# igashov/DiffLinker

Hardware: NVIDIA H100
Metric: molecules/sec (T=500 denoising) (higher is better)
Workload: dtype f32

## Files before the change

difflinker_b200/_native.py:

```python
import ctypes as C
import os

from .build import LIB_PATH, build_native, is_stale, nvcc_path

DL_OK, DL_NAN_DETECTED = 0, 1
GRAPH_TYPES = {"FC": 0, "4A": 1, "FC-4A": 2, "FC-10A-4A": 3}
EDGE_IMPLS = {"auto": 0, "simt": 1, "wgmma": 2}
SAMPLER_LINKER, SAMPLER_INPAINT = 0, 1


class DLConfig(C.Structure):
    _fields_ = [("n_dims", C.c_int32), ("in_node_nf", C.c_int32), ("context_node_nf", C.c_int32),
                ("hidden_nf", C.c_int32), ("n_layers", C.c_int32), ("inv_sublayers", C.c_int32),
                ("condition_time", C.c_int32), ("centering", C.c_int32), ("graph_type", C.c_int32),
                ("device", C.c_int32), ("edge_impl", C.c_int32), ("norm_constant", C.c_float),
                ("normalization_factor", C.c_float)]


class DLSizeGNNConfig(C.Structure):
    _fields_ = [("in_node_nf", C.c_int32), ("hidden_nf", C.c_int32), ("out_node_nf", C.c_int32),
                ("n_layers", C.c_int32), ("device", C.c_int32)]


class DLStepCoef(C.Structure):
    _fields_ = [("t", C.c_float), ("a", C.c_float), ("b", C.c_float), ("c", C.c_float), ("frame", C.c_int32),
                ("qa", C.c_float), ("qb", C.c_float), ("pad", C.c_float)]


_P, _I32, _I64, _F = C.c_void_p, C.c_int32, C.c_int64, C.c_float
SYMBOLS = {
    "dl_version": (C.c_char_p, []),
    "dl_last_error": (C.c_char_p, []),
    "dl_create": (_I32, [C.POINTER(DLConfig), C.POINTER(_P)]),
    "dl_destroy": (_I32, [_P]),
    "dl_set_weight": (_I32, [_P, C.c_char_p, _P, _I64]),
    "dl_finalize_weights": (_I32, [_P]),
    "dl_expected_param_count": (_I64, [_P]),
    "dl_dynamics_forward": (_I32, [_P, _I32, _I32, _P, _I32, _P, _P, _P, _P, _P, _P, _P, _P]),
    "dl_dynamics_forward_host": (_I32, [_P, _I32, _I32, _P, _I32, _P, _P, _P, _P, _P, _P, _P]),
    "dl_sample_chain": (_I32, [_P, _I32, _I32, _I32, _I32, _I32, _P, _P, _P, _P, _P, _P, _P, _P, _P, _P, _P, _P]),
    "dl_sample_chain_rng": (_I32, [_P, _I32, _I32, _I32, _I32, _I32, _P, _P, _P, _P, _P, _P, C.c_uint64, C.c_uint64, _P, _P, _P, _P,
                                   _P, _P]),
    "dl_set_noise_slice": (_I32, [_P, _I32, _I32]),
    "dl_noise_fill": (_I32, [_P, _I32, _I32, _I32, C.c_uint64, C.c_uint64, _P, _P, _P]),
    "dl_sample_chain_host": (_I32, [_P, _I32, _I32, _I32, _I32, _I32, _P, _P, _P, _P, _P, _P, _P, _P, _P, _P, _P]),
    "dl_launch_count": (_I64, [_P]),
    "dl_last_elapsed_ms": (_F, [_P]),
    "dl_time_edge_kernel": (_F, [_P, _I32]),
    "dl_selftest_tc": (_I32, [_P, C.POINTER(_F), C.POINTER(_F)]),
    "dl_selftest_tc_layout": (_I32, [_P, _I32, C.POINTER(_F), C.POINTER(_F)]),
    "dl_cut_graph_stats": (_I32, [_P, C.POINTER(_I64)]),
    "dl_sizegnn_create": (_I32, [C.POINTER(DLSizeGNNConfig), C.POINTER(_P)]),
    "dl_sizegnn_destroy": (_I32, [_P]),
    "dl_sizegnn_set_weight": (_I32, [_P, C.c_char_p, _P, _I64]),
    "dl_sizegnn_finalize_weights": (_I32, [_P]),
    "dl_sizegnn_forward": (_I32, [_P, _I32, _I32, _P, _P, _P, _P, _P]),
    "dl_restore_frame": (_I32, [_I32, _I32, _I32, _P, _P, _P, _P, _P]),
    "dl_restore_frame2": (_I32, [_I32, _I32, _I32, _I32, _P, _P, _P, _P, _P]),
    "dl_bond_orders": (_I32, [_I32, _I32, _I32, _P, _I32, _P, _P, _P, _P, _P, _P, _P]),
    "dl_format_xyz": (_I64, [_I32, _I32, _I32, _P, _I32, _P, _I32, _P, C.POINTER(C.c_char_p), _I32, _P, _I64, _P]),
}

_lib = None


def load_library():
    global _lib
    if _lib is not None:
        return _lib
    if is_stale():
        if nvcc_path() is not None:
            build_native()
        elif not os.path.isfile(LIB_PATH):
            raise RuntimeError(
                f"{LIB_PATH} is missing and nvcc is unavailable; build it with `python -m difflinker_b200.build`. "
                "difflinker_b200 has no CPU fallback.")
    lib = C.CDLL(LIB_PATH)
    for name, (res, args) in SYMBOLS.items():
        fn = getattr(lib, name)
        fn.restype = res
        fn.argtypes = args
    _lib = lib
    return lib


class NativeError(RuntimeError):
    pass


def check(status: int, what: str):
    if status < 0:
        raise NativeError(f"{what} failed with status {status}: {load_library().dl_last_error().decode()}")
    return status
```

difflinker_b200/build.py:

```python
import os
import shutil
import subprocess
import sys

PKG_DIR = os.path.dirname(os.path.abspath(__file__))
CSRC = os.path.join(PKG_DIR, "csrc")
LIB_PATH = os.path.join(PKG_DIR, "libdifflinker_b200.so")
SOURCES = ["dl_engine.cu", "output_stage.cu"]
HEADERS = ["common.cuh", "size_gnn.cuh", "kernels_simt.cuh", "kernels_tc.cuh", "kernels_node_tc.cuh", os.path.join("..", "..", "include", "difflinker_b200.h")]


def nvcc_path():
    for cand in (os.environ.get("NVCC"), shutil.which("nvcc"), "/usr/local/cuda/bin/nvcc"):
        if cand and os.path.isfile(cand):
            return cand
    return None


def is_stale() -> bool:
    if not os.path.isfile(LIB_PATH):
        return True
    t = os.path.getmtime(LIB_PATH)
    for f in SOURCES + HEADERS:
        p = os.path.join(CSRC, f)
        if os.path.isfile(p) and os.path.getmtime(p) > t:
            return True
    return False


def build_native(force: bool = False, verbose: bool = False) -> str:
    if not force and not is_stale():
        return LIB_PATH
    nvcc = nvcc_path()
    if nvcc is None:
        raise RuntimeError("nvcc not found: cannot build libdifflinker_b200.so")
    cmd = [nvcc, "-gencode", "arch=compute_90a,code=sm_90a", "-O3", "-lineinfo", "-std=c++17",
           "-Xcompiler", "-fPIC", "-shared", "-o", LIB_PATH] + [os.path.join(CSRC, s) for s in SOURCES]
    if verbose:
        cmd.insert(1, "-Xptxas=-v")
        print(" ".join(cmd), file=sys.stderr)
    res = subprocess.run(cmd, capture_output=True, text=True)
    if res.returncode != 0:
        raise RuntimeError(f"nvcc failed:\n{res.stdout}\n{res.stderr}")
    if verbose:
        print(res.stderr, file=sys.stderr)
    return LIB_PATH


if __name__ == "__main__":
    print(build_native(force="--force" in sys.argv, verbose=True))
```

difflinker_b200/csrc/common.cuh:

```cuda
#pragma once
#include <cuda_runtime.h>
#include <stdint.h>

namespace dl {

constexpr int H = 128;
constexpr int MAX_DIN = 32;
constexpr int MAX_XHD = 16;

__device__ __forceinline__ void chain_wait() { asm volatile("griddepcontrol.wait;" ::: "memory"); }
__device__ __forceinline__ void chain_release() { asm volatile("griddepcontrol.launch_dependents;" ::: "memory"); }

inline bool& chain_overlap_enabled() { static bool on = true; return on; }

template <typename... KArgs, typename... Args>
inline cudaError_t launch_chain(void (*kernel)(KArgs...), dim3 grid, dim3 block, size_t smem, cudaStream_t st, Args&&... args) {
  cudaLaunchConfig_t cfg = {};
  cfg.gridDim = grid; cfg.blockDim = block; cfg.dynamicSmemBytes = smem; cfg.stream = st;
  cudaLaunchAttribute at[1];
  at[0].id = cudaLaunchAttributeProgrammaticStreamSerialization;
  at[0].val.programmaticStreamSerializationAllowed = chain_overlap_enabled() ? 1 : 0;
  cfg.attrs = at; cfg.numAttrs = 1;
  return cudaLaunchKernelEx(&cfg, kernel, KArgs(static_cast<Args&&>(args))...);
}

__device__ __forceinline__ float silu_f(float x) {
  float t, r;
  asm("ex2.approx.ftz.f32 %0, %1;" : "=f"(t) : "f"(x * -1.4426950408889634f));
  asm("rcp.approx.ftz.f32 %0, %1;" : "=f"(r) : "f"(1.0f + t));
  return x * r;
}

__device__ __forceinline__ float usig_f(float u) {
  float t, r;
  asm("ex2.approx.ftz.f32 %0, %1;" : "=f"(t) : "f"(u));
  asm("rcp.approx.ftz.f32 %0, %1;" : "=f"(r) : "f"(1.0f + t));
  return u * r;
}

__device__ __forceinline__ float2 fadd2(float2 a, float2 b) { return make_float2(__fadd_rn(a.x, b.x), __fadd_rn(a.y, b.y)); }
__device__ __forceinline__ float2 fmul2(float2 a, float2 b) { return make_float2(__fmul_rn(a.x, b.x), __fmul_rn(a.y, b.y)); }
__device__ __forceinline__ float2 ffma2(float2 a, float2 b, float2 c) { return make_float2(__fmaf_rn(a.x, b.x, c.x), __fmaf_rn(a.y, b.y, c.y)); }
__device__ __forceinline__ float ex2_approx(float x) { float y; asm("ex2.approx.ftz.f32 %0, %1;" : "=f"(y) : "f"(x)); return y; }
__device__ __forceinline__ float rcp_approx(float x) { float y; asm("rcp.approx.ftz.f32 %0, %1;" : "=f"(y) : "f"(x)); return y; }
__device__ __forceinline__ float2 sigmoid_pair_log2(float2 u) {
  const float2 den = fadd2(make_float2(ex2_approx(fminf(u.x, 63.0f)), ex2_approx(fminf(u.y, 63.0f))), make_float2(1.0f, 1.0f));
  const float r = rcp_approx(den.x * den.y);
  return fmul2(make_float2(r, r), make_float2(den.y, den.x));
}
__device__ __forceinline__ void usig4(float2 u01, float2 u23, float2& s01, float2& s23) {
  const float2 one = make_float2(1.0f, 1.0f);
  const float2 ab = fadd2(make_float2(ex2_approx(fminf(u01.x, 31.0f)), ex2_approx(fminf(u01.y, 31.0f))), one);
  const float2 cd = fadd2(make_float2(ex2_approx(fminf(u23.x, 31.0f)), ex2_approx(fminf(u23.y, 31.0f))), one);
  const float2 m = fmul2(ab, cd);
  const float r = rcp_approx(m.x * m.y);
  const float2 rm = fmul2(make_float2(r, r), make_float2(m.y, m.x));
  s01 = fmul2(u01, fmul2(rm, cd));
  s23 = fmul2(u23, fmul2(rm, ab));
}
__device__ __forceinline__ float2 usig2(float2 u) { return fmul2(u, sigmoid_pair_log2(u)); }
__device__ __forceinline__ float2 silu2(float2 x) {
  return fmul2(x, sigmoid_pair_log2(fmul2(x, make_float2(-1.4426950408889634f, -1.4426950408889634f))));
}

struct GclW {
  const float* W1a_t;
  const float* W1b_t;
  const float* b1;
  const float* wd;
  const float* w0;
  const float* W2_t;
  const float* b2;
  const float* W3_t;
  const float* b3;
  const float* W4_t;
  const float* b4;
  const void* W2_tc;
  float w2_descale;
  float wdmax, w0max;
  const void* W1_tc;
  const void* W3_tc;
  const void* W4_tc;
  float w1_descale, w3_descale, w4_descale;
  const float* b1_u;
  const float* wd_u;
  const float* w0_u;
};

struct EqW {
  const float* W1a_t;
  const float* W1b_t;
  const float* b1;
  const float* wd;
  const float* w0;
  const float* W2_t;
  const float* b2;
  const float* w5;
  const void* W2_tc;
  float w2_descale;
  float wdmax, w0max;
  const void* W1_tc;
  float w1_descale;
  const float* b1_u;
  const float* wd_u;
  const float* w0_u;
};

struct ProjW {
  const float* W1a_t;
  const float* W1b_t;
  const float* b1;
};

struct Plan {
  const int* rowidx;
  const int* colidx;
  const int* xrowidx;
  const int* nr;
  const int* nc;
  const int* nxr;
  const int4* items;
  const int* n_items;
  const int* xmols;
  const int* n_xmols;
  const int4* xitems;
  const int* n_xitems;
};

struct Geom {
  int B, N;
  int F;
  int C;
  int D;
  int graph_type;
  float norm_constant;
  float normalization_factor;
};

}
```

difflinker_b200/csrc/dl_engine.cu:

```cuda
#include <cuda_fp16.h>
#include <cuda_runtime.h>

#include <algorithm>
#include <cmath>
#include <cstdarg>
#include <cstdio>
#include <cstdlib>
#include <cstring>
#include <ctime>
#include <map>
#include <string>
#include <vector>

#include "../../include/difflinker_b200.h"
#include "kernels_simt.cuh"
#include "kernels_tc.cuh"
#include "kernels_node_tc.cuh"

using namespace dl;

static thread_local char g_err[1024] = "";
static void set_err(const char* fmt, ...) {
  va_list ap;
  va_start(ap, fmt);
  vsnprintf(g_err, sizeof(g_err), fmt, ap);
  va_end(ap);
}

#define CK(call)                                                                          \
  do {                                                                                    \
    cudaError_t _e = (call);                                                              \
    if (_e != cudaSuccess) {                                                              \
      set_err("%s:%d %s -> %s", __FILE__, __LINE__, #call, cudaGetErrorString(_e));       \
      return DL_ERR_CUDA;                                                                 \
    }                                                                                     \
  } while (0)

namespace {

struct Workspace {
  int B = 0, N = 0;
  float *nm = nullptr, *x0 = nullptr, *xa = nullptr, *xb = nullptr, *h = nullptr, *ABg = nullptr, *ABc = nullptr,
        *agg = nullptr, *z = nullptr, *ABgmax = nullptr, *ABcmax = nullptr, *eps = nullptr;
  int* cls = nullptr;
  int *nbr = nullptr, *recs = nullptr, *xrecs = nullptr, *n_recs = nullptr;
  float4 *x04 = nullptr, *xa4 = nullptr, *xb4 = nullptr;
  int *rowidx = nullptr, *colidx = nullptr, *xrowidx = nullptr, *nr = nullptr, *nc = nullptr, *nxr = nullptr,
      *n_items = nullptr, *xmols = nullptr, *n_xmols = nullptr, *n_xitems = nullptr;
  int4* items = nullptr;
  int4* xitems = nullptr;
  int* tile_ctr = nullptr;
  std::vector<void*> allocs;
};

struct HostStage {
  size_t cap = 0;
  char* buf = nullptr;
};

}

struct dl_engine {
  dl_config cfg{};
  int D = 0;
  int num_sms = 0;
  int max_threads_per_sm = 2048;
  int slice_B_full = 0, slice_b0 = 0;
  bool finalized = false;
  std::map<std::string, std::vector<float>> raw;
  float* wblob = nullptr;
  void* wblob_tc = nullptr;
  std::vector<GclW> gcl;
  std::vector<EqW> eq;
  const float *We_t = nullptr, *be = nullptr, *Wo = nullptr, *bo = nullptr;
  Workspace ws;
  cudaStream_t loop_stream = nullptr;
  cudaEvent_t ev_in = nullptr, ev_out = nullptr, ev_t0 = nullptr, ev_t1 = nullptr;
  float* coef_dev = nullptr;
  int coef_cap = 0;
  int* step_ctr = nullptr;
  int64_t launches = 0;
  HostStage stage;
  bool use_tc = false;
  const int8_t* last_edge_mask = nullptr;
  const float* last_linker_mask = nullptr;
  int last_B = 0, last_N = 0;
};

namespace {

struct KernelTimes {
  bool on = false;
  struct Rec { const char* label; cudaEvent_t a, b; };
  std::vector<Rec> pending;
  std::map<std::string, std::pair<double, long>> acc;
  void begin(cudaStream_t st, const char* label) {
    if (!on) return;
    cudaStreamCaptureStatus cap = cudaStreamCaptureStatusNone;
    cudaStreamIsCapturing(st, &cap);
    if (cap != cudaStreamCaptureStatusNone) return;
    Rec r{label, nullptr, nullptr};
    cudaEventCreate(&r.a); cudaEventCreate(&r.b);
    cudaEventRecord(r.a, st);
    pending.push_back(r);
  }
  void end(cudaStream_t st) {
    if (!on || pending.empty() || pending.back().b == nullptr) return;
    cudaStreamCaptureStatus cap = cudaStreamCaptureStatusNone;
    cudaStreamIsCapturing(st, &cap);
    if (cap != cudaStreamCaptureStatusNone) return;
    cudaEventRecord(pending.back().b, st);
  }
  void collect(cudaStream_t st) {
    if (!on || pending.empty()) return;
    cudaStreamSynchronize(st);
    for (auto& r : pending) {
      float ms = 0.f;
      if (cudaEventElapsedTime(&ms, r.a, r.b) == cudaSuccess) { auto& a = acc[r.label]; a.first += ms; a.second += 1; }
      cudaEventDestroy(r.a); cudaEventDestroy(r.b);
    }
    pending.clear();
  }
  void report() {
    if (!on || acc.empty()) return;
    double tot = 0;
    for (auto& kv : acc) tot += kv.second.first;
    for (auto& kv : acc)
      fprintf(stderr, "[dl times] %-22s %6ld launches  avg %8.2f us  share %5.1f%%\n", kv.first.c_str(), kv.second.second,
              1e3 * kv.second.first / kv.second.second, 100.0 * kv.second.first / tot);
  }
};
KernelTimes g_times;
#define TIMED(label, stream, stmt) do { g_times.begin(stream, label); stmt; g_times.end(stream); } while (0)

struct ExpectedParam {
  std::string name;
  int64_t numel;
};

std::vector<ExpectedParam> expected_params(const dl_config& c) {
  const int D = c.in_node_nf + c.context_node_nf + (c.condition_time ? 1 : 0);
  const int Hh = c.hidden_nf;
  std::vector<ExpectedParam> v;
  v.push_back({"dynamics.embedding.weight", (int64_t)Hh * D});
  v.push_back({"dynamics.embedding.bias", Hh});
  v.push_back({"dynamics.embedding_out.weight", (int64_t)D * Hh});
  v.push_back({"dynamics.embedding_out.bias", D});
  char buf[160];
  for (int l = 0; l < c.n_layers; ++l) {
    for (int s = 0; s < c.inv_sublayers; ++s) {
      snprintf(buf, sizeof(buf), "dynamics.e_block_%d.gcl_%d.", l, s);
      std::string p(buf);
      v.push_back({p + "edge_mlp.0.weight", (int64_t)Hh * (2 * Hh + 2)});
      v.push_back({p + "edge_mlp.0.bias", Hh});
      v.push_back({p + "edge_mlp.2.weight", (int64_t)Hh * Hh});
      v.push_back({p + "edge_mlp.2.bias", Hh});
      v.push_back({p + "node_mlp.0.weight", (int64_t)Hh * 2 * Hh});
      v.push_back({p + "node_mlp.0.bias", Hh});
      v.push_back({p + "node_mlp.2.weight", (int64_t)Hh * Hh});
      v.push_back({p + "node_mlp.2.bias", Hh});
    }
    snprintf(buf, sizeof(buf), "dynamics.e_block_%d.gcl_equiv.", l);
    std::string p(buf);
    v.push_back({p + "coord_mlp.0.weight", (int64_t)Hh * (2 * Hh + 2)});
    v.push_back({p + "coord_mlp.0.bias", Hh});
    v.push_back({p + "coord_mlp.2.weight", (int64_t)Hh * Hh});
    v.push_back({p + "coord_mlp.2.bias", Hh});
    v.push_back({p + "coord_mlp.4.weight", Hh});
  }
  return v;
}

struct Packer {
  std::vector<float> blob;
  size_t add(const std::vector<float>& seg) {
    while (blob.size() % 4) blob.push_back(0.f);
    size_t off = blob.size();
    blob.insert(blob.end(), seg.begin(), seg.end());
    return off;
  }
};

std::vector<float> transpose_block(const std::vector<float>& W, int out, int in_stride, int c0, int k) {
  std::vector<float> t((size_t)k * out);
  for (int o = 0; o < out; ++o)
    for (int i = 0; i < k; ++i) t[(size_t)i * out + o] = W[(size_t)o * in_stride + c0 + i];
  return t;
}
std::vector<float> column(const std::vector<float>& W, int out, int in_stride, int c) {
  std::vector<float> t(out);
  for (int o = 0; o < out; ++o) t[o] = W[(size_t)o * in_stride + c];
  return t;
}

template <typename T>
dl_status dev_alloc(Workspace& ws, T** p, size_t count) {
  void* q = nullptr;
  CK(cudaMalloc(&q, std::max<size_t>(count, 1) * sizeof(T)));
  ws.allocs.push_back(q);
  *p = reinterpret_cast<T*>(q);
  return DL_OK;
}

void free_workspace(Workspace& ws) {
  for (void* p : ws.allocs) cudaFree(p);
  ws = Workspace();
}

dl_status ensure_workspace(dl_engine* e, int B, int N) {
  Workspace& ws = e->ws;
  if (ws.B == B && ws.N == N) return DL_OK;
  free_workspace(ws);
  const size_t n = (size_t)B * N;
  const int xd = 3 + e->cfg.in_node_nf;
  dl_status s;
#define WSA(field, cnt) if ((s = dev_alloc(ws, &ws.field, (cnt))) != DL_OK) return s
  WSA(nm, n); WSA(x0, n * 3); WSA(xa, n * 3); WSA(xb, n * 3); WSA(h, n * H); WSA(ABg, n * 2 * H); WSA(ABc, n * 2 * H);
  WSA(agg, n * H); WSA(z, n * xd); WSA(eps, n * xd); WSA(cls, n); WSA(x04, n); WSA(xa4, n); WSA(xb4, n); WSA(ABgmax, n * 2); WSA(ABcmax, n * 2);
  WSA(rowidx, n); WSA(colidx, n); WSA(xrowidx, n); WSA(nr, B); WSA(nc, B); WSA(nxr, B); WSA(n_items, 1);
  WSA(xmols, B); WSA(n_xmols, 1); WSA(items, n); WSA(xitems, n); WSA(n_xitems, 1); WSA(tile_ctr, 64);
  if (e->use_tc && e->cfg.graph_type != 0) { WSA(nbr, n * N); WSA(recs, n * CUT_REC); WSA(xrecs, n * CUT_REC); WSA(n_recs, 2); }
#undef WSA
  ws.B = B; ws.N = N;
  return DL_OK;
}

Plan make_plan(const Workspace& ws) {
  Plan p;
  p.rowidx = ws.rowidx; p.colidx = ws.colidx; p.xrowidx = ws.xrowidx; p.nr = ws.nr; p.nc = ws.nc; p.nxr = ws.nxr;
  p.items = ws.items; p.n_items = ws.n_items; p.xmols = ws.xmols; p.n_xmols = ws.n_xmols;
  p.xitems = ws.xitems; p.n_xitems = ws.n_xitems;
  return p;
}

Geom make_geom(const dl_engine* e, int B, int N) {
  Geom g;
  g.B = B; g.N = N; g.F = e->cfg.in_node_nf; g.C = e->cfg.context_node_nf; g.D = e->D;
  g.graph_type = e->cfg.graph_type; g.norm_constant = e->cfg.norm_constant;
  g.normalization_factor = e->cfg.normalization_factor;
  return g;
}

#define LAUNCH_CHECK()                                                                    \
  do {                                                                                    \
    cudaError_t _e = cudaGetLastError();                                                  \
    if (_e != cudaSuccess) {                                                              \
      set_err("%s:%d kernel launch -> %s", __FILE__, __LINE__, cudaGetErrorString(_e));   \
      return DL_ERR_CUDA;                                                                 \
    }                                                                                     \
  } while (0)

dl_status build_plan(dl_engine* e, int B, int N, const int8_t* node_mask, const float* linker_mask,
                     const int8_t* edge_mask, cudaStream_t st) {
  Workspace& ws = e->ws;
  CK(cudaMemsetAsync(ws.agg, 0, (size_t)B * N * H * sizeof(float), st));
  k_plan_mol<<<B, 256, 2 * N * sizeof(int), st>>>(N, e->cfg.graph_type, edge_mask, node_mask, linker_mask, ws.rowidx,
                                                  ws.colidx, ws.xrowidx, ws.nr, ws.nc, ws.nxr);
  LAUNCH_CHECK();
  const int tile_edges = e->use_tc ? tc::TN : ET;
  const int max_rows = e->use_tc ? tc::MAXR : MAXR;
  k_plan_items<<<1, 1, 0, st>>>(B, tile_edges, max_rows, 1, max_rows, ws.nr, ws.nc, ws.nxr, ws.items, ws.n_items, ws.xmols,
                                ws.n_xmols, ws.xitems, ws.n_xitems);
  LAUNCH_CHECK();
  e->launches += 2;
  return DL_OK;
}

struct FwdIO {
  const float* xh = nullptr; const float* t = nullptr; int t_numel = 0; float* out = nullptr;
  const int8_t* node_mask = nullptr; const float* linker_mask = nullptr; const int8_t* edge_mask = nullptr;
  const float* context = nullptr; int* nan_flags = nullptr;
  bool sampler = false; bool inpaint = false; const float* xh0 = nullptr; const float* upd_linker_mask = nullptr;
  const float* fragment_mask = nullptr; const float* noise = nullptr; float* chain = nullptr;
  NoiseRng rng{};
  int T = 0; float norm0 = 1.f, norm1 = 1.f, bias1 = 0.f;
};

ProjW proj_of(const GclW& w) { return ProjW{w.W1a_t, w.W1b_t, w.b1}; }
ProjW proj_of(const EqW& w) { return ProjW{w.W1a_t, w.W1b_t, w.b1}; }

dl_status launch_edge(dl_engine* e, const Geom& gm, const EdgeArgs& ea, bool coord, const void* w2_tc, cudaStream_t st) {
  if (e->use_tc) {
    dl_status s = tc::launch_edge_tc(gm, ea, coord, w2_tc, e->num_sms, st);
    if (s != DL_OK) return s;
  } else {
    if (coord) k_edge_simt<true><<<e->num_sms, 256, EDGE_SIMT_SMEM, st>>>(gm, ea);
    else k_edge_simt<false><<<e->num_sms, 256, EDGE_SIMT_SMEM, st>>>(gm, ea);
  }
  LAUNCH_CHECK();
  e->launches += 1;
  return DL_OK;
}

dl_status enqueue_forward(dl_engine* e, int B, int N, const FwdIO& io, cudaStream_t st) {
  Workspace& ws = e->ws;
  const Geom gm = make_geom(e, B, N);
  const int n = B * N;
  const int L = e->cfg.n_layers, S = e->cfg.inv_sublayers;
  const int node_blocks = (n + NODE_TM - 1) / NODE_TM;
  const size_t node_smem = 3 * NODE_TM * LDX * sizeof(float);

  PrepArgs pa{};
  pa.xh = io.sampler ? ws.z : io.xh;
  pa.node_mask = io.node_mask; pa.linker_mask = io.linker_mask;
  pa.t = io.t; pa.t_numel = io.t_numel; pa.context = io.context;
  pa.We_t = e->We_t; pa.be = e->be; pa.proj = proj_of(e->gcl[0]);
  pa.nm = ws.nm; pa.x0 = ws.x0; pa.x = ws.xa; pa.x04 = e->use_tc ? ws.x04 : nullptr; pa.x4 = e->use_tc ? ws.xa4 : nullptr; pa.cls = ws.cls; pa.h = ws.h;
  pa.AB = e->use_tc ? nullptr : ws.ABg; pa.ABmax = ws.ABgmax;
  pa.coef = io.sampler ? e->coef_dev : nullptr;
  pa.step_prep = io.sampler ? e->step_ctr : nullptr;
  pa.step_fin = io.sampler ? e->step_ctr + 1 : nullptr;
  TIMED("k_prep", st, (launch_chain(k_prep, dim3(node_blocks), dim3(256), 0, st, gm, pa)));
  LAUNCH_CHECK();
  e->launches += 1;
  if (e->use_tc) {
    const GclW& w0 = e->gcl[0];
    tcn::NodeTcArgs ta{};
    ta.h = ws.h; ta.agg = ws.h; ta.nm = ws.nm; ta.proj_only = 1;
    ta.w3 = reinterpret_cast<const __half*>(w0.W3_tc); ta.w4 = reinterpret_cast<const __half*>(w0.W4_tc);
    ta.b3 = w0.b3; ta.b4 = w0.b4; ta.w3_descale = 1.f; ta.w4_descale = 1.f;
    ta.n_proj = 1; ta.pw[0] = reinterpret_cast<const __half*>(w0.W1_tc); ta.pb1[0] = w0.b1_u;
    ta.p_descale[0] = w0.w1_descale; ta.AB[0] = ws.ABg; ta.ABmax[0] = ws.ABgmax;
    ta.tile_nodes = tcn::pick_tile_nodes(n, e->num_sms);
    TIMED("k_node_tc(proj only)", st, (tcn::launch_node(n, ta, st)));
    LAUNCH_CHECK();
    e->launches += 1;
  }

  if (ws.nbr != nullptr) {
    CK(cudaMemsetAsync(ws.n_recs, 0, 2 * sizeof(int), st));
    k_nbr<<<B, 512, (size_t)N * CUT_SMEM_PER_NODE, st>>>(N, e->cfg.graph_type, ws.x04, ws.cls, ws.rowidx, ws.colidx,
                                                        ws.xrowidx, ws.nr, ws.nc, ws.nxr, ws.nbr, ws.recs, ws.xrecs,
                                                        ws.n_recs);
    LAUNCH_CHECK();
    e->launches += 1;
  }

  float* xin = ws.xa;
  float* xout = ws.xb;
  float4* xin4 = ws.xa4;
  float4* xout4 = ws.xb4;
  const Plan plan = make_plan(ws);
  const float ksc = e->use_tc ? 1.4426950408889634f : 1.0f;
  e->last_edge_mask = io.edge_mask; e->last_linker_mask = io.linker_mask; e->last_B = B; e->last_N = N;
  for (int l = 0; l < L; ++l) {
    for (int s = 0; s < S; ++s) {
      const GclW& w = e->gcl[l * S + s];
      EdgeArgs ea{};
      ea.AB = ws.ABg; ea.ABmax = ws.ABgmax; ea.w2_descale = w.w2_descale; ea.wdmax = w.wdmax * ksc; ea.w0max = w.w0max * ksc;
      ea.x = xin; ea.x0 = ws.x0; ea.x4 = xin4; ea.x04 = ws.x04; ea.x4_out = nullptr;
      ea.edge_mask = io.edge_mask; ea.cls = ws.cls; ea.nm = ws.nm;
      ea.linker_mask = io.linker_mask; ea.W2_t = w.W2_t; ea.b2 = w.b2; ea.wd = e->use_tc ? w.wd_u : w.wd; ea.w0 = e->use_tc ? w.w0_u : w.w0; ea.w5 = nullptr;
      ea.plan = plan; ea.agg = ws.agg; ea.x_out = nullptr; ea.nbr = ws.nbr; ea.recs = ws.recs; ea.n_recs = ws.n_recs;
      g_times.begin(st, "edge GCL");
      dl_status st2 = launch_edge(e, gm, ea, false, w.W2_tc, st);
      g_times.end(st);
      if (st2 != DL_OK) return st2;

      const bool last_sub = s + 1 >= S;
      if (e->use_tc) {
        tcn::NodeTcArgs ta{};
        ta.h = ws.h; ta.agg = ws.agg; ta.nm = ws.nm;
        ta.w3 = reinterpret_cast<const __half*>(w.W3_tc); ta.w4 = reinterpret_cast<const __half*>(w.W4_tc);
        ta.b3 = w.b3; ta.b4 = w.b4; ta.w3_descale = w.w3_descale; ta.w4_descale = w.w4_descale;
        if (!last_sub) {
          const GclW& nx = e->gcl[l * S + s + 1];
          ta.n_proj = 1; ta.pw[0] = reinterpret_cast<const __half*>(nx.W1_tc); ta.pb1[0] = nx.b1_u;
          ta.p_descale[0] = nx.w1_descale; ta.AB[0] = ws.ABg; ta.ABmax[0] = ws.ABgmax;
        } else {
          const EqW& q = e->eq[l];
          ta.n_proj = 1; ta.pw[0] = reinterpret_cast<const __half*>(q.W1_tc); ta.pb1[0] = q.b1_u;
          ta.p_descale[0] = q.w1_descale; ta.AB[0] = ws.ABc; ta.ABmax[0] = ws.ABcmax;
          if (l + 1 < L) {
            const GclW& nx = e->gcl[(l + 1) * S];
            ta.n_proj = 2; ta.pw[1] = reinterpret_cast<const __half*>(nx.W1_tc); ta.pb1[1] = nx.b1_u;
            ta.p_descale[1] = nx.w1_descale; ta.AB[1] = ws.ABg; ta.ABmax[1] = ws.ABgmax;
          }
        }
        ta.tile_nodes = tcn::pick_tile_nodes(n, e->num_sms);
        TIMED(ta.n_proj == 2 ? "k_node_tc(2 proj)" : "k_node_tc(1 proj)", st, (tcn::launch_node(n, ta, st)));
      } else {
        NodeArgs na{};
        na.h = ws.h; na.agg = ws.agg; na.nm = ws.nm; na.W3_t = w.W3_t; na.b3 = w.b3; na.W4_t = w.W4_t; na.b4 = w.b4;
        if (!last_sub) {
          na.proj1 = proj_of(e->gcl[l * S + s + 1]); na.AB1 = ws.ABg; na.ABmax1 = ws.ABgmax; na.AB2 = nullptr;
        } else {
          na.proj1 = proj_of(e->eq[l]); na.AB1 = ws.ABc; na.ABmax1 = ws.ABcmax;
          if (l + 1 < L) { na.proj2 = proj_of(e->gcl[(l + 1) * S]); na.AB2 = ws.ABg; na.ABmax2 = ws.ABgmax; }
          else na.AB2 = nullptr;
        }
        k_node<ACT_SILU><<<node_blocks, 256, node_smem, st>>>(n, na);
      }
      LAUNCH_CHECK();
      e->launches += 1;
    }
    k_copy_x<<<(n * 3 + 255) / 256, 256, 0, st>>>(n * 3, xin, xout, e->use_tc ? xin4 : nullptr, xout4);
    LAUNCH_CHECK();
    e->launches += 1;
    const EqW& w = e->eq[l];
    EdgeArgs ea{};
    ea.AB = ws.ABc; ea.ABmax = ws.ABcmax; ea.w2_descale = w.w2_descale; ea.wdmax = w.wdmax * ksc; ea.w0max = w.w0max * ksc;
    ea.x = xin; ea.x0 = ws.x0; ea.x4 = xin4; ea.x04 = ws.x04; ea.x4_out = xout4;
    ea.edge_mask = io.edge_mask; ea.cls = ws.cls; ea.nm = ws.nm;
    ea.linker_mask = io.linker_mask; ea.W2_t = w.W2_t; ea.b2 = w.b2; ea.wd = e->use_tc ? w.wd_u : w.wd; ea.w0 = e->use_tc ? w.w0_u : w.w0; ea.w5 = w.w5;
    ea.plan = plan; ea.agg = nullptr; ea.x_out = xout; ea.nbr = ws.nbr; ea.recs = ws.xrecs; ea.n_recs = ws.n_recs ? ws.n_recs + 1 : nullptr;
    g_times.begin(st, "edge COORD");
    dl_status st2 = launch_edge(e, gm, ea, true, w.W2_tc, st);
    g_times.end(st);
    if (st2 != DL_OK) return st2;
    std::swap(xin, xout);
    std::swap(xin4, xout4);
  }

  FinishArgs fa{};
  fa.h = ws.h; fa.x = xin; fa.x0 = ws.x0; fa.nm = ws.nm; fa.Wo = e->Wo; fa.bo = e->bo;
  fa.nan_flags = io.nan_flags;
  const bool fused_update = io.sampler && !io.inpaint;
  fa.out = fused_update ? nullptr : (io.sampler ? ws.eps : io.out);
  if (fused_update) {
    fa.z = ws.z; fa.fragment_mask = io.fragment_mask; fa.linker_mask = io.linker_mask; fa.noise = io.noise; fa.rng = io.rng;
    fa.coef = e->coef_dev; fa.step_fin = e->step_ctr + 1; fa.step_prep = e->step_ctr; fa.T = io.T;
    fa.norm0 = io.norm0; fa.norm1 = io.norm1; fa.bias1 = io.bias1; fa.chain = io.chain;
  } else if (io.sampler) {
    fa.tag_step = e->step_ctr + 1;
  }
  TIMED("k_finish", st, (launch_chain(k_finish, dim3((n + 15) / 16), dim3(256), 0, st, gm, fa)));
  LAUNCH_CHECK();
  e->launches += 1;
  if (e->cfg.centering || io.inpaint) {
    InpaintArgs ia{};
    ia.mode = io.inpaint ? 1 : 0;
    ia.eps = io.inpaint ? ws.eps : io.out; ia.nm = ws.nm; ia.z = ws.z; ia.xh0 = io.xh0;
    ia.fragment_mask = io.fragment_mask; ia.linker_mask = io.upd_linker_mask; ia.noise = io.noise; ia.coef = e->coef_dev;
    ia.step_prep = e->step_ctr; ia.step_fin = e->step_ctr + 1; ia.T = io.T;
    ia.norm0 = io.norm0; ia.norm1 = io.norm1; ia.bias1 = io.bias1; ia.chain = io.chain;
    k_inpaint<<<B, 256, 0, st>>>(gm, ia);
    LAUNCH_CHECK();
    e->launches += 1;
  }
  return DL_OK;
}

dl_status check_shapes(const dl_engine* e, int B, int N) {
  if (!e || !e->finalized) { set_err("engine not finalized (dl_finalize_weights)"); return DL_ERR_INVALID; }
  if (B <= 0 || N <= 0) { set_err("B and N must be positive (got %d, %d)", B, N); return DL_ERR_INVALID; }
  if ((int64_t)B * N * N > (int64_t)1 << 40) { set_err("B*N*N too large"); return DL_ERR_INVALID; }
  if (e->use_tc && e->cfg.graph_type != 0 && N > 4000) {
    set_err("cut-off graphs: N = %d exceeds the neighbour-list kernel's shared-memory staging (N <= 4000)", N);
    return DL_ERR_INVALID;
  }
  return DL_OK;
}

dl_status stage_reserve(dl_engine* e, size_t bytes) {
  if (e->stage.cap >= bytes) return DL_OK;
  if (e->stage.buf) cudaFree(e->stage.buf);
  e->stage.buf = nullptr; e->stage.cap = 0;
  CK(cudaMalloc((void**)&e->stage.buf, bytes));
  e->stage.cap = bytes;
  return DL_OK;
}

size_t align256(size_t v) { return (v + 255) & ~(size_t)255; }

}

extern "C" {

const char* dl_version(void) { return "difflinker_b200 0.1 (sm_90a)"; }
const char* dl_last_error(void) { return g_err; }

dl_status dl_create(const dl_config* cfg, dl_engine** out) {
  if (!cfg || !out) { set_err("null argument"); return DL_ERR_INVALID; }
  if (cfg->hidden_nf != H) { set_err("hidden_nf must be %d (got %d)", H, cfg->hidden_nf); return DL_ERR_UNSUPPORTED; }
  if (cfg->n_dims != 3) { set_err("n_dims must be 3"); return DL_ERR_UNSUPPORTED; }
  const int D = cfg->in_node_nf + cfg->context_node_nf + (cfg->condition_time ? 1 : 0);
  if (D > MAX_DIN || cfg->in_node_nf < 1 || 3 + cfg->in_node_nf > MAX_XHD) {
    set_err("unsupported feature widths F=%d C=%d", cfg->in_node_nf, cfg->context_node_nf);
    return DL_ERR_UNSUPPORTED;
  }
  if (cfg->n_layers < 1 || cfg->inv_sublayers < 1) { set_err("n_layers/inv_sublayers must be >= 1"); return DL_ERR_INVALID; }
  if (cfg->graph_type < 0 || cfg->graph_type > 3) { set_err("bad graph_type"); return DL_ERR_INVALID; }
  if (cfg->graph_type != DL_GRAPH_FC && cfg->context_node_nf < 2) {
    set_err("pocket graphs need fragment_only/pocket_only context columns"); return DL_ERR_INVALID;
  }
  int ndev = 0;
  CK(cudaGetDeviceCount(&ndev));
  if (cfg->device < 0 || cfg->device >= ndev) { set_err("device %d not available (%d devices)", cfg->device, ndev); return DL_ERR_INVALID; }
  CK(cudaSetDevice(cfg->device));
  cudaDeviceProp prop;
  CK(cudaGetDeviceProperties(&prop, cfg->device));
  if (prop.major != 9 || prop.minor != 0) {
    set_err("difflinker_b200 is built for sm_90a only; device is sm_%d%d", prop.major, prop.minor);
    return DL_ERR_UNSUPPORTED;
  }
  dl_engine* e = new dl_engine();
  e->cfg = *cfg;
  e->D = D;
  e->num_sms = prop.multiProcessorCount;
  e->max_threads_per_sm = prop.maxThreadsPerMultiProcessor;
  e->use_tc = tc::AVAILABLE && cfg->edge_impl != DL_EDGE_SIMT;
  CK(cudaStreamCreateWithFlags(&e->loop_stream, cudaStreamNonBlocking));
  CK(cudaEventCreateWithFlags(&e->ev_in, cudaEventDisableTiming));
  CK(cudaEventCreateWithFlags(&e->ev_out, cudaEventDisableTiming));
  CK(cudaEventCreate(&e->ev_t0));
  CK(cudaEventCreate(&e->ev_t1));
  CK(cudaMalloc((void**)&e->step_ctr, 2 * sizeof(int)));
  CK(cudaFuncSetAttribute(k_node<ACT_SILU>, cudaFuncAttributeMaxDynamicSharedMemorySize, 3 * NODE_TM * LDX * sizeof(float)));
  CK(cudaFuncSetAttribute(k_edge_simt<true>, cudaFuncAttributeMaxDynamicSharedMemorySize, (int)EDGE_SIMT_SMEM));
  CK(cudaFuncSetAttribute(k_edge_simt<false>, cudaFuncAttributeMaxDynamicSharedMemorySize, (int)EDGE_SIMT_SMEM));
  CK(cudaFuncSetAttribute(k_nbr, cudaFuncAttributeMaxDynamicSharedMemorySize, 4000 * CUT_SMEM_PER_NODE));
  if (getenv("DL_TIME_KERNELS")) g_times.on = true;
  if (const char* v = getenv("DL_WAIT_MODE")) { const int m = atoi(v); cudaMemcpyToSymbol(tc::c_wait_mode, &m, sizeof(int)); }
  if (const char* v = getenv("DL_CHAIN_OVERLAP")) chain_overlap_enabled() = atoi(v) != 0;
  dl_status s = tc::configure();
  if (s == DL_OK) s = tcn::configure_node();
  if (s != DL_OK) { set_err("cudaFuncSetAttribute failed for the tensor-core kernels"); delete e; return s; }
  *out = e;
  return DL_OK;
}

dl_status dl_destroy(dl_engine* e) {
  if (!e) return DL_OK;
  g_times.report();
  g_times.acc.clear();
  cudaSetDevice(e->cfg.device);
  cudaDeviceSynchronize();
  free_workspace(e->ws);
  if (e->wblob) cudaFree(e->wblob);
  if (e->wblob_tc) cudaFree(e->wblob_tc);
  if (e->coef_dev) cudaFree(e->coef_dev);
  if (e->step_ctr) cudaFree(e->step_ctr);
  if (e->stage.buf) cudaFree(e->stage.buf);
  if (e->loop_stream) cudaStreamDestroy(e->loop_stream);
  if (e->ev_in) cudaEventDestroy(e->ev_in);
  if (e->ev_out) cudaEventDestroy(e->ev_out);
  if (e->ev_t0) cudaEventDestroy(e->ev_t0);
  if (e->ev_t1) cudaEventDestroy(e->ev_t1);
  delete e;
  return DL_OK;
}

int64_t dl_expected_param_count(const dl_engine* e) {
  if (!e) return 0;
  int64_t n = 0;
  for (auto& p : expected_params(e->cfg)) n += p.numel;
  return n;
}

dl_status dl_set_weight(dl_engine* e, const char* name, const float* data, int64_t numel) {
  if (!e || !name || !data) { set_err("null argument"); return DL_ERR_INVALID; }
  for (auto& p : expected_params(e->cfg)) {
    if (p.name == name) {
      if (p.numel != numel) {
        set_err("weight %s: expected %lld elements, got %lld", name, (long long)p.numel, (long long)numel);
        return DL_ERR_WEIGHTS;
      }
      e->raw[p.name].assign(data, data + numel);
      e->finalized = false;
      return DL_OK;
    }
  }
  set_err("unexpected weight name %s", name);
  return DL_ERR_WEIGHTS;
}

dl_status dl_finalize_weights(dl_engine* e) {
  if (!e) { set_err("null engine"); return DL_ERR_INVALID; }
  CK(cudaSetDevice(e->cfg.device));
  for (auto& p : expected_params(e->cfg))
    if (!e->raw.count(p.name)) { set_err("missing weight %s", p.name.c_str()); return DL_ERR_WEIGHTS; }
  const int L = e->cfg.n_layers, S = e->cfg.inv_sublayers, D = e->D;
  const int IN1 = 2 * H + 2;
  Packer pk;
  std::vector<__half> tcblob;
  struct GOff { size_t W1a, W1b, b1, wd, w0, W2, b2, W3, b3, W4, b4, w5, tc, tc1, tc3, tc4, b1u, wdu, w0u; float descale, wdmax, w0max, d1, d3, d4; };
  auto scaled = [](const std::vector<float>& v) { std::vector<float> o(v.size()); for (size_t i = 0; i < v.size(); ++i) o[i] = (float)((double)v[i] * tc::NEG_LOG2E); return o; };
  auto absmax = [](const std::vector<float>& v) { float m = 0.f; for (float x : v) m = std::max(m, std::fabs(x)); return m; };
  std::vector<GOff> goff(L * S), eoff(L);
  auto R = [&](const std::string& k) -> const std::vector<float>& { return e->raw[k]; };
  size_t oWe = pk.add(transpose_block(R("dynamics.embedding.weight"), H, D, 0, D));
  size_t obe = pk.add(R("dynamics.embedding.bias"));
  size_t oWo = pk.add(R("dynamics.embedding_out.weight"));
  size_t obo = pk.add(R("dynamics.embedding_out.bias"));
  char buf[160];
  for (int l = 0; l < L; ++l) {
    for (int s = 0; s < S; ++s) {
      snprintf(buf, sizeof(buf), "dynamics.e_block_%d.gcl_%d.", l, s);
      std::string p(buf);
      GOff& o = goff[l * S + s];
      const auto& W1 = R(p + "edge_mlp.0.weight");
      o.W1a = pk.add(transpose_block(W1, H, IN1, 0, H));
      o.W1b = pk.add(transpose_block(W1, H, IN1, H, H));
      o.b1 = pk.add(R(p + "edge_mlp.0.bias"));
      o.wd = pk.add(column(W1, H, IN1, 2 * H));
      o.w0 = pk.add(column(W1, H, IN1, 2 * H + 1));
      o.W2 = pk.add(transpose_block(R(p + "edge_mlp.2.weight"), H, H, 0, H));
      o.b2 = pk.add(R(p + "edge_mlp.2.bias"));
      o.W3 = pk.add(transpose_block(R(p + "node_mlp.0.weight"), H, 2 * H, 0, 2 * H));
      o.b3 = pk.add(R(p + "node_mlp.0.bias"));
      o.W4 = pk.add(transpose_block(R(p + "node_mlp.2.weight"), H, H, 0, H));
      o.b4 = pk.add(R(p + "node_mlp.2.bias"));
      o.tc = tc::pack_w2(R(p + "edge_mlp.2.weight"), tcblob, &o.descale);
      o.tc1 = tcn::pack_blocks(scaled(W1), IN1, 2, tcblob, &o.d1);
      o.b1u = pk.add(scaled(R(p + "edge_mlp.0.bias")));
      o.wdu = pk.add(scaled(column(W1, H, IN1, 2 * H)));
      o.w0u = pk.add(scaled(column(W1, H, IN1, 2 * H + 1)));
      o.tc3 = tcn::pack_blocks(R(p + "node_mlp.0.weight"), 2 * H, 2, tcblob, &o.d3);
      o.tc4 = tcn::pack_blocks(R(p + "node_mlp.2.weight"), H, 1, tcblob, &o.d4);
      o.wdmax = absmax(column(W1, H, IN1, 2 * H)); o.w0max = absmax(column(W1, H, IN1, 2 * H + 1));
    }
    snprintf(buf, sizeof(buf), "dynamics.e_block_%d.gcl_equiv.", l);
    std::string p(buf);
    GOff& o = eoff[l];
    const auto& W1 = R(p + "coord_mlp.0.weight");
    o.W1a = pk.add(transpose_block(W1, H, IN1, 0, H));
    o.W1b = pk.add(transpose_block(W1, H, IN1, H, H));
    o.b1 = pk.add(R(p + "coord_mlp.0.bias"));
    o.wd = pk.add(column(W1, H, IN1, 2 * H));
    o.w0 = pk.add(column(W1, H, IN1, 2 * H + 1));
    o.W2 = pk.add(transpose_block(R(p + "coord_mlp.2.weight"), H, H, 0, H));
    o.b2 = pk.add(R(p + "coord_mlp.2.bias"));
    o.w5 = pk.add(R(p + "coord_mlp.4.weight"));
    o.tc = tc::pack_w2(R(p + "coord_mlp.2.weight"), tcblob, &o.descale);
    o.tc1 = tcn::pack_blocks(scaled(W1), IN1, 2, tcblob, &o.d1);
    o.b1u = pk.add(scaled(R(p + "coord_mlp.0.bias")));
    o.wdu = pk.add(scaled(column(W1, H, IN1, 2 * H)));
    o.w0u = pk.add(scaled(column(W1, H, IN1, 2 * H + 1)));
    o.wdmax = absmax(column(W1, H, IN1, 2 * H)); o.w0max = absmax(column(W1, H, IN1, 2 * H + 1));
  }
  if (e->wblob) { cudaFree(e->wblob); e->wblob = nullptr; }
  if (e->wblob_tc) { cudaFree(e->wblob_tc); e->wblob_tc = nullptr; }
  CK(cudaMalloc((void**)&e->wblob, pk.blob.size() * sizeof(float)));
  CK(cudaMemcpy(e->wblob, pk.blob.data(), pk.blob.size() * sizeof(float), cudaMemcpyHostToDevice));
  CK(cudaMalloc(&e->wblob_tc, std::max<size_t>(tcblob.size(), 1) * sizeof(__half)));
  CK(cudaMemcpy(e->wblob_tc, tcblob.data(), tcblob.size() * sizeof(__half), cudaMemcpyHostToDevice));
  const float* base = e->wblob;
  const __half* tbase = reinterpret_cast<const __half*>(e->wblob_tc);
  e->We_t = base + oWe; e->be = base + obe; e->Wo = base + oWo; e->bo = base + obo;
  e->gcl.assign(L * S, GclW{});
  e->eq.assign(L, EqW{});
  for (int i = 0; i < L * S; ++i) {
    const GOff& o = goff[i];
    e->gcl[i] = GclW{base + o.W1a, base + o.W1b, base + o.b1, base + o.wd, base + o.w0, base + o.W2, base + o.b2,
                     base + o.W3,  base + o.b3,  base + o.W4, base + o.b4, tbase + o.tc, o.descale, o.wdmax, o.w0max,
                     tbase + o.tc1, tbase + o.tc3, tbase + o.tc4, o.d1, o.d3, o.d4,
                     base + o.b1u, base + o.wdu, base + o.w0u};
  }
  for (int l = 0; l < L; ++l) {
    const GOff& o = eoff[l];
    e->eq[l] = EqW{base + o.W1a, base + o.W1b, base + o.b1, base + o.wd, base + o.w0,
                   base + o.W2,  base + o.b2,  base + o.w5, tbase + o.tc, o.descale, o.wdmax, o.w0max, tbase + o.tc1, o.d1,
                   base + o.b1u, base + o.wdu, base + o.w0u};
  }
  e->finalized = true;
  return DL_OK;
}

dl_status dl_dynamics_forward(dl_engine* e, int32_t B, int32_t N, const float* t, int32_t t_numel, const float* xh,
                              const int8_t* node_mask, const float* linker_mask, const int8_t* edge_mask,
                              const float* context, float* out, int32_t* nan_flags, void* stream) {
  dl_status s = check_shapes(e, B, N);
  if (s != DL_OK) return s;
  if (!xh || !node_mask || !out) { set_err("xh/node_mask/out must not be null"); return DL_ERR_INVALID; }
  if (e->cfg.condition_time && (!t || (t_numel != 1 && t_numel != B))) { set_err("t must hold 1 or B values"); return DL_ERR_INVALID; }
  if (e->cfg.context_node_nf > 0 && !context) { set_err("context required (context_node_nf=%d)", e->cfg.context_node_nf); return DL_ERR_INVALID; }
  CK(cudaSetDevice(e->cfg.device));
  cudaStream_t st = reinterpret_cast<cudaStream_t>(stream);
  if ((s = ensure_workspace(e, B, N)) != DL_OK) return s;
  CK(cudaEventRecord(e->ev_t0, st));
  if (nan_flags) CK(cudaMemsetAsync(nan_flags, 0, B * sizeof(int32_t), st));
  if ((s = build_plan(e, B, N, node_mask, linker_mask, edge_mask, st)) != DL_OK) return s;
  FwdIO io;
  io.xh = xh; io.t = t; io.t_numel = t_numel; io.out = out; io.node_mask = node_mask; io.linker_mask = linker_mask;
  io.edge_mask = edge_mask; io.context = context; io.nan_flags = nan_flags;
  if ((s = enqueue_forward(e, B, N, io, st)) != DL_OK) return s;
  CK(cudaEventRecord(e->ev_t1, st));
  g_times.collect(st);
  return DL_OK;
}

dl_status dl_dynamics_forward_host(dl_engine* e, int32_t B, int32_t N, const float* t, int32_t t_numel,
                                   const float* xh, const int8_t* node_mask, const float* linker_mask,
                                   const int8_t* edge_mask, const float* context, float* out, int32_t* nan_flags) {
  dl_status s = check_shapes(e, B, N);
  if (s != DL_OK) return s;
  CK(cudaSetDevice(e->cfg.device));
  const size_t n = (size_t)B * N;
  const int xd = 3 + e->cfg.in_node_nf, C = e->cfg.context_node_nf;
  const size_t o_t = 0, o_xh = o_t + align256(sizeof(float) * std::max(t_numel, 1)), o_nm = o_xh + align256(n * xd * 4),
               o_lm = o_nm + align256(n), o_em = o_lm + align256(n * 4), o_ctx = o_em + align256(n * N),
               o_out = o_ctx + align256(n * std::max(C, 1) * 4), o_fl = o_out + align256(n * xd * 4),
               total = o_fl + align256(B * 4);
  if ((s = stage_reserve(e, total)) != DL_OK) return s;
  char* d = e->stage.buf;
  cudaStream_t st = e->loop_stream;
  if (t) CK(cudaMemcpyAsync(d + o_t, t, sizeof(float) * t_numel, cudaMemcpyHostToDevice, st));
  CK(cudaMemcpyAsync(d + o_xh, xh, n * xd * 4, cudaMemcpyHostToDevice, st));
  CK(cudaMemcpyAsync(d + o_nm, node_mask, n, cudaMemcpyHostToDevice, st));
  if (linker_mask) CK(cudaMemcpyAsync(d + o_lm, linker_mask, n * 4, cudaMemcpyHostToDevice, st));
  if (edge_mask && e->cfg.graph_type == DL_GRAPH_FC) CK(cudaMemcpyAsync(d + o_em, edge_mask, n * N, cudaMemcpyHostToDevice, st));
  if (context) CK(cudaMemcpyAsync(d + o_ctx, context, n * C * 4, cudaMemcpyHostToDevice, st));
  s = dl_dynamics_forward(e, B, N, t ? (const float*)(d + o_t) : nullptr, t_numel, (const float*)(d + o_xh),
                          (const int8_t*)(d + o_nm), linker_mask ? (const float*)(d + o_lm) : nullptr,
                          (edge_mask && e->cfg.graph_type == DL_GRAPH_FC) ? (const int8_t*)(d + o_em) : nullptr,
                          context ? (const float*)(d + o_ctx) : nullptr, (float*)(d + o_out), (int32_t*)(d + o_fl), st);
  if (s != DL_OK) return s;
  std::vector<int32_t> flags(B);
  CK(cudaMemcpyAsync(out, d + o_out, n * xd * 4, cudaMemcpyDeviceToHost, st));
  CK(cudaMemcpyAsync(flags.data(), d + o_fl, B * 4, cudaMemcpyDeviceToHost, st));
  CK(cudaStreamSynchronize(st));
  bool any = false;
  for (int i = 0; i < B; ++i) { any |= flags[i] != 0; if (nan_flags) nan_flags[i] = flags[i]; }
  return any ? DL_NAN_DETECTED : DL_OK;
}

static void randn_geometry(const dl_engine* e, long long numel, int* S, unsigned long long* consumed) {
  long long grid = (numel + 255) / 256;
  grid = std::min<long long>(grid, (long long)e->num_sms * (e->max_threads_per_sm / 256));
  grid = std::max<long long>(grid, 1);
  *S = (int)(256 * grid);
  *consumed = (unsigned long long)(((numel - 1) / (4LL * *S) + 1) * 4);
}
static NoiseRng make_rng(const dl_engine* e, int B, int N, uint64_t seed, uint64_t offset) {
  NoiseRng q{};
  const int F = e->cfg.in_node_nf;
  unsigned long long cx = 0, ch = 0;
  const int B_full = e->slice_B_full > 0 ? e->slice_B_full : B;
  randn_geometry(e, (long long)B_full * N * 3, &q.Sx, &cx);
  randn_geometry(e, (long long)B_full * N * F, &q.Sh, &ch);
  q.seed = seed; q.offset = offset; q.cx = cx; q.per_draw = cx + ch; q.F = F; q.on = 1;
  q.g0 = e->slice_B_full > 0 ? e->slice_b0 * N : 0;
  return q;
}

static dl_status sample_chain_impl(dl_engine* e, int32_t sampler, int32_t B, int32_t N, int32_t T, int32_t keep_frames,
                                   const float* xh, const int8_t* node_mask, const float* fragment_mask,
                                   const float* linker_mask, const int8_t* edge_mask, const float* context,
                                   const float* noise, const NoiseRng* rng, const dl_step_coef* coef, const float* norm,
                                   float* chain, int32_t* nan_flags, void* stream);

dl_status dl_sample_chain(dl_engine* e, int32_t sampler, int32_t B, int32_t N, int32_t T, int32_t keep_frames,
                          const float* xh, const int8_t* node_mask, const float* fragment_mask,
                          const float* linker_mask, const int8_t* edge_mask, const float* context,
                          const float* noise, const dl_step_coef* coef, const float* norm, float* chain,
                          int32_t* nan_flags, void* stream) {
  if (!noise) { set_err("null argument (noise): use dl_sample_chain_rng to draw on the device"); return DL_ERR_INVALID; }
  return sample_chain_impl(e, sampler, B, N, T, keep_frames, xh, node_mask, fragment_mask, linker_mask, edge_mask, context, noise,
                           nullptr, coef, norm, chain, nan_flags, stream);
}

dl_status dl_sample_chain_rng(dl_engine* e, int32_t sampler, int32_t B, int32_t N, int32_t T, int32_t keep_frames,
                              const float* xh, const int8_t* node_mask, const float* fragment_mask,
                              const float* linker_mask, const int8_t* edge_mask, const float* context, uint64_t seed,
                              uint64_t offset, uint64_t* offset_consumed, const dl_step_coef* coef, const float* norm,
                              float* chain, int32_t* nan_flags, void* stream) {
  dl_status s = check_shapes(e, B, N);
  if (s != DL_OK) return s;
  if (e->slice_B_full > 0 && e->slice_b0 + B > e->slice_B_full) { set_err("batch slice [%d, %d) exceeds the full batch %d", e->slice_b0, e->slice_b0 + B, e->slice_B_full); return DL_ERR_INVALID; }
  if (sampler != DL_SAMPLER_LINKER) { set_err("device-side noise is implemented for the linker sampler (the inpainting sampler takes prepared slabs)"); return DL_ERR_UNSUPPORTED; }
  if (offset % 4 != 0) { set_err("philox offset must be a multiple of 4 (torch.Generator.get_offset())"); return DL_ERR_INVALID; }
  const NoiseRng q = make_rng(e, B, N, seed, offset);
  if (offset_consumed) *offset_consumed = (uint64_t)(T + 2) * q.per_draw;
  return sample_chain_impl(e, sampler, B, N, T, keep_frames, xh, node_mask, fragment_mask, linker_mask, edge_mask, context, nullptr,
                           &q, coef, norm, chain, nan_flags, stream);
}

dl_status dl_set_noise_slice(dl_engine* e, int32_t B_full, int32_t b0) {
  if (!e) { set_err("null engine"); return DL_ERR_INVALID; }
  if (B_full < 0 || b0 < 0 || (B_full > 0 && b0 >= B_full)) { set_err("bad batch slice (%d of %d)", b0, B_full); return DL_ERR_INVALID; }
  e->slice_B_full = B_full; e->slice_b0 = B_full > 0 ? b0 : 0;
  return DL_OK;
}

dl_status dl_noise_fill(dl_engine* e, int32_t n_draws, int32_t B, int32_t N, uint64_t seed, uint64_t offset, float* out,
                        uint64_t* offset_consumed, void* stream) {
  dl_status s = check_shapes(e, B, N);
  if (s != DL_OK) return s;
  if (!out || n_draws < 1) { set_err("null argument"); return DL_ERR_INVALID; }
  CK(cudaSetDevice(e->cfg.device));
  const NoiseRng q = make_rng(e, B, N, seed, offset);
  if (offset_consumed) *offset_consumed = (uint64_t)n_draws * q.per_draw;
  k_noise_fill<<<e->num_sms * 4, 256, 0, reinterpret_cast<cudaStream_t>(stream)>>>(n_draws, B * N, 3 + e->cfg.in_node_nf, q, out);
  LAUNCH_CHECK();
  return DL_OK;
}

static dl_status sample_chain_impl(dl_engine* e, int32_t sampler, int32_t B, int32_t N, int32_t T, int32_t keep_frames,
                                   const float* xh, const int8_t* node_mask, const float* fragment_mask,
                                   const float* linker_mask, const int8_t* edge_mask, const float* context,
                                   const float* noise, const NoiseRng* rng, const dl_step_coef* coef, const float* norm,
                                   float* chain, int32_t* nan_flags, void* stream) {
  dl_status s = check_shapes(e, B, N);
  if (s != DL_OK) return s;
  if (sampler != DL_SAMPLER_LINKER && sampler != DL_SAMPLER_INPAINT) { set_err("unknown sampler %d", sampler); return DL_ERR_INVALID; }
  const bool inpaint = sampler == DL_SAMPLER_INPAINT;
  if (inpaint != (e->cfg.centering != 0)) { set_err("the inpainting sampler needs a model built with centering=1 (and vice versa)"); return DL_ERR_INVALID; }
  if (!xh || !node_mask || !fragment_mask || !linker_mask || (!noise && !rng) || !coef || !norm || !chain) {
    set_err("null argument"); return DL_ERR_INVALID;
  }
  if (T < 1 || keep_frames < 1 || keep_frames > T) { set_err("need 1 <= keep_frames <= T"); return DL_ERR_INVALID; }
  if (e->cfg.context_node_nf > 0 && !context) { set_err("context required"); return DL_ERR_INVALID; }
  static_assert(sizeof(dl_step_coef) == 32, "dl_step_coef layout");
  CK(cudaSetDevice(e->cfg.device));
  cudaStream_t user = reinterpret_cast<cudaStream_t>(stream);
  cudaStream_t st = e->loop_stream;
  static const bool time_chain = getenv("DL_TIME_CHAIN") != nullptr;
  auto now_ms = [] { timespec ts; clock_gettime(CLOCK_MONOTONIC, &ts); return ts.tv_sec * 1e3 + ts.tv_nsec * 1e-6; };
  const double tc0 = time_chain ? now_ms() : 0.0;
  double tc_plan = 0, tc_capture = 0, tc_inst = 0, tc_launch = 0;
  if ((s = ensure_workspace(e, B, N)) != DL_OK) return s;
  if (e->coef_cap < T + 1) {
    if (e->coef_dev) cudaFree(e->coef_dev);
    e->coef_dev = nullptr;
    CK(cudaMalloc((void**)&e->coef_dev, (size_t)(T + 1) * sizeof(dl_step_coef)));
    e->coef_cap = T + 1;
  }
  if (user != st) {
    CK(cudaEventRecord(e->ev_in, user));
    CK(cudaStreamWaitEvent(st, e->ev_in, 0));
  }
  CK(cudaMemcpyAsync(e->coef_dev, coef, (size_t)(T + 1) * sizeof(dl_step_coef), cudaMemcpyHostToDevice, st));
  CK(cudaMemsetAsync(e->step_ctr, 0, 2 * sizeof(int), st));
  if (nan_flags) CK(cudaMemsetAsync(nan_flags, 0, B * sizeof(int32_t), st));
  const int n = B * N, xd = 3 + e->cfg.in_node_nf;
  CK(cudaMemsetAsync(chain, 0, (size_t)keep_frames * n * xd * sizeof(float), st));
  if (inpaint) {
    CK(cudaMemcpyAsync(e->ws.z, noise, (size_t)n * xd * sizeof(float), cudaMemcpyDeviceToDevice, st));
  } else {
    k_init_z<<<(n * xd + 255) / 256, 256, 0, st>>>(n, xd, xh, fragment_mask, linker_mask, noise, rng ? *rng : NoiseRng{}, e->ws.z);
    LAUNCH_CHECK();
    e->launches += 1;
  }
  if ((s = build_plan(e, B, N, node_mask, inpaint ? nullptr : linker_mask, edge_mask, st)) != DL_OK) return s;

  if (time_chain) { cudaStreamSynchronize(st); tc_plan = now_ms(); }
  FwdIO io;
  io.sampler = true; io.inpaint = inpaint; io.xh0 = xh; io.upd_linker_mask = linker_mask;
  io.node_mask = node_mask; io.linker_mask = inpaint ? nullptr : linker_mask; io.edge_mask = edge_mask;
  io.context = context; io.nan_flags = nan_flags; io.fragment_mask = fragment_mask; io.noise = noise;
  if (rng) io.rng = *rng;
  io.chain = chain; io.T = T; io.norm0 = norm[0]; io.norm1 = norm[1]; io.bias1 = norm[2];

  cudaGraph_t graph = nullptr;
  cudaGraphExec_t exec = nullptr;
  const int64_t before = e->launches;
  CK(cudaStreamBeginCapture(st, cudaStreamCaptureModeThreadLocal));
  s = enqueue_forward(e, B, N, io, st);
  cudaError_t ce = cudaStreamEndCapture(st, &graph);
  if (s != DL_OK) { if (graph) cudaGraphDestroy(graph); return s; }
  if (ce != cudaSuccess) { set_err("cudaStreamEndCapture -> %s", cudaGetErrorString(ce)); return DL_ERR_CUDA; }
  const int64_t per_step = e->launches - before;
  if (time_chain) tc_capture = now_ms();
  cudaError_t ge = cudaGraphInstantiate(&exec, graph, 0);
  if (time_chain) tc_inst = now_ms();
  if (ge == cudaSuccess) ge = cudaEventRecord(e->ev_t0, st);
  int failed_step = -1;
  for (int r = 0; ge == cudaSuccess && r <= T; ++r) {
    ge = cudaGraphLaunch(exec, st);
    if (ge != cudaSuccess) failed_step = r;
  }
  if (ge == cudaSuccess) ge = cudaEventRecord(e->ev_t1, st);
  if (time_chain) {
    tc_launch = now_ms();
    cudaStreamSynchronize(st);
    const double tc_done = now_ms();
    float loop = 0.f; cudaEventElapsedTime(&loop, e->ev_t0, e->ev_t1);
    fprintf(stderr, "[dl chain] setup+plan %.2f ms | capture %.2f | instantiate %.2f | %d graph launches enqueued in %.2f | wait for the GPU %.2f | device loop %.2f\n",
            tc_plan - tc0, tc_capture - tc_plan, tc_inst - tc_capture, T + 1, tc_launch - tc_inst, tc_done - tc_launch, loop);
  }
  if (ge == cudaSuccess && user != st) {
    ge = cudaEventRecord(e->ev_out, st);
    if (ge == cudaSuccess) ge = cudaStreamWaitEvent(user, e->ev_out, 0);
  }
  if (exec) cudaGraphExecDestroy(exec);
  cudaGraphDestroy(graph);
  if (ge != cudaSuccess) {
    if (failed_step >= 0) set_err("cudaGraphLaunch step %d -> %s", failed_step, cudaGetErrorString(ge));
    else set_err("%s:%d reverse-loop graph -> %s", __FILE__, __LINE__, cudaGetErrorString(ge));
    return DL_ERR_CUDA;
  }
  e->launches = before + per_step * (T + 1);
  return DL_OK;
}

dl_status dl_sample_chain_host(dl_engine* e, int32_t sampler, int32_t B, int32_t N, int32_t T, int32_t keep_frames,
                               const float* xh, const int8_t* node_mask, const float* fragment_mask,
                               const float* linker_mask, const int8_t* edge_mask, const float* context,
                               const float* noise, const dl_step_coef* coef, const float* norm, float* chain,
                               int32_t* nan_flags) {
  dl_status s = check_shapes(e, B, N);
  if (s != DL_OK) return s;
  if (!xh || !node_mask || !fragment_mask || !linker_mask || !noise || !coef || !norm || !chain) {
    set_err("null argument"); return DL_ERR_INVALID;
  }
  if (T < 1 || keep_frames < 1 || keep_frames > T) { set_err("need 1 <= keep_frames <= T"); return DL_ERR_INVALID; }
  CK(cudaSetDevice(e->cfg.device));
  const size_t n = (size_t)B * N;
  const int xd = 3 + e->cfg.in_node_nf, C = e->cfg.context_node_nf;
  const bool has_em = edge_mask && e->cfg.graph_type == DL_GRAPH_FC;
  const size_t n_slabs = sampler == DL_SAMPLER_INPAINT ? (size_t)2 * T + 3 : (size_t)T + 2;
  const size_t o_xh = 0, o_nm = o_xh + align256(n * xd * 4), o_fm = o_nm + align256(n), o_lm = o_fm + align256(n * 4),
               o_em = o_lm + align256(n * 4), o_ctx = o_em + align256(has_em ? n * N : 1),
               o_nz = o_ctx + align256(n * std::max(C, 1) * 4), o_ch = o_nz + align256((size_t)n_slabs * n * xd * 4),
               o_fl = o_ch + align256((size_t)keep_frames * n * xd * 4), total = o_fl + align256(B * 4);
  if ((s = stage_reserve(e, total)) != DL_OK) return s;
  char* d = e->stage.buf;
  cudaStream_t st = e->loop_stream;
  CK(cudaMemcpyAsync(d + o_xh, xh, n * xd * 4, cudaMemcpyHostToDevice, st));
  CK(cudaMemcpyAsync(d + o_nm, node_mask, n, cudaMemcpyHostToDevice, st));
  CK(cudaMemcpyAsync(d + o_fm, fragment_mask, n * 4, cudaMemcpyHostToDevice, st));
  CK(cudaMemcpyAsync(d + o_lm, linker_mask, n * 4, cudaMemcpyHostToDevice, st));
  if (has_em) CK(cudaMemcpyAsync(d + o_em, edge_mask, n * N, cudaMemcpyHostToDevice, st));
  if (context) CK(cudaMemcpyAsync(d + o_ctx, context, n * C * 4, cudaMemcpyHostToDevice, st));
  CK(cudaMemcpyAsync(d + o_nz, noise, n_slabs * n * xd * 4, cudaMemcpyHostToDevice, st));
  s = dl_sample_chain(e, sampler, B, N, T, keep_frames, (const float*)(d + o_xh), (const int8_t*)(d + o_nm),
                      (const float*)(d + o_fm), (const float*)(d + o_lm), has_em ? (const int8_t*)(d + o_em) : nullptr,
                      context ? (const float*)(d + o_ctx) : nullptr, (const float*)(d + o_nz), coef, norm,
                      (float*)(d + o_ch), (int32_t*)(d + o_fl), st);
  if (s != DL_OK) return s;
  std::vector<int32_t> flags(B);
  CK(cudaMemcpyAsync(chain, d + o_ch, (size_t)keep_frames * n * xd * 4, cudaMemcpyDeviceToHost, st));
  CK(cudaMemcpyAsync(flags.data(), d + o_fl, B * 4, cudaMemcpyDeviceToHost, st));
  CK(cudaStreamSynchronize(st));
  bool any = false;
  for (int i = 0; i < B; ++i) { any |= flags[i] != 0; if (nan_flags) nan_flags[i] = flags[i]; }
  return any ? DL_NAN_DETECTED : DL_OK;
}

int64_t dl_launch_count(const dl_engine* e) { return e ? e->launches : 0; }

float dl_last_elapsed_ms(dl_engine* e) {
  if (!e) return -1.f;
  float ms = -1.f;
  if (cudaEventElapsedTime(&ms, e->ev_t0, e->ev_t1) != cudaSuccess) { cudaGetLastError(); return -1.f; }
  return ms;
}

dl_status dl_cut_graph_stats(dl_engine* e, int64_t* out) {
  if (!e || !out) return DL_ERR_INVALID;
  Workspace& ws = e->ws;
  out[0] = out[1] = out[2] = out[3] = 0;
  if (ws.recs == nullptr) return DL_OK;
  if (cudaSetDevice(e->cfg.device) != cudaSuccess) return DL_ERR_CUDA;
  CK(cudaDeviceSynchronize());
  int n[2] = {0, 0};
  CK(cudaMemcpy(n, ws.n_recs, sizeof(n), cudaMemcpyDeviceToHost));
  std::vector<int> recs((size_t)n[0] * CUT_REC);
  CK(cudaMemcpy(recs.data(), ws.recs, recs.size() * sizeof(int), cudaMemcpyDeviceToHost));
  out[0] = n[0]; out[3] = n[1];
  long long n_heavy = 0, e_heavy = 0, max_heavy = 0, rows_light = 0;
  for (int k = 0; k < n[0]; ++k) {
    const int* r = recs.data() + (size_t)k * CUT_REC;
    const bool heavy = (r[1] >> 8) & 1;
    out[1] += heavy ? (r[2] + tc::TN - 1) / tc::TN : 1;
    out[2] += r[2];
    if (heavy) { ++n_heavy; e_heavy += r[2]; max_heavy = std::max<long long>(max_heavy, r[2]); }
    else rows_light += r[1] & 0xff;
  }
  if (getenv("DL_DEBUG_CUT"))
    fprintf(stderr, "[dl cut] records %d (heavy %lld, deg sum %lld, max %lld; light rows %lld) tiles %lld edges %lld | coord records %d\n",
            n[0], n_heavy, e_heavy, max_heavy, rows_light, (long long)out[1], (long long)out[2], n[1]);
  return DL_OK;
}

float dl_time_edge_kernel(dl_engine* e, int32_t reps) {
  if (!e || !e->finalized || e->last_B == 0 || reps < 1) { set_err("dl_time_edge_kernel: no previous forward"); return -1.f; }
  if (cudaSetDevice(e->cfg.device) != cudaSuccess) return -1.f;
  Workspace& ws = e->ws;
  const Geom gm = make_geom(e, e->last_B, e->last_N);
  const GclW& w = e->gcl[0];
  EdgeArgs ea{};
  const float ksc = e->use_tc ? 1.4426950408889634f : 1.0f;
  ea.AB = ws.ABg; ea.ABmax = ws.ABgmax; ea.w2_descale = w.w2_descale; ea.wdmax = w.wdmax * ksc; ea.w0max = w.w0max * ksc;
  ea.x = ws.xa; ea.x0 = ws.x0; ea.x4 = ws.xa4; ea.x04 = ws.x04; ea.x4_out = nullptr; ea.edge_mask = e->last_edge_mask; ea.cls = ws.cls; ea.nm = ws.nm;
  ea.linker_mask = e->last_linker_mask; ea.W2_t = w.W2_t; ea.b2 = w.b2; ea.wd = e->use_tc ? w.wd_u : w.wd; ea.w0 = e->use_tc ? w.w0_u : w.w0; ea.w5 = nullptr;
  ea.plan = make_plan(ws); ea.agg = ws.agg; ea.x_out = nullptr; ea.nbr = ws.nbr; ea.recs = ws.recs; ea.n_recs = ws.n_recs;
  cudaStream_t st = e->loop_stream;
  for (int i = 0; i < 2; ++i) if (launch_edge(e, gm, ea, false, w.W2_tc, st) != DL_OK) return -1.f;
  if (cudaEventRecord(e->ev_t0, st) != cudaSuccess) return -1.f;
  for (int i = 0; i < reps; ++i) if (launch_edge(e, gm, ea, false, w.W2_tc, st) != DL_OK) return -1.f;
  if (cudaEventRecord(e->ev_t1, st) != cudaSuccess) return -1.f;
  if (cudaStreamSynchronize(st) != cudaSuccess) { set_err("dl_time_edge_kernel: %s", cudaGetErrorString(cudaGetLastError())); return -1.f; }
  float ms = -1.f;
  if (cudaEventElapsedTime(&ms, e->ev_t0, e->ev_t1) != cudaSuccess) return -1.f;
  return ms / reps;
}

dl_status dl_selftest_tc(dl_engine* e, float* max_abs_err, float* max_rel_err) {
  if (!e) { set_err("null engine"); return DL_ERR_INVALID; }
  CK(cudaSetDevice(e->cfg.device));
  return tc::selftest(e->num_sms, max_abs_err, max_rel_err, false);
}

dl_status dl_selftest_tc_layout(dl_engine* e, int32_t b_mn_major, float* max_abs_err, float* max_rel_err) {
  if (!e) { set_err("null engine"); return DL_ERR_INVALID; }
  CK(cudaSetDevice(e->cfg.device));
  if (b_mn_major < 0 || b_mn_major > 1) { set_err("b_mn_major must be 0 (K-major B) or 1 (MN-major B)"); return DL_ERR_INVALID; }
  return tc::selftest(e->num_sms, max_abs_err, max_rel_err, b_mn_major != 0);
}

}

#include "size_gnn.cuh"
```

difflinker_b200/csrc/kernels_simt.cuh:

```cuda
#pragma once
#include <curand_kernel.h>

#include "common.cuh"

namespace dl {

__global__ void k_plan_mol(int N, int graph_type, const int8_t* __restrict__ edge_mask,
                           const int8_t* __restrict__ node_mask, const float* __restrict__ linker_mask,
                           int* __restrict__ rowidx, int* __restrict__ colidx, int* __restrict__ xrowidx,
                           int* __restrict__ nr, int* __restrict__ nc, int* __restrict__ nxr) {
  extern __shared__ int sm_plan[];
  int* rowlive = sm_plan;
  int* collive = sm_plan + N;
  const int b = blockIdx.x;
  const int tid = threadIdx.x, lane = tid & 31, warp = tid >> 5, nwarp = blockDim.x >> 5;
  for (int i = tid; i < N; i += blockDim.x) { rowlive[i] = 0; collive[i] = 0; }
  __syncthreads();
  if ((graph_type == 0 || graph_type == 4) && edge_mask != nullptr) {
    const int8_t* em = edge_mask + (size_t)b * N * N;
    for (int i = warp; i < N; i += nwarp) {
      int any = 0;
      for (int j = lane; j < N; j += 32) {
        int v = em[(size_t)i * N + j];
        if (v != 0) { any = 1; collive[j] = 1; }
      }
      any = __any_sync(0xffffffffu, any);
      if (lane == 0 && any) rowlive[i] = 1;
    }
  } else if (graph_type == 0 || graph_type == 4) {
    for (int i = tid; i < N; i += blockDim.x) { rowlive[i] = 1; collive[i] = 1; }
  } else {
    for (int i = tid; i < N; i += blockDim.x) {
      int v = node_mask[(size_t)b * N + i] != 0;
      rowlive[i] = v; collive[i] = v;
    }
  }
  __syncthreads();
  if (tid == 0) {
    int a = 0, c = 0, x = 0;
    for (int i = 0; i < N; ++i) {
      if (rowlive[i]) {
        rowidx[(size_t)b * N + a++] = i;
        if (linker_mask == nullptr || linker_mask[(size_t)b * N + i] != 0.0f) xrowidx[(size_t)b * N + x++] = i;
      }
      if (collive[i]) colidx[(size_t)b * N + c++] = i;
    }
    nr[b] = a; nc[b] = c; nxr[b] = x;
  }
}

__global__ void k_plan_items(int B, int tile_edges, int max_rows, int col_pad, int max_rows_gcl, const int* __restrict__ nr,
                             const int* __restrict__ nc, const int* __restrict__ nxr, int4* __restrict__ items,
                             int* __restrict__ n_items, int* __restrict__ xmols, int* __restrict__ n_xmols,
                             int4* __restrict__ xitems, int* __restrict__ n_xitems, int n_cta = 0,
                             int* __restrict__ cta_begin = nullptr, int* __restrict__ xcta_begin = nullptr) {
  if (threadIdx.x != 0 || blockIdx.x != 0) return;
  int cnt = 0, xc = 0, xi = 0;
  for (int b = 0; b < B; ++b) {
    int r = nr[b], c = nc[b];
    if (r > 0 && c > 0) {
      const int cp = (c + col_pad - 1) / col_pad * col_pad;
      int per = cp >= tile_edges ? 1 : tile_edges / cp;
      if (per > max_rows_gcl) per = max_rows_gcl;
      for (int r0 = 0; r0 < r; r0 += per) items[cnt++] = make_int4(b, r0, min(per, r - r0), c);
    }
    if (nxr[b] > 0 && c > 0) {
      xmols[xc++] = b;
      int per;
      if (col_pad > 1) {
        const int cp = (c + col_pad - 1) / col_pad * col_pad;
        per = cp >= tile_edges ? 1 : tile_edges / cp;
        if (per > max_rows_gcl) per = max_rows_gcl;
      } else {
        per = c >= tile_edges ? 1 : tile_edges / c;
        if (per > max_rows) per = max_rows;
      }
      for (int r0 = 0; r0 < nxr[b]; r0 += per) xitems[xi++] = make_int4(b, r0, min(per, nxr[b] - r0), c);
    }
  }
  *n_items = cnt;
  *n_xmols = xc;
  *n_xitems = xi;
  if (n_cta > 0 && cta_begin != nullptr) {
    for (int pass = 0; pass < 2; ++pass) {
      const int4* list = pass == 0 ? items : xitems;
      const int total = pass == 0 ? cnt : xi;
      int* out = pass == 0 ? cta_begin : xcta_begin;
      if (out == nullptr) continue;
      long long sum = 0;
      for (int k = 0; k < total; ++k) sum += (long long)list[k].z * ((list[k].w + col_pad - 1) / col_pad * col_pad) + 32;
      long long run = 0;
      int c = 0;
      out[0] = 0;
      for (int k = 0; k < total; ++k) {
        while (c + 1 < n_cta && run * n_cta >= (long long)(c + 1) * sum) out[++c] = k;
        run += (long long)list[k].z * ((list[k].w + col_pad - 1) / col_pad * col_pad) + 32;
      }
      while (c < n_cta) out[++c] = total;
    }
  }
}

constexpr int ACT_SILU = 0, ACT_RELU = 1;
template <int ACT>
__device__ __forceinline__ float act_f(float x) { return ACT == ACT_RELU ? fmaxf(x, 0.f) : silu_f(x); }

constexpr int NODE_TM = 32;
constexpr int LDX = 132;

template <int K>
__device__ __forceinline__ void warp_gemm_4x4(const float* __restrict__ xs, const float* __restrict__ Wt, int lane,
                                              float (&acc)[4][4]) {
#pragma unroll 2
  for (int k = 0; k < K; k += 4) {
    float4 w[4], x[4];
#pragma unroll
    for (int q = 0; q < 4; ++q) w[q] = __ldg(reinterpret_cast<const float4*>(Wt + (size_t)(k + q) * H + lane * 4));
#pragma unroll
    for (int r = 0; r < 4; ++r) x[r] = *reinterpret_cast<const float4*>(xs + r * LDX + k);
#pragma unroll
    for (int r = 0; r < 4; ++r) {
      const float xv[4] = {x[r].x, x[r].y, x[r].z, x[r].w};
#pragma unroll
      for (int q = 0; q < 4; ++q) {
        acc[r][0] = fmaf(xv[q], w[q].x, acc[r][0]);
        acc[r][1] = fmaf(xv[q], w[q].y, acc[r][1]);
        acc[r][2] = fmaf(xv[q], w[q].z, acc[r][2]);
        acc[r][3] = fmaf(xv[q], w[q].w, acc[r][3]);
      }
    }
  }
}

__device__ __forceinline__ void zero_acc(float (&acc)[4][4]) {
#pragma unroll
  for (int r = 0; r < 4; ++r)
#pragma unroll
    for (int c = 0; c < 4; ++c) acc[r][c] = 0.f;
}

__device__ __forceinline__ float warp_absmax4(const float (&v)[4]) {
  float m = fmaxf(fmaxf(fabsf(v[0]), fabsf(v[1])), fmaxf(fabsf(v[2]), fabsf(v[3])));
#pragma unroll
  for (int o = 16; o > 0; o >>= 1) m = fmaxf(m, __shfl_xor_sync(0xffffffffu, m, o));
  return m;
}

__device__ __forceinline__ void project_ab(const float* hs_warp, const ProjW& pw, float* __restrict__ AB,
                                           float* __restrict__ ABmax, int g0, int n_total, int warp, int lane) {
  float acc[4][4];
  zero_acc(acc);
  warp_gemm_4x4<H>(hs_warp, pw.W1a_t, lane, acc);
  const float4 bb = __ldg(reinterpret_cast<const float4*>(pw.b1 + lane * 4));
#pragma unroll
  for (int r = 0; r < 4; ++r) {
    int g = g0 + warp * 4 + r;
    const float o[4] = {acc[r][0] + bb.x, acc[r][1] + bb.y, acc[r][2] + bb.z, acc[r][3] + bb.w};
    const float mx = warp_absmax4(o);
    if (g < n_total) {
      *reinterpret_cast<float4*>(AB + (size_t)g * 2 * H + lane * 4) = make_float4(o[0], o[1], o[2], o[3]);
      if (lane == 0) ABmax[(size_t)g * 2] = mx;
    }
  }
  zero_acc(acc);
  warp_gemm_4x4<H>(hs_warp, pw.W1b_t, lane, acc);
#pragma unroll
  for (int r = 0; r < 4; ++r) {
    int g = g0 + warp * 4 + r;
    const float mx = warp_absmax4(acc[r]);
    if (g < n_total) {
      *reinterpret_cast<float4*>(AB + (size_t)g * 2 * H + H + lane * 4) =
          make_float4(acc[r][0], acc[r][1], acc[r][2], acc[r][3]);
      if (lane == 0) ABmax[(size_t)g * 2 + 1] = mx;
    }
  }
}

struct PrepArgs {
  const float* xh;
  const int8_t* node_mask;
  const float* linker_mask;
  const float* t;
  int t_numel;
  const float* context;
  const float* We_t;
  const float* be;
  ProjW proj;
  float* nm;
  float* x0;
  float* x;
  float4* x04;
  float4* x4;
  int* cls;
  float* h;
  float* AB;
  float* ABmax;
  const float* coef;
  const int* step_prep;
  int* step_fin;
};

__global__ void __launch_bounds__(256) k_prep(Geom gm, PrepArgs a) {
  __shared__ __align__(16) float hs[NODE_TM * LDX];
  __shared__ float hin[NODE_TM][MAX_DIN];
  const int tid = threadIdx.x, lane = tid & 31, warp = tid >> 5;
  const int n_total = gm.B * gm.N;
  const int g0 = blockIdx.x * NODE_TM;
  const int xd = 3 + gm.F;
  int step = 0;
  chain_wait();
  chain_release();
  if (a.step_prep != nullptr) {
    step = *a.step_prep;
    if (blockIdx.x == 0 && tid == 0) *a.step_fin = step;
  }
  for (int idx = tid; idx < NODE_TM * MAX_DIN; idx += 256) {
    int r = idx / MAX_DIN, d = idx % MAX_DIN;
    int g = g0 + r;
    float v = 0.f;
    if (g < n_total && d < gm.D) {
      float m = (float)a.node_mask[g];
      if (d < gm.F) {
        v = a.xh[(size_t)g * xd + 3 + d] * m;
      } else if (d == gm.F && gm.D > gm.F + gm.C) {
        if (a.coef != nullptr) v = a.coef[(size_t)step * 8 + 0];
        else v = a.t[a.t_numel == 1 ? 0 : g / gm.N];
      } else {
        int cidx = d - (gm.D - gm.C);
        v = a.context[(size_t)g * gm.C + cidx];
      }
    }
    hin[r][d] = v;
  }
  if (tid < NODE_TM) {
    int g = g0 + tid;
    if (g < n_total) {
      float m = (float)a.node_mask[g];
      a.nm[g] = m;
      for (int d = 0; d < 3; ++d) {
        float v = a.xh[(size_t)g * xd + d] * m;
        a.x0[(size_t)g * 3 + d] = v;
        a.x[(size_t)g * 3 + d] = v;
        if (a.x4 != nullptr) {
          reinterpret_cast<float*>(a.x04 + g)[d] = v;
          reinterpret_cast<float*>(a.x4 + g)[d] = v;
        }
      }
      if (gm.graph_type >= 1 && gm.graph_type <= 3) {
        int valid = m != 0.f;
        int pk = a.context[(size_t)g * gm.C + gm.C - 1] != 0.f;
        int fr = a.context[(size_t)g * gm.C + gm.C - 2] != 0.f;
        int lk = a.linker_mask != nullptr ? (a.linker_mask[g] != 0.f) : 0;
        int c = 0;
        if (valid) {
          if (gm.graph_type == 1) c = 1;
          else c = (lk || fr) ? 1 : (pk ? 2 : 3);
        }
        a.cls[g] = c;
      }
    }
  }
  __syncthreads();
  {
    float acc[4][4];
    zero_acc(acc);
    for (int d = 0; d < gm.D; ++d) {
      const float4 w = __ldg(reinterpret_cast<const float4*>(a.We_t + (size_t)d * H + lane * 4));
#pragma unroll
      for (int r = 0; r < 4; ++r) {
        float xv = hin[warp * 4 + r][d];
        acc[r][0] = fmaf(xv, w.x, acc[r][0]);
        acc[r][1] = fmaf(xv, w.y, acc[r][1]);
        acc[r][2] = fmaf(xv, w.z, acc[r][2]);
        acc[r][3] = fmaf(xv, w.w, acc[r][3]);
      }
    }
    const float4 bb = __ldg(reinterpret_cast<const float4*>(a.be + lane * 4));
#pragma unroll
    for (int r = 0; r < 4; ++r) {
      float4 o = make_float4(acc[r][0] + bb.x, acc[r][1] + bb.y, acc[r][2] + bb.z, acc[r][3] + bb.w);
      *reinterpret_cast<float4*>(hs + (warp * 4 + r) * LDX + lane * 4) = o;
      int g = g0 + warp * 4 + r;
      if (g < n_total) *reinterpret_cast<float4*>(a.h + (size_t)g * H + lane * 4) = o;
    }
  }
  __syncwarp();
  if (a.AB != nullptr) project_ab(hs + warp * 4 * LDX, a.proj, a.AB, a.ABmax, g0, n_total, warp, lane);
}

struct NodeArgs {
  float* h;
  const float* agg;
  const float* nm;
  const float* W3_t; const float* b3; const float* W4_t; const float* b4;
  ProjW proj1; float* AB1; float* ABmax1;
  ProjW proj2; float* AB2; float* ABmax2;
};

template <int ACT = ACT_SILU>
__global__ void __launch_bounds__(256) k_node(int n_total, NodeArgs a) {
  extern __shared__ __align__(16) float sm_node[];
  float* hs = sm_node;
  float* as = sm_node + NODE_TM * LDX;
  float* hid = as + NODE_TM * LDX;
  const int tid = threadIdx.x, lane = tid & 31, warp = tid >> 5;
  const int g0 = blockIdx.x * NODE_TM;
#pragma unroll
  for (int r = 0; r < 4; ++r) {
    int row = warp * 4 + r, g = g0 + row;
    float4 hv = make_float4(0, 0, 0, 0), av = hv;
    if (g < n_total) {
      hv = *reinterpret_cast<const float4*>(a.h + (size_t)g * H + lane * 4);
      av = *reinterpret_cast<const float4*>(a.agg + (size_t)g * H + lane * 4);
    }
    *reinterpret_cast<float4*>(hs + row * LDX + lane * 4) = hv;
    *reinterpret_cast<float4*>(as + row * LDX + lane * 4) = av;
  }
  __syncwarp();
  float acc[4][4];
  zero_acc(acc);
  warp_gemm_4x4<H>(hs + warp * 4 * LDX, a.W3_t, lane, acc);
  warp_gemm_4x4<H>(as + warp * 4 * LDX, a.W3_t + (size_t)H * H, lane, acc);
  {
    const float4 bb = __ldg(reinterpret_cast<const float4*>(a.b3 + lane * 4));
#pragma unroll
    for (int r = 0; r < 4; ++r)
      *reinterpret_cast<float4*>(hid + (warp * 4 + r) * LDX + lane * 4) =
          make_float4(act_f<ACT>(acc[r][0] + bb.x), act_f<ACT>(acc[r][1] + bb.y), act_f<ACT>(acc[r][2] + bb.z),
                      act_f<ACT>(acc[r][3] + bb.w));
  }
  __syncwarp();
  zero_acc(acc);
  warp_gemm_4x4<H>(hid + warp * 4 * LDX, a.W4_t, lane, acc);
  {
    const float4 bb = __ldg(reinterpret_cast<const float4*>(a.b4 + lane * 4));
#pragma unroll
    for (int r = 0; r < 4; ++r) {
      int row = warp * 4 + r, g = g0 + row;
      float m = g < n_total ? a.nm[g] : 0.f;
      float4 hv = *reinterpret_cast<const float4*>(hs + row * LDX + lane * 4);
      float4 o = make_float4((hv.x + (acc[r][0] + bb.x)) * m, (hv.y + (acc[r][1] + bb.y)) * m,
                             (hv.z + (acc[r][2] + bb.z)) * m, (hv.w + (acc[r][3] + bb.w)) * m);
      __syncwarp();
      *reinterpret_cast<float4*>(hs + row * LDX + lane * 4) = o;
      if (g < n_total) *reinterpret_cast<float4*>(a.h + (size_t)g * H + lane * 4) = o;
    }
  }
  __syncwarp();
  if (a.AB1 != nullptr) project_ab(hs + warp * 4 * LDX, a.proj1, a.AB1, a.ABmax1, g0, n_total, warp, lane);
  if (a.AB2 != nullptr) project_ab(hs + warp * 4 * LDX, a.proj2, a.AB2, a.ABmax2, g0, n_total, warp, lane);
}

__device__ __forceinline__ float edge_weight(int graph_type, const int8_t* __restrict__ em_mol, int N, int i, int j,
                                             int ci, int cj, float d0) {
  if (graph_type == 0) return em_mol != nullptr ? (float)em_mol[(size_t)i * N + j] : 1.0f;
  if (graph_type == 4)
    return ((em_mol == nullptr || em_mol[(size_t)i * N + j] != 0) && d0 < 6.0f) ? 1.f : 0.f;
  if (i == j || ci == 0 || cj == 0) return 0.f;
  float dist = sqrtf(d0);
  if (graph_type == 1) return dist <= 4.0f ? 1.f : 0.f;
  if (ci == 3 || cj == 3) return 0.f;
  if (ci == 1 && cj == 1) return 1.f;
  if (ci == 2 && cj == 2) return dist <= 4.0f ? 1.f : 0.f;
  float cut = graph_type == 2 ? 4.0f : 10.0f;
  return dist <= cut ? 1.f : 0.f;
}

constexpr int CUT_TN = 128;
constexpr int CUT_MAXR = 28;
constexpr int CUT_REC = 32;

__device__ __forceinline__ void cut_pack_rows(int b, int N, int nrows, const int* __restrict__ rowlist ,
                                              const int* degn, int* srt, int* row_bin, int* row_pos, int* row_start,
                                              int* bin_rem, int* bin_cnt, int* misc, int* __restrict__ recs,
                                              int* __restrict__ n_recs) {
  const int tid = threadIdx.x, lane = tid & 31, warp = tid >> 5;
  if (tid == 0) { misc[0] = 0; misc[1] = 0; }
  __syncthreads();
  for (int s = tid; s < nrows; s += blockDim.x) {
    const int node = rowlist[s], d = degn[node];
    if (d <= CUT_TN) {
      int rank = 0;
      for (int s2 = 0; s2 < nrows; ++s2) {
        const int d2 = degn[rowlist[s2]];
        rank += (d2 <= CUT_TN && (d2 > d || (d2 == d && s2 < s))) ? 1 : 0;
      }
      srt[rank] = node;
      atomicAdd(&misc[0], 1);
    } else {
      row_pos[node] = atomicAdd(&misc[1], 1);
    }
  }
  __syncthreads();
  const int n_light = misc[0], n_heavy = misc[1];
  if (warp == 0) {
    int nb = 0, first_open = 0;
    const int d_min = n_light > 0 ? degn[srt[n_light - 1]] : 0;
    for (int idx = 0; idx < n_light; ++idx) {
      const int node = srt[idx], d = degn[node];
      int found = -1;
      for (int base = first_open; base < nb && found < 0; base += 32) {
        const int bb = base + lane;
        const bool ok = bb < nb && bin_rem[bb] >= d && bin_cnt[bb] < CUT_MAXR;
        const unsigned m = __ballot_sync(0xffffffffu, ok);
        if (m) found = base + __ffs(m) - 1;
      }
      if (lane == 0) {
        if (found < 0) { bin_rem[nb] = CUT_TN; bin_cnt[nb] = 0; }
      }
      if (found < 0) { found = nb; ++nb; }
      __syncwarp();
      if (lane == 0) {
        row_bin[node] = found; row_pos[node] = bin_cnt[found]; row_start[node] = CUT_TN - bin_rem[found];
        bin_rem[found] -= d; bin_cnt[found] += 1;
      }
      __syncwarp();
      while (first_open < nb && (bin_rem[first_open] < d_min || bin_cnt[first_open] >= CUT_MAXR)) ++first_open;
    }
    if (lane == 0) {
      misc[2] = nb;
      misc[3] = atomicAdd(n_recs, nb + n_heavy);
    }
  }
  __syncthreads();
  const int nb = misc[2];
  int* out = recs + (size_t)misc[3] * CUT_REC;
  for (int bb = tid; bb < nb; bb += blockDim.x) {
    int* r = out + (size_t)bb * CUT_REC;
    r[0] = b; r[1] = bin_cnt[bb]; r[2] = CUT_TN - bin_rem[bb]; r[3] = 0;
  }
  for (int s = tid; s < nrows; s += blockDim.x) {
    const int node = rowlist[s], d = degn[node];
    if (d <= CUT_TN) {
      out[(size_t)row_bin[node] * CUT_REC + 4 + row_pos[node]] = node | (row_start[node] << 16);
    } else {
      int* r = out + (size_t)(nb + row_pos[node]) * CUT_REC;
      r[0] = b; r[1] = 1 | (1 << 8); r[2] = d; r[3] = 0; r[4] = node;
    }
  }
  __syncthreads();
}

__global__ void __launch_bounds__(512) k_nbr(int N, int graph_type, const float4* __restrict__ x04,
                                             const int* __restrict__ cls, const int* __restrict__ rowidx,
                                             const int* __restrict__ colidx, const int* __restrict__ xrowidx,
                                             const int* __restrict__ nr, const int* __restrict__ nc,
                                             const int* __restrict__ nxr, int* __restrict__ nbr,
                                             int* __restrict__ recs, int* __restrict__ xrecs,
                                             int* __restrict__ n_recs ) {
  extern __shared__ uint8_t sm_nbr[];
  float4* xs = reinterpret_cast<float4*>(sm_nbr);
  int* cl = reinterpret_cast<int*>(xs + N);
  int* col = cl + N;
  int* degn = col + N;
  int* srt = degn + N;
  int* row_bin = srt + N; int* row_pos = row_bin + N; int* row_start = row_pos + N;
  int* bin_rem = row_start + N; int* bin_cnt = bin_rem + N;
  __shared__ int misc[4];
  const int b = blockIdx.x, tid = threadIdx.x, lane = tid & 31, warp = tid >> 5, nwarp = blockDim.x >> 5;
  const size_t gb = (size_t)b * N;
  const int nrows = nr[b], ncols = nc[b];
  for (int i = tid; i < N; i += blockDim.x) {
    xs[i] = x04[gb + i]; cl[i] = cls[gb + i];
    col[i] = i < ncols ? colidx[gb + i] : 0;
    degn[i] = 0;
  }
  __syncthreads();
  for (int slot = warp; slot < nrows; slot += nwarp) {
    const int i = rowidx[gb + slot];
    const float4 xi = xs[i];
    const int ci = cl[i];
    int* out = nbr + (gb + i) * N;
    int count = 0;
    for (int c0 = 0; c0 < ncols; c0 += 32) {
      const int c = c0 + lane;
      bool keep = false;
      int j = 0;
      if (c < ncols) {
        j = col[c];
        const float4 xj = xs[j];
        const float ex = xi.x - xj.x, ey = xi.y - xj.y, ez = xi.z - xj.z;
        const float d0 = ex * ex + ey * ey + ez * ez;
        keep = edge_weight(graph_type, nullptr, N, i, j, ci, cl[j], d0) != 0.f;
      }
      const unsigned m = __ballot_sync(0xffffffffu, keep);
      if (keep) out[count + __popc(m & ((1u << lane) - 1u))] = j;
      count += __popc(m);
    }
    if (lane == 0) {
      if (count == 0) { out[0] = i | (int)0x80000000; count = 1; }
      degn[i] = count;
    }
  }
  __syncthreads();
  cut_pack_rows(b, N, nrows, rowidx + gb, degn, srt, row_bin, row_pos, row_start, bin_rem, bin_cnt, misc, recs, n_recs);
  cut_pack_rows(b, N, nxr[b], xrowidx + gb, degn, srt, row_bin, row_pos, row_start, bin_rem, bin_cnt, misc, xrecs, n_recs + 1);
}
constexpr int CUT_SMEM_PER_NODE = 16 + 9 * 4;

constexpr int ET = 128;
constexpr int MAXR = 8;
constexpr int LDB = H + 1;

struct EdgeArgs {
  const float* AB;
  const float* ABmax;
  float w2_descale, wdmax, w0max;
  const float* x;
  const float* x0;
  const float4* x4;
  const float4* x04;
  float4* x4_out;
  const int8_t* edge_mask;
  const int* cls;
  const float* nm;
  const float* linker_mask;
  const float* W2_t; const float* b2; const float* wd; const float* w0; const float* w5;
  Plan plan;
  float* agg;
  float* x_out;
  const int* nbr;
  const int* recs;
  const int* n_recs;
};

constexpr size_t EDGE_SIMT_SMEM =
    sizeof(float) * ((size_t)H * H  + (size_t)H * ET  + (size_t)ET * LDB  + (size_t)MAXR * H  +
                     4 * H  + ET  + ET * 3  + ET );

template <bool COORD, int ACT = ACT_SILU>
__global__ void __launch_bounds__(256, 1) k_edge_simt(Geom gm, EdgeArgs a) {
  extern __shared__ __align__(16) float sm_edge[];
  float* W2s = sm_edge;
  float* S1 = W2s + H * H;
  float* Bs = S1 + H * ET;
  float* As = Bs + ET * LDB;
  float* b2s = As + MAXR * H;
  float* wds = b2s + H;
  float* w0s = wds + H;
  float* w5s = w0s + H;
  float* ems = w5s + H;
  float* cds = ems + ET;
  float* phis = cds + ET * 3;
  __shared__ float xacc[COORD ? 1 : 1];
  (void)xacc;

  const int tid = threadIdx.x, lane = tid & 31, warp = tid >> 5;
  const int N = gm.N;
  for (int idx = tid; idx < H * H / 4; idx += 256)
    reinterpret_cast<float4*>(W2s)[idx] = __ldg(reinterpret_cast<const float4*>(a.W2_t) + idx);
  if (tid < H) {
    b2s[tid] = a.b2[tid]; wds[tid] = a.wd[tid]; w0s[tid] = a.w0[tid];
    w5s[tid] = COORD ? a.w5[tid] : 0.f;
  }
  __syncthreads();

  const int n_work = COORD ? *a.plan.n_xmols : *a.plan.n_items;
  for (int wi = blockIdx.x; wi < n_work; wi += gridDim.x) {
    int b, r_begin, r_count;
    if (COORD) { b = a.plan.xmols[wi]; r_begin = 0; r_count = a.plan.nxr[b]; }
    else { int4 it = a.plan.items[wi]; b = it.x; r_begin = it.y; r_count = it.z; }
    const int nc = a.plan.nc[b];
    const int* rows = (COORD ? a.plan.xrowidx : a.plan.rowidx) + (size_t)b * N;
    const int* cols = a.plan.colidx + (size_t)b * N;
    const size_t gb = (size_t)b * N;
    const int8_t* em_mol = a.edge_mask ? a.edge_mask + gb * N : nullptr;
    int per = nc >= ET ? 1 : ET / nc;
    if (per > MAXR) per = MAXR;

    for (int rt = 0; rt < r_count; rt += per) {
      const int nrt = min(per, r_count - rt);
      for (int r = warp; r < nrt; r += 8) {
        int i = rows[r_begin + rt + r];
        *reinterpret_cast<float4*>(As + r * H + lane * 4) =
            *reinterpret_cast<const float4*>(a.AB + (gb + i) * 2 * H + lane * 4);
      }
      float run = 0.f;
      float xrun = 0.f;
      for (int c0 = 0; c0 < nc; c0 += ET) {
        const int ncc = min(ET, nc - c0);
        const int Et = nrt * ncc;
        __syncthreads();
        for (int idx = tid; idx < ncc * H; idx += 256) {
          int jj = idx >> 7, k = idx & (H - 1);
          Bs[jj * LDB + k] = a.AB[(gb + cols[c0 + jj]) * 2 * H + H + k];
        }
        __syncthreads();
        {
          const int e = tid & (ET - 1), kh = tid >> 7;
          const bool valid = e < Et;
          int rr = 0, jj = 0;
          float d = 0.f, d0 = 0.f;
          if (valid) {
            rr = e / ncc; jj = e - rr * ncc;
            const int i = rows[r_begin + rt + rr], j = cols[c0 + jj];
            const float* xi = a.x + (gb + i) * 3; const float* xj = a.x + (gb + j) * 3;
            const float* yi = a.x0 + (gb + i) * 3; const float* yj = a.x0 + (gb + j) * 3;
            float dx = xi[0] - xj[0], dy = xi[1] - xj[1], dz = xi[2] - xj[2];
            d = dx * dx + dy * dy + dz * dz;
            float ex = yi[0] - yj[0], ey = yi[1] - yj[1], ez = yi[2] - yj[2];
            d0 = ex * ex + ey * ey + ez * ez;
            if (kh == 0) {
              int ci = 0, cj = 0;
              if (gm.graph_type >= 1 && gm.graph_type <= 3) { ci = a.cls[gb + i]; cj = a.cls[gb + j]; }
              ems[e] = edge_weight(gm.graph_type, em_mol, N, i, j, ci, cj, d0);
              if (COORD) {
                float inv = 1.0f / (sqrtf(d + 1e-8f) + gm.norm_constant);
                cds[e * 3 + 0] = dx * inv; cds[e * 3 + 1] = dy * inv; cds[e * 3 + 2] = dz * inv;
              }
            }
          } else if (kh == 0) {
            ems[e] = 0.f;
            if (COORD) { cds[e * 3 + 0] = 0.f; cds[e * 3 + 1] = 0.f; cds[e * 3 + 2] = 0.f; }
          }
          const float* Ar = As + rr * H;
          const float* Br = Bs + jj * LDB;
#pragma unroll 8
          for (int kk = 0; kk < H / 2; ++kk) {
            int k = kh * (H / 2) + kk;
            float pre = Ar[k] + Br[k] + d * wds[k] + d0 * w0s[k];
            S1[k * ET + e] = valid ? act_f<ACT>(pre) : 0.f;
          }
        }
        __syncthreads();
        const int ty = tid >> 4, tx = tid & 15;
        float acc[8][8];
#pragma unroll
        for (int p = 0; p < 8; ++p)
#pragma unroll
          for (int q = 0; q < 8; ++q) acc[p][q] = 0.f;
#pragma unroll 4
        for (int k = 0; k < H; ++k) {
          float4 a0 = *reinterpret_cast<const float4*>(S1 + k * ET + ty * 4);
          float4 a1 = *reinterpret_cast<const float4*>(S1 + k * ET + 64 + ty * 4);
          float4 b0 = *reinterpret_cast<const float4*>(W2s + k * H + tx * 4);
          float4 b1 = *reinterpret_cast<const float4*>(W2s + k * H + 64 + tx * 4);
          const float av[8] = {a0.x, a0.y, a0.z, a0.w, a1.x, a1.y, a1.z, a1.w};
          const float bv[8] = {b0.x, b0.y, b0.z, b0.w, b1.x, b1.y, b1.z, b1.w};
#pragma unroll
          for (int p = 0; p < 8; ++p)
#pragma unroll
            for (int q = 0; q < 8; ++q) acc[p][q] = fmaf(av[p], bv[q], acc[p][q]);
        }
        __syncthreads();
        float* Outs = S1;
#pragma unroll
        for (int p = 0; p < 8; ++p) {
          int e = (p < 4 ? ty * 4 + p : 64 + ty * 4 + (p - 4));
          float w = COORD ? 1.f : ems[e];
#pragma unroll
          for (int qh = 0; qh < 2; ++qh) {
            int c = qh * 64 + tx * 4;
            float4 o;
            o.x = act_f<ACT>(acc[p][qh * 4 + 0] + b2s[c + 0]) * w;
            o.y = act_f<ACT>(acc[p][qh * 4 + 1] + b2s[c + 1]) * w;
            o.z = act_f<ACT>(acc[p][qh * 4 + 2] + b2s[c + 2]) * w;
            o.w = act_f<ACT>(acc[p][qh * 4 + 3] + b2s[c + 3]) * w;
            *reinterpret_cast<float4*>(Outs + e * H + c) = o;
          }
        }
        __syncthreads();
        if (!COORD) {
          const int c = tid & (H - 1);
          if (nc <= ET) {
            for (int rr = tid >> 7; rr < nrt; rr += 2) {
              float s = 0.f;
              for (int jj = 0; jj < ncc; ++jj) s += Outs[(rr * ncc + jj) * H + c];
              a.agg[(gb + rows[r_begin + rt + rr]) * H + c] = s / gm.normalization_factor;
            }
          } else if (tid < H) {
            for (int jj = 0; jj < ncc; ++jj) run += Outs[jj * H + c];
            if (c0 + ET >= nc) a.agg[(gb + rows[r_begin + rt]) * H + c] = run / gm.normalization_factor;
          }
        } else {
          for (int e = warp; e < Et; e += 8) {
            float s = 0.f;
#pragma unroll
            for (int q = 0; q < 4; ++q) s = fmaf(Outs[e * H + lane + 32 * q], w5s[lane + 32 * q], s);
#pragma unroll
            for (int o = 16; o > 0; o >>= 1) s += __shfl_xor_sync(0xffffffffu, s, o);
            if (lane == 0) phis[e] = s * ems[e];
          }
          __syncthreads();
          if (tid < nrt * 3) {
            int rr = tid / 3, dim = tid - rr * 3;
            float s = 0.f;
            for (int jj = 0; jj < ncc; ++jj) s += cds[(rr * ncc + jj) * 3 + dim] * phis[rr * ncc + jj];
            xrun += s;
            if (c0 + ET >= nc) {
              int i = rows[r_begin + rt + rr];
              float lm = a.linker_mask ? a.linker_mask[gb + i] : 1.f;
              float xv = a.x[(gb + i) * 3 + dim];
              a.x_out[(gb + i) * 3 + dim] = (xv + (xrun / gm.normalization_factor) * lm) * a.nm[gb + i];
            }
          }
        }
      }
    }
  }
}

__global__ void k_copy_x(int n3, const float* __restrict__ src, float* __restrict__ dst, const float4* __restrict__ src4,
                         float4* __restrict__ dst4) {
  int i = blockIdx.x * blockDim.x + threadIdx.x;
  if (i < n3) dst[i] = src[i];
  if (src4 != nullptr && i * 3 < n3) dst4[i] = src4[i];
}

struct NoiseRng {
  unsigned long long seed, offset;
  unsigned long long per_draw;
  unsigned long long cx;
  int Sx, Sh;
  int F;
  int on;
  int g0;
};
__device__ __forceinline__ float philox_normal_elem(unsigned long long seed, unsigned long long offset, int S, long long e) {
  const long long per_round = 4LL * S;
  const long long rr = e / per_round;
  const int rem = (int)(e - rr * per_round);
  const int ii = rem / S, idx = rem - ii * S;
  curandStatePhilox4_32_10_t st;
  curand_init(seed, (unsigned long long)idx, offset + 4ULL * (unsigned long long)rr, &st);
  const float4 v = curand_normal4(&st);
  return ii == 0 ? v.x : ii == 1 ? v.y : ii == 2 ? v.z : v.w;
}
__device__ __forceinline__ float noise_draw(const NoiseRng& q, int r, int g, int d) {
  const unsigned long long base = q.offset + (unsigned long long)r * q.per_draw;
  const long long gg = (long long)g + q.g0;
  if (d < 3) return philox_normal_elem(q.seed, base, q.Sx, gg * 3 + d);
  return philox_normal_elem(q.seed, base + q.cx, q.Sh, gg * q.F + (d - 3));
}

struct FinishArgs {
  const float* h;
  const float* x;
  const float* x0;
  const float* nm;
  const float* Wo;
  const float* bo;
  float* out;
  int* nan_flags;
  float* z;
  const float* fragment_mask; const float* linker_mask;
  const float* noise;
  NoiseRng rng;
  const float* coef;
  const int* step_fin; int* step_prep;
  int T;
  float norm0, norm1, bias1;
  float* chain;
  const int* tag_step;
};

__global__ void __launch_bounds__(256) k_finish(Geom gm, FinishArgs a) {
  const int tid = threadIdx.x;
  const int d = tid & 15, r = tid >> 4;
  const int n_total = gm.B * gm.N;
  const int g = blockIdx.x * 16 + r;
  const int xd = 3 + gm.F;
  const bool act = g < n_total && d < xd;
  __shared__ __align__(16) float hs[16][H + 4];
  __shared__ float ws[H][16];
  for (int idx = tid; idx < 16 * H; idx += 256) {
    const int j = idx / H, k = idx - j * H;
    ws[k][j] = j < gm.F ? __ldg(a.Wo + (size_t)j * H + k) : 0.f;
  }
  chain_wait();
  chain_release();
  int step = 0;
  if (a.z != nullptr) {
    step = *a.step_fin;
    if (blockIdx.x == 0 && tid == 0) *a.step_prep = step + 1;
  } else if (a.tag_step != nullptr) {
    step = *a.tag_step;
  }
  for (int idx = tid; idx < 16 * (H / 4); idx += 256) {
    const int rr = idx / (H / 4), k4 = idx - rr * (H / 4);
    const int gg = blockIdx.x * 16 + rr;
    const float4 v = gg < n_total ? *reinterpret_cast<const float4*>(a.h + (size_t)gg * H + k4 * 4) : make_float4(0.f, 0.f, 0.f, 0.f);
    *reinterpret_cast<float4*>(&hs[rr][k4 * 4]) = v;
  }
  __syncthreads();
  float e = 0.f;
  if (act) {
    float m = a.nm[g];
    if (d < 3) {
      e = (a.x[(size_t)g * 3 + d] - a.x0[(size_t)g * 3 + d]) * m;
    } else {
      const int j = d - 3;
      float s = 0.f;
#pragma unroll 8
      for (int k = 0; k < H; k += 4) {
        const float4 hv = *reinterpret_cast<const float4*>(&hs[r][k]);
        s = fmaf(hv.x, ws[k][j], s); s = fmaf(hv.y, ws[k + 1][j], s); s = fmaf(hv.z, ws[k + 2][j], s); s = fmaf(hv.w, ws[k + 3][j], s);
      }
      e = (s + a.bo[j]) * m;
    }
    if (e != e && a.nan_flags != nullptr) {
      const int bits = d < 3 ? 1 : 2;
      const int tag = ((a.z != nullptr || a.tag_step != nullptr) ? step + 1 : 0) << 8;
      int* p = a.nan_flags + g / gm.N;
      const int old = atomicCAS(p, 0, bits | tag);
      if (old != 0 && (old & ~0xff) == tag) atomicOr(p, bits);
    }
    if (a.out != nullptr) a.out[(size_t)g * xd + d] = e;
  }
  if (a.z == nullptr) return;

  const float* cf = a.coef + (size_t)step * 8;
  const float ca = cf[1], cb = cf[2], cc = cf[3];
  const int frame = __float_as_int(cf[4]);
  float znew = 0.f;
  float lm = 0.f, fm = 0.f;
  if (act) {
    lm = a.linker_mask[g]; fm = a.fragment_mask[g];
    const float zt = a.z[(size_t)g * xd + d];
    const float eps = e * lm;
    const float nz = (a.rng.on ? noise_draw(a.rng, step + 1, g, d)
                               : a.noise[((size_t)(step + 1) * n_total + g) * xd + d]) * lm;
    if (step < a.T) {
      float mu = zt / ca - cb * eps;
      float zs = mu + cc * nz;
      znew = zt * fm + zs * lm;
      a.z[(size_t)g * xd + d] = znew;
      if (frame >= 0) {
        float o = d < 3 ? znew * a.norm0 : znew * a.norm1 + a.bias1;
        a.chain[((size_t)frame * n_total + g) * xd + d] = o;
      }
    } else {
      float mux = ca * (zt - cb * eps);
      float xo = mux + cc * nz;
      znew = zt * fm + xo * lm;
    }
  }
  if (step >= a.T) {
    float hv = (act && d >= 3) ? znew * a.norm1 + a.bias1 : -INFINITY;
    int best = d;
    float bv = hv;
    const unsigned gmask = 0xffffffffu;
#pragma unroll
    for (int o = 8; o > 0; o >>= 1) {
      float ov = __shfl_xor_sync(gmask, bv, o, 16);
      int oi = __shfl_xor_sync(gmask, best, o, 16);
      if (ov > bv || (ov == bv && oi < best)) { bv = ov; best = oi; }
    }
    if (act) {
      float o = d < 3 ? znew * a.norm0 : ((d == best ? 1.f : 0.f) * a.nm[g]);
      a.chain[(size_t)g * xd + d] = o;
    }
  }
}

struct InpaintArgs {
  int mode;
  float* eps;
  const float* nm;
  float* z;
  const float* xh0;
  const float* fragment_mask; const float* linker_mask;
  const float* noise;
  const float* coef;
  int* step_prep; const int* step_fin;
  int T;
  float norm0, norm1, bias1;
  float* chain;
};

__device__ __forceinline__ float block_sum_256(float v, float* red) {
#pragma unroll
  for (int o = 16; o > 0; o >>= 1) v += __shfl_xor_sync(0xffffffffu, v, o);
  __syncthreads();
  if ((threadIdx.x & 31) == 0) red[threadIdx.x >> 5] = v;
  __syncthreads();
  float s = 0.f;
#pragma unroll
  for (int w = 0; w < 8; ++w) s += red[w];
  return s;
}

__global__ void __launch_bounds__(256) k_inpaint(Geom gm, InpaintArgs a) {
  __shared__ float red[8];
  __shared__ float means[4];
  const int b = blockIdx.x, tid = threadIdx.x, N = gm.N, xd = 3 + gm.F;
  const size_t g0 = (size_t)b * N;
  int step = 0;
  if (a.mode == 1) step = *a.step_fin;
  float cnt = 0.f, sx = 0.f, sy = 0.f, sz = 0.f;
  for (int n = tid; n < N; n += 256) {
    const float m = a.nm[g0 + n];
    cnt += m;
    sx += a.eps[(g0 + n) * xd + 0]; sy += a.eps[(g0 + n) * xd + 1]; sz += a.eps[(g0 + n) * xd + 2];
  }
  cnt = block_sum_256(cnt, red);
  sx = block_sum_256(sx, red); sy = block_sum_256(sy, red); sz = block_sum_256(sz, red);
  const float mvx = sx / cnt, mvy = sy / cnt, mvz = sz / cnt;
  if (a.mode == 0) {
    for (int n = tid; n < N; n += 256) {
      const float m = a.nm[g0 + n];
      a.eps[(g0 + n) * xd + 0] -= mvx * m; a.eps[(g0 + n) * xd + 1] -= mvy * m; a.eps[(g0 + n) * xd + 2] -= mvz * m;
    }
    return;
  }
  const float* cf = a.coef + (size_t)step * 8;
  const float ca = cf[1], cb = cf[2], cc = cf[3], qa = cf[5], qb = cf[6];
  const int frame = __float_as_int(cf[4]);
  const size_t slab = (size_t)gm.B * N * xd;
  const float* nA = a.noise + (size_t)(1 + 2 * step) * slab;
  const float* nB = nA + slab;
  if (step < a.T) {
    float cx = 0.f, cy = 0.f, cz = 0.f;
    for (int idx = tid; idx < N * xd; idx += 256) {
      const int n = idx / xd, d = idx - n * xd;
      const float m = a.nm[g0 + n], lm = a.linker_mask[g0 + n], fm = a.fragment_mask[g0 + n];
      const size_t gi = (g0 + n) * xd + d;
      float e = a.eps[gi];
      if (d < 3) e -= (d == 0 ? mvx : d == 1 ? mvy : mvz) * m;
      const float zt = a.z[gi];
      const float zl = (zt / ca - cb * e) + cc * nA[gi];
      const float zf = (qa * zt + qb * (a.xh0[gi] * fm)) + cc * nB[gi];
      const float zn = zl * lm + zf * fm;
      a.z[gi] = zn;
      if (d == 0) cx += zn; else if (d == 1) cy += zn; else if (d == 2) cz += zn;
    }
    cx = block_sum_256(cx, red); cy = block_sum_256(cy, red); cz = block_sum_256(cz, red);
    if (tid == 0) { means[0] = cx / cnt; means[1] = cy / cnt; means[2] = cz / cnt; }
    __syncthreads();
    for (int idx = tid; idx < N * xd; idx += 256) {
      const int n = idx / xd, d = idx - n * xd;
      const size_t gi = (g0 + n) * xd + d;
      float zn = a.z[gi];
      if (d < 3) { zn -= means[d] * a.nm[g0 + n]; a.z[gi] = zn; }
      if (frame >= 0) a.chain[(size_t)frame * slab + gi] = d < 3 ? zn * a.norm0 : zn * a.norm1 + a.bias1;
    }
  } else {
    for (int n = tid; n < N; n += 256) {
      const float m = a.nm[g0 + n], lm = a.linker_mask[g0 + n], fm = a.fragment_mask[g0 + n];
      int bl = 0, bf = 0;
      float vl = -INFINITY, vf = -INFINITY;
      for (int d = 0; d < xd; ++d) {
        const size_t gi = (g0 + n) * xd + d;
        float e = a.eps[gi];
        if (d < 3) e -= (d == 0 ? mvx : d == 1 ? mvy : mvz) * m;
        const float zt = a.z[gi];
        const float xl = ca * (zt - cb * e) + cc * nA[gi];
        const float xf = ca * zt - qa * nB[gi];
        if (d < 3) {
          a.chain[gi] = (xl * a.norm0) * lm + (xf * a.norm0) * fm;
        } else {
          const float hl = xl * a.norm1 + a.bias1, hf = xf * a.norm1 + a.bias1;
          if (hl > vl) { vl = hl; bl = d; }
          if (hf > vf) { vf = hf; bf = d; }
        }
      }
      for (int d = 3; d < xd; ++d)
        a.chain[(g0 + n) * xd + d] = ((d == bl ? 1.f : 0.f) * m) * lm + ((d == bf ? 1.f : 0.f) * m) * fm;
    }
  }
  if (tid == 0 && b == 0) *a.step_prep = step + 1;
}

__global__ void k_init_z(int n_total, int xd, const float* __restrict__ xh, const float* __restrict__ fm,
                         const float* __restrict__ lm, const float* __restrict__ noise, NoiseRng rng, float* __restrict__ z) {
  int idx = blockIdx.x * blockDim.x + threadIdx.x;
  if (idx >= n_total * xd) return;
  int g = idx / xd;
  float l = lm[g];
  const float nz = rng.on ? noise_draw(rng, 0, g, idx - g * xd) : noise[idx];
  z[idx] = xh[idx] * fm[g] + (nz * l) * l;
}

__global__ void k_noise_fill(int n_draws, int n_total, int xd, NoiseRng rng, float* __restrict__ out) {
  const long long total = (long long)n_draws * n_total * xd;
  for (long long i = (long long)blockIdx.x * blockDim.x + threadIdx.x; i < total; i += (long long)gridDim.x * blockDim.x) {
    const int d = (int)(i % xd);
    const long long gi = i / xd;
    out[i] = noise_draw(rng, (int)(gi / n_total), (int)(gi % n_total), d);
  }
}

constexpr int SZ_MAX_OUT = 64;
__global__ void __launch_bounds__(256) k_sz_out(int N, int out_nf, const float* __restrict__ h, const float* __restrict__ Wo,
                                               const float* __restrict__ bo, float* __restrict__ out) {
  __shared__ float part[8][SZ_MAX_OUT];
  const int b = blockIdx.x, tid = threadIdx.x, lane = tid & 31, warp = tid >> 5;
  for (int o = lane; o < out_nf; o += 32) part[warp][o] = 0.f;
  __syncwarp();
  for (int n = warp; n < N; n += 8) {
    const float4 hv = *reinterpret_cast<const float4*>(h + ((size_t)b * N + n) * H + lane * 4);
    for (int o = 0; o < out_nf; ++o) {
      const float4 w = __ldg(reinterpret_cast<const float4*>(Wo + (size_t)o * H + lane * 4));
      float s = hv.x * w.x + hv.y * w.y + hv.z * w.z + hv.w * w.w;
#pragma unroll
      for (int k = 16; k > 0; k >>= 1) s += __shfl_xor_sync(0xffffffffu, s, k);
      if (lane == 0) part[warp][o] += s + bo[o];
    }
  }
  __syncthreads();
  if (tid < out_nf) {
    float s = 0.f;
    for (int w = 0; w < 8; ++w) s += part[w][tid];
    out[(size_t)b * out_nf + tid] = s / (float)N;
  }
}


}
```

difflinker_b200/csrc/kernels_tc.cuh:

```cuda
#pragma once
#include <cuda_fp16.h>

#include <cmath>
#include <cstdio>
#include <type_traits>
#include <vector>

#include "../../include/difflinker_b200.h"
#include "kernels_simt.cuh"

namespace dl {
namespace tc {

constexpr bool AVAILABLE = true;
constexpr int TN = 128;
constexpr int MAXR = 32;
constexpr int KC = 16;
constexpr int W_LBO = H * 16;
constexpr int B_LBO = TN * 16 + 16;
constexpr int SBO = 128;
constexpr int W_BYTES = KC * W_LBO;
constexpr int B_BYTES = KC * B_LBO;
constexpr float F16_TARGET = 16384.0f;

constexpr int N_STAGE = 2;
constexpr int N_ACC = 4;

constexpr int W_EPI = 0;
constexpr int N_EPI_WARPS = 8;
constexpr int W_LOAD = 8;
constexpr int W_TBL = 9;
constexpr int N_TBL_WARPS = 3;
constexpr int W_PROD = 12;
constexpr int N_PROD_WARPS = 8;
constexpr int EDGE_TC_THREADS = 32 * (W_PROD + N_PROD_WARPS);
constexpr int REGS_EPI = 112, REGS_CTRL = 64;
constexpr int BAR_TURN0 = 3, BAR_TURN1 = 4;

constexpr int OFF_WHI = 0;
constexpr int OFF_WLO = OFF_WHI + W_BYTES;
constexpr int OFF_ST = OFF_WLO + W_BYTES;
constexpr int STAGE_BYTES = 2 * B_BYTES;
constexpr int OFF_TBL = OFF_ST + N_STAGE * STAGE_BYTES;
constexpr int TBL_HDR = 0;
constexpr int TBL_ROWOFF = 64;
constexpr int TBL_COLOFF = TBL_ROWOFF + TN * 4;
constexpr int TBL_D = TBL_COLOFF + TN * 4;
constexpr int TBL_D0 = TBL_D + TN * 4;
constexpr int TBL_SC = TBL_D0 + TN * 4;
constexpr int TBL_EM = TBL_SC + TN * 4;
constexpr int TBL_CD = TBL_EM + TN * 8;
constexpr int TBL_ROWNODE = TBL_CD + TN * 12;
constexpr int TBL_ROWSTART = TBL_ROWNODE + MAXR * 4;
constexpr int TBL_BYTES = TBL_ROWSTART + (MAXR + 4) * 4;
constexpr int OFF_B2W5 = OFF_TBL + N_ACC * TBL_BYTES;
constexpr int OFF_TX = OFF_B2W5 + H * 8;
constexpr int OFF_BAR = OFF_TX + TN * 12;
constexpr int BAR_W = 0, BAR_FULL = 8, BAR_EMPTY = BAR_FULL + 8 * N_STAGE, BAR_TBL = BAR_EMPTY + 8 * N_STAGE,
              BAR_TEMPTY = BAR_TBL + 8 * N_ACC, BAR_END = BAR_TEMPTY + 8 * N_ACC;
constexpr int SMEM_BYTES = OFF_BAR + BAR_END + 1024;
static_assert(SMEM_BYTES <= 232448, "k_edge_tc exceeds the 227 KB of shared memory a CTA can opt into");
static_assert(TBL_BYTES % 16 == 0, "table slots must keep 16-byte alignment");

__device__ __forceinline__ uint32_t smem_u32(const void* p) { return (uint32_t)__cvta_generic_to_shared(p); }

__device__ __forceinline__ void mbar_init(uint32_t bar, uint32_t count) {
  asm volatile("mbarrier.init.shared::cta.b64 [%0], %1;" ::"r"(bar), "r"(count));
}
__device__ __forceinline__ void mbar_expect_tx(uint32_t bar, uint32_t bytes) {
  asm volatile("mbarrier.arrive.expect_tx.shared::cta.b64 _, [%0], %1;" ::"r"(bar), "r"(bytes) : "memory");
}
__device__ __constant__ int c_wait_mode = 1;
constexpr uint32_t WAIT_HINT_NS = 20000;
__device__ __forceinline__ void mbar_wait(uint32_t bar, uint32_t parity) {
  uint32_t done = 0;
  const int mode = c_wait_mode;
  if (mode == 1) {
    for (uint32_t spin = 0; spin < (1u << 20); ++spin) {
      asm volatile(
          "{\n\t.reg .pred p;\n\t"
          "mbarrier.try_wait.parity.shared::cta.b64 p, [%1], %2, %3;\n\t"
          "selp.u32 %0, 1, 0, p;\n\t}"
          : "=r"(done)
          : "r"(bar), "r"(parity), "r"(WAIT_HINT_NS)
          : "memory");
      if (done) return;
    }
    __trap();
  }
  for (uint32_t spin = 0; spin < (1u << 28); ++spin) {
    asm volatile(
        "{\n\t.reg .pred p;\n\t"
        "mbarrier.try_wait.parity.shared::cta.b64 p, [%1], %2;\n\t"
        "selp.u32 %0, 1, 0, p;\n\t}"
        : "=r"(done)
        : "r"(bar), "r"(parity)
        : "memory");
    if (done) return;
    if (mode == 2) __nanosleep(32);
  }
  __trap();
}
__device__ __forceinline__ void mbar_arrive(uint32_t bar) {
  asm volatile("mbarrier.arrive.shared::cta.b64 _, [%0];" ::"r"(bar) : "memory");
}
__device__ __forceinline__ void named_sync(int id, int nthreads) {
  asm volatile("bar.sync %0, %1;" ::"r"(id), "r"(nthreads) : "memory");
}
__device__ __forceinline__ void named_arrive(int id, int nthreads) {
  asm volatile("bar.arrive %0, %1;" ::"r"(id), "r"(nthreads) : "memory");
}
__device__ __forceinline__ void mbar_wait_relaxed(uint32_t bar, uint32_t parity) {
  uint32_t done = 0;
  for (uint32_t spin = 0; spin < (1u << 24); ++spin) {
    asm volatile(
        "{\n\t.reg .pred p;\n\t"
        "mbarrier.try_wait.parity.shared::cta.b64 p, [%1], %2;\n\t"
        "selp.u32 %0, 1, 0, p;\n\t}"
        : "=r"(done)
        : "r"(bar), "r"(parity)
        : "memory");
    if (done) return;
    __nanosleep(64);
  }
  __trap();
}
__device__ __forceinline__ void fence_barrier_init() { asm volatile("fence.mbarrier_init.release.cluster;" ::: "memory"); }
__device__ __forceinline__ void fence_proxy_async() { asm volatile("fence.proxy.async.shared::cta;" ::: "memory"); }

__device__ __forceinline__ void bulk_g2s(uint32_t dst, const void* src, uint32_t bytes, uint32_t bar) {
  asm volatile("cp.async.bulk.shared::cluster.global.mbarrier::complete_tx::bytes [%0], [%1], %2, [%3];" ::"r"(dst),
               "l"(src), "r"(bytes), "r"(bar)
               : "memory");
}

__device__ __forceinline__ uint64_t wg_desc(uint32_t saddr, uint32_t lbo, uint32_t sbo) {
  return (uint64_t)((saddr & 0x3FFFFu) >> 4) | ((uint64_t)(lbo >> 4) << 16) | ((uint64_t)(sbo >> 4) << 32);
}
__device__ __forceinline__ void wg_fence() { asm volatile("wgmma.fence.sync.aligned;" ::: "memory"); }
__device__ __forceinline__ void wg_commit() { asm volatile("wgmma.commit_group.sync.aligned;" ::: "memory"); }
__device__ __forceinline__ void wg_wait_all() { asm volatile("wgmma.wait_group.sync.aligned 0;" ::: "memory"); }
__device__ __forceinline__ void fence_acc(float (&d)[64]) {
#pragma unroll
  for (int i = 0; i < 64; ++i) asm volatile("" : "+f"(d[i])::"memory");
}
template <int TRANS_B>
__device__ __forceinline__ void wgmma_m64n128k16(float (&d)[64], uint64_t adesc, uint64_t bdesc, uint32_t accumulate) {
  asm volatile(
      "{\n\t.reg .pred p;\n\t"
      "setp.ne.b32 p, %66, 0;\n\t"
      "wgmma.mma_async.sync.aligned.m64n128k16.f32.f16.f16 "
      "{%0, %1, %2, %3, %4, %5, %6, %7, %8, %9, %10, %11, %12, %13, %14, %15, %16, %17, %18, %19, %20, %21, %22, %23, %24, %25, %26, %27, %28, %29, %30, %31, %32, %33, %34, %35, %36, %37, %38, %39, %40, %41, %42, %43, %44, %45, %46, %47, %48, %49, %50, %51, %52, %53, %54, %55, %56, %57, %58, %59, %60, %61, %62, %63}, %64, %65, p, 1, 1, 0, %67;\n\t}"
      : "+f"(d[0]), "+f"(d[1]), "+f"(d[2]), "+f"(d[3]), "+f"(d[4]), "+f"(d[5]), "+f"(d[6]), "+f"(d[7]), "+f"(d[8]), "+f"(d[9]), "+f"(d[10]), "+f"(d[11]), "+f"(d[12]), "+f"(d[13]), "+f"(d[14]), "+f"(d[15]), "+f"(d[16]), "+f"(d[17]), "+f"(d[18]), "+f"(d[19]), "+f"(d[20]), "+f"(d[21]), "+f"(d[22]), "+f"(d[23]), "+f"(d[24]), "+f"(d[25]), "+f"(d[26]), "+f"(d[27]), "+f"(d[28]), "+f"(d[29]), "+f"(d[30]), "+f"(d[31]), "+f"(d[32]), "+f"(d[33]), "+f"(d[34]), "+f"(d[35]), "+f"(d[36]), "+f"(d[37]), "+f"(d[38]), "+f"(d[39]), "+f"(d[40]), "+f"(d[41]), "+f"(d[42]), "+f"(d[43]), "+f"(d[44]), "+f"(d[45]), "+f"(d[46]), "+f"(d[47]), "+f"(d[48]), "+f"(d[49]), "+f"(d[50]), "+f"(d[51]), "+f"(d[52]), "+f"(d[53]), "+f"(d[54]), "+f"(d[55]), "+f"(d[56]), "+f"(d[57]), "+f"(d[58]), "+f"(d[59]), "+f"(d[60]), "+f"(d[61]), "+f"(d[62]), "+f"(d[63])
      : "l"(adesc), "l"(bdesc), "r"(accumulate), "n"(TRANS_B));
}
template <int TRANS_B = 0>
__device__ __forceinline__ void mma_3xf16(float (&d)[64], uint32_t a_hi, uint32_t a_lo, uint32_t a_lbo, uint32_t b_hi,
                                          uint32_t b_lo, uint32_t b_lbo, uint32_t b_ks_stride, int nks, bool accumulate) {
#pragma unroll
  for (int ks = 0; ks < nks; ++ks) {
    const uint64_t ah = wg_desc(a_hi + ks * 2 * a_lbo, a_lbo, SBO), al = wg_desc(a_lo + ks * 2 * a_lbo, a_lbo, SBO);
    const uint64_t bh = wg_desc(b_hi + ks * b_ks_stride, b_lbo, SBO), bl = wg_desc(b_lo + ks * b_ks_stride, b_lbo, SBO);
    wgmma_m64n128k16<TRANS_B>(d, al, bh, (accumulate || ks > 0) ? 1u : 0u);
    wgmma_m64n128k16<TRANS_B>(d, ah, bl, 1u);
    wgmma_m64n128k16<TRANS_B>(d, ah, bh, 1u);
  }
}
template <int TRANS_B = 0>
__device__ __forceinline__ void gemm_3xf16(float (&d)[64], uint32_t a_hi, uint32_t a_lo, uint32_t a_lbo, uint32_t b_hi,
                                           uint32_t b_lo, uint32_t b_lbo, uint32_t b_ks_stride, int nks, bool accumulate) {
  fence_acc(d);
  wg_fence();
  mma_3xf16<TRANS_B>(d, a_hi, a_lo, a_lbo, b_hi, b_lo, b_lbo, b_ks_stride, nks, accumulate);
  wg_commit();
  wg_wait_all();
  fence_acc(d);
}

__device__ __forceinline__ void split2v(float2 v, uint32_t& hi, uint32_t& lo) {
  __half2 h = __float22half2_rn(v);
  float2 back = __half22float2(h);
  __half2 l = __float22half2_rn(fadd2(v, make_float2(-back.x, -back.y)));
  hi = *reinterpret_cast<uint32_t*>(&h);
  lo = *reinterpret_cast<uint32_t*>(&l);
}
__device__ __forceinline__ void split2(float a, float b, uint32_t& hi, uint32_t& lo) {
  __half2 h = __floats2half2_rn(a, b);
  float2 back = __half22float2(h);
  __half2 l = __floats2half2_rn(a - back.x, b - back.y);
  hi = *reinterpret_cast<uint32_t*>(&h);
  lo = *reinterpret_cast<uint32_t*>(&l);
}
__device__ __forceinline__ int gcl_row_of_edge(int e) { return 8 * ((e & 31) >> 1) + 2 * (e >> 5) + (e & 1); }
struct Tile {
  int b, nc, slot0, nrt, c0, ncc;
  bool first_chunk, last_chunk;
  const int* rows;
  int Et;
  int start;
  int node;
};

template <bool COORD>
struct TileIter {
  const int4* list;
  const int* rowlist;
  int N, wi_end, wi, rt, c0, cache_base, lane;
  int4 cache;
  __device__ TileIter(const Plan& p, int N_) : N(N_), rt(0), c0(0), cache_base(-(1 << 30)), lane(threadIdx.x & 31) {
    list = COORD ? p.xitems : p.items;
    rowlist = COORD ? p.xrowidx : p.rowidx;
    const int total = COORD ? *p.n_xitems : *p.n_items;
    const int per = total / (int)gridDim.x, extra = total % (int)gridDim.x, c = (int)blockIdx.x;
    wi = c * per + min(c, extra);
    wi_end = wi + per + (c < extra ? 1 : 0);
    cache = make_int4(0, 0, 0, 0);
  }
  __device__ bool next(Tile& t) {
    while (wi < wi_end) {
      if (wi - cache_base >= 32) {
        cache_base = wi;
        cache = list[min(wi + lane, wi_end - 1)];
      }
      const int src = wi - cache_base;
      const int b = __shfl_sync(0xffffffffu, cache.x, src), r_begin = __shfl_sync(0xffffffffu, cache.y, src);
      const int r_count = __shfl_sync(0xffffffffu, cache.z, src), nc = __shfl_sync(0xffffffffu, cache.w, src);
      int per = nc >= TN ? 1 : TN / max(nc, 1);
      if (per > MAXR) per = MAXR;
      if (rt >= r_count || nc <= 0) { wi += 1; rt = 0; c0 = 0; continue; }
      t.b = b; t.nc = nc; t.slot0 = r_begin + rt; t.nrt = min(per, r_count - rt);
      t.c0 = c0; t.ncc = min(TN, nc - c0);
      t.first_chunk = c0 == 0; t.last_chunk = c0 + TN >= nc;
      t.rows = rowlist + (size_t)b * N;
      c0 += TN;
      if (c0 >= nc) { c0 = 0; rt += per; }
      return true;
    }
    return false;
  }
};

struct RecIter {
  const int* recs;
  int n, k, G, lane, cur, nxt, chunk;
  __device__ RecIter(const int* recs_, const int* n_recs) : recs(recs_), lane(threadIdx.x & 31), cur(0), chunk(0) {
    n = *n_recs; G = (int)gridDim.x; k = (int)blockIdx.x;
    nxt = k < n ? recs[(size_t)k * CUT_REC + lane] : 0;
  }
  __device__ bool next(Tile& t) {
    if (chunk == 0) {
      if (k >= n) return false;
      cur = nxt;
      const int kn = k + G;
      nxt = kn < n ? recs[(size_t)kn * CUT_REC + lane] : 0;
    }
    const int w1 = __shfl_sync(0xffffffffu, cur, 1), v2 = __shfl_sync(0xffffffffu, cur, 2);
    const int info = __shfl_sync(0xffffffffu, cur, (4 + lane) & 31);
    t.b = __shfl_sync(0xffffffffu, cur, 0);
    t.nc = 0; t.slot0 = 0; t.rows = nullptr;
    if (((w1 >> 8) & 1) == 0) {
      t.nrt = w1 & 0xff; t.Et = v2; t.ncc = v2; t.c0 = 0; t.first_chunk = true; t.last_chunk = true;
      t.node = info & 0xffff; t.start = info >> 16;
      k += G;
    } else {
      const int deg = v2, c0 = chunk * TN;
      t.nrt = 1; t.Et = min(TN, deg - c0); t.ncc = t.Et; t.c0 = c0;
      t.first_chunk = chunk == 0; t.last_chunk = c0 + TN >= deg;
      t.node = __shfl_sync(0xffffffffu, cur, 4) & 0xffff;
      t.start = lane == 0 ? 0 : t.Et;
      ++chunk;
      if (t.last_chunk) { chunk = 0; k += G; }
    }
    return true;
  }
};

template <bool COORD, bool SPARSE>
__device__ __forceinline__ typename std::conditional<SPARSE, RecIter, TileIter<COORD>>::type make_iter(const EdgeArgs& a, int N) {
  if constexpr (SPARSE) return RecIter(a.recs, a.n_recs);
  else return TileIter<COORD>(a.plan, N);
}

template <bool COORD, bool SPARSE = false>
__global__ void __launch_bounds__(EDGE_TC_THREADS, 1) k_edge_tc(Geom gm, EdgeArgs a, const __half* __restrict__ w2tc) {
  extern __shared__ uint8_t smem_raw[];
  uint8_t* sm = smem_raw + ((1024u - (smem_u32(smem_raw) & 1023u)) & 1023u);
  const uint32_t sbase = smem_u32(sm);
  const int tid = threadIdx.x, lane = tid & 31, warp = tid >> 5;
  const int N = gm.N;

  const uint32_t bars = sbase + OFF_BAR;
  float2* b2w5 = reinterpret_cast<float2*>(sm + OFF_B2W5);

  if (tid == 0) {
    mbar_init(bars + BAR_W, 1);
    for (int i = 0; i < N_STAGE; ++i) { mbar_init(bars + BAR_FULL + 8 * i, N_PROD_WARPS); mbar_init(bars + BAR_EMPTY + 8 * i, N_EPI_WARPS); }
    for (int i = 0; i < N_ACC; ++i) {
      mbar_init(bars + BAR_TBL + 8 * i, 1);
      mbar_init(bars + BAR_TEMPTY + 8 * i, N_EPI_WARPS);
    }
    fence_barrier_init();
  }
  if (tid < H) b2w5[tid] = make_float2(a.b2[tid], COORD ? a.w5[tid] : 0.f);
  __syncthreads();

  if (warp >= W_LOAD && warp < W_PROD) {
    asm volatile("setmaxnreg.dec.sync.aligned.u32 %0;" ::"n"(REGS_CTRL));
  if (warp >= W_TBL && warp < W_TBL + N_TBL_WARPS) {
    const int tw = warp - W_TBL;
    typename std::conditional<SPARSE, RecIter, TileIter<COORD>>::type iter = make_iter<COORD, SPARSE>(a, N);
    Tile cur;
    for (int t = 0;; ++t) {
      const int acc = t & (N_ACC - 1);
      const bool more = iter.next(cur);
      if (t % N_TBL_WARPS != tw) { if (!more) break; continue; }
      if (t >= N_ACC) mbar_wait_relaxed(bars + BAR_TEMPTY + 8 * acc, ((t - N_ACC) / N_ACC) & 1);
      uint8_t* tb = sm + OFF_TBL + acc * TBL_BYTES;
      int* hdr = reinterpret_cast<int*>(tb + TBL_HDR);
      if (more) {
        const int Et = SPARSE ? cur.Et : cur.nrt * cur.ncc;
        const size_t gb = (size_t)cur.b * N;
        if (lane == 0) {
          hdr[0] = Et; hdr[1] = cur.nrt; hdr[2] = cur.ncc;
          hdr[3] = (cur.first_chunk ? 1 : 0) | (cur.last_chunk ? 2 : 0);
          hdr[4] = cur.b;
        }
        if (SPARSE) {
          if (lane < cur.nrt) {
            reinterpret_cast<int*>(tb + TBL_ROWNODE)[lane] = cur.node;
            reinterpret_cast<int*>(tb + TBL_ROWSTART)[lane] = cur.start;
          }
          if (lane == 0) reinterpret_cast<int*>(tb + TBL_ROWSTART)[cur.nrt] = Et;
        } else {
          if (lane < cur.nrt) {
            reinterpret_cast<int*>(tb + TBL_ROWNODE)[lane] = cur.rows[cur.slot0 + lane];
            reinterpret_cast<int*>(tb + TBL_ROWSTART)[lane] = lane * cur.ncc;
          }
          if (lane == 0) reinterpret_cast<int*>(tb + TBL_ROWSTART)[cur.nrt] = Et;
        }
        bool any_rescale = false;
#pragma unroll
        for (int e = lane; e < TN; e += 32) {
          const int ev = min(e, Et - 1);
          int i, j;
          float ew_list = 1.f;
          if (SPARSE) {
            int rr = 0;
            for (int r = 1; r < cur.nrt; ++r) rr += ev >= __shfl_sync(0xffffffffu, cur.start, r) ? 1 : 0;
            i = __shfl_sync(0xffffffffu, cur.node, rr);
            const int first_col = __shfl_sync(0xffffffffu, cur.start, rr);
            const int raw = a.nbr[(gb + i) * N + cur.c0 + (ev - first_col)];
            j = raw & 0x7fffffff;
            ew_list = raw < 0 ? 0.f : 1.f;
          } else {
            const int rr = ev / cur.ncc, jj = ev - rr * cur.ncc;
            i = cur.rows[cur.slot0 + rr];
            j = a.plan.colidx[gb + cur.c0 + jj];
          }
          const float4 xi = a.x4[gb + i], xj = a.x4[gb + j], yi = a.x04[gb + i], yj = a.x04[gb + j];
          const float dx = xi.x - xj.x, dy = xi.y - xj.y, dz = xi.z - xj.z;
          const float d = dx * dx + dy * dy + dz * dz;
          const float ex = yi.x - yj.x, ey = yi.y - yj.y, ez = yi.z - yj.z;
          const float d0 = ex * ex + ey * ey + ez * ez;
          int ci = 0, cj = 0;
          if (!SPARSE && gm.graph_type != 0) { ci = a.cls[gb + i]; cj = a.cls[gb + j]; }
          reinterpret_cast<int*>(tb + TBL_ROWOFF)[e] = (int)((gb + i) * 2 * H);
          reinterpret_cast<int*>(tb + TBL_COLOFF)[e] = (int)((gb + j) * 2 * H + H);
          reinterpret_cast<float*>(tb + TBL_D)[e] = d;
          reinterpret_cast<float*>(tb + TBL_D0)[e] = d0;
          const float bound = a.ABmax[(gb + i) * 2] + a.ABmax[(gb + j) * 2 + 1] + d * a.wdmax + d0 * a.w0max;
          float sc = 1.0f;
          if (!(bound <= F16_TARGET)) {
            const int ex2 = ((__float_as_int(bound) >> 23) & 0xff) - 127;
            sc = __int_as_float(max(127 + 13 - ex2, 1) << 23);
          }
          reinterpret_cast<float*>(tb + TBL_SC)[e] = sc;
          any_rescale |= (sc != 1.0f);
          const float ew = SPARSE ? ew_list
                                  : edge_weight(gm.graph_type, a.edge_mask ? a.edge_mask + gb * N : nullptr, N, i, j, ci, cj, d0);
          reinterpret_cast<float2*>(tb + TBL_EM)[e] =
              COORD ? make_float2(ew, a.w2_descale / sc)
                    : make_float2(ew * -0.6931471805599453f, (a.w2_descale / sc) * -1.4426950408889634f);
          if (COORD) {
            const float inv = 1.0f / (sqrtf(d + 1e-8f) + gm.norm_constant);
            float* cds = reinterpret_cast<float*>(tb + TBL_CD);
            cds[e * 3 + 0] = dx * inv; cds[e * 3 + 1] = dy * inv; cds[e * 3 + 2] = dz * inv;
          }
        }
        any_rescale = __any_sync(0xffffffffu, any_rescale);
        if (lane == 0) hdr[5] = any_rescale ? 1 : 0;
      } else if (lane == 0) {
        hdr[0] = 0;
      }
      __syncwarp();
      if (lane == 0) mbar_arrive(bars + BAR_TBL + 8 * acc);
      if (!more) break;
    }
  } else if (warp == W_LOAD) {
    if (lane == 0) {
      mbar_expect_tx(bars + BAR_W, 2 * W_BYTES);
      bulk_g2s(sbase + OFF_WHI, w2tc, 2 * W_BYTES, bars + BAR_W);
    }
  }
  } else if (warp >= W_PROD) {
    const int pw = warp - W_PROD;
    const int kc = lane & 15, esub = lane >> 4;
    float2 wdr[4], w0r[4];
#pragma unroll
    for (int q = 0; q < 4; ++q) {
      wdr[q] = make_float2(__ldg(a.wd + kc * 8 + 2 * q), __ldg(a.wd + kc * 8 + 2 * q + 1));
      w0r[q] = make_float2(__ldg(a.w0 + kc * 8 + 2 * q), __ldg(a.w0 + kc * 8 + 2 * q + 1));
    }
    for (int t = 0;; ++t) {
      const int acc = t & (N_ACC - 1), s = t & (N_STAGE - 1);
      mbar_wait(bars + BAR_TBL + 8 * acc, (t / N_ACC) & 1);
      const uint8_t* tb = sm + OFF_TBL + acc * TBL_BYTES;
      const int Et = reinterpret_cast<const int*>(tb + TBL_HDR)[0];
      if (t >= N_STAGE) mbar_wait(bars + BAR_EMPTY + 8 * s, ((t - N_STAGE) / N_STAGE) & 1);
      if (Et > 0) {
        const int* rowoff = reinterpret_cast<const int*>(tb + TBL_ROWOFF);
        const int* coloff = reinterpret_cast<const int*>(tb + TBL_COLOFF);
        const float* dv = reinterpret_cast<const float*>(tb + TBL_D);
        const float* d0v = reinterpret_cast<const float*>(tb + TBL_D0);
        const float* scv = reinterpret_cast<const float*>(tb + TBL_SC);
        uint8_t* bhi = sm + OFF_ST + s * STAGE_BYTES + kc * B_LBO;
        uint8_t* blo = bhi + B_BYTES;
        const bool rescale = reinterpret_cast<const int*>(tb + TBL_HDR)[5] != 0;
        constexpr int ITEMS = TN / (2 * N_PROD_WARPS);
        float4 pa0, pa1, pb[2][2];
        const int e_base = ITEMS * (2 * pw + esub);
        int ro_cur = rowoff[e_base];
        {
          const float* ap = a.AB + ro_cur + kc * 8;
          pa0 = __ldg(reinterpret_cast<const float4*>(ap)); pa1 = __ldg(reinterpret_cast<const float4*>(ap + 4));
        }
#pragma unroll
        for (int pf = 0; pf < 2; ++pf) {
          const float* bp = a.AB + coloff[e_base + pf] + kc * 8;
          pb[pf][0] = __ldg(reinterpret_cast<const float4*>(bp)); pb[pf][1] = __ldg(reinterpret_cast<const float4*>(bp + 4));
        }
#pragma unroll
        for (int it = 0; it < ITEMS; ++it) {
          const int e = e_base + it;
          const int slot = it & 1;
          const float4 b0 = pb[slot][0], b1 = pb[slot][1];
          if (it + 2 < ITEMS) {
            const float* bp = a.AB + coloff[e + 2] + kc * 8;
            pb[slot][0] = __ldg(reinterpret_cast<const float4*>(bp)); pb[slot][1] = __ldg(reinterpret_cast<const float4*>(bp + 4));
          }
          const int ro = rowoff[e];
          if (ro != ro_cur) {
            ro_cur = ro;
            const float* ap = a.AB + ro + kc * 8;
            pa0 = __ldg(reinterpret_cast<const float4*>(ap)); pa1 = __ldg(reinterpret_cast<const float4*>(ap + 4));
          }
          const float4 a0 = pa0, a1 = pa1;
          if (e < Et) {
            const float d = dv[e], d0 = d0v[e];
            const float2 dd = make_float2(d, d), dd0 = make_float2(d0, d0);
            const float2 av[4] = {make_float2(a0.x, a0.y), make_float2(a0.z, a0.w), make_float2(a1.x, a1.y), make_float2(a1.z, a1.w)};
            const float2 bv[4] = {make_float2(b0.x, b0.y), make_float2(b0.z, b0.w), make_float2(b1.x, b1.y), make_float2(b1.z, b1.w)};
            float2 sv[4];
#pragma unroll
            for (int q = 0; q < 4; ++q)
              sv[q] = usig2(ffma2(dd0, w0r[q], ffma2(dd, wdr[q], fadd2(av[q], bv[q]))));
            if (rescale) {
              const float sc = scv[e];
#pragma unroll
              for (int q = 0; q < 4; ++q) sv[q] = fmul2(sv[q], make_float2(sc, sc));
            }
            uint4 hi, lo;
            split2v(sv[0], hi.x, lo.x); split2v(sv[1], hi.y, lo.y);
            split2v(sv[2], hi.z, lo.z); split2v(sv[3], hi.w, lo.w);
            const int row = COORD ? e : gcl_row_of_edge(e);
            *reinterpret_cast<uint4*>(bhi + row * 16) = hi;
            *reinterpret_cast<uint4*>(blo + row * 16) = lo;
          }
        }
        fence_proxy_async();
      }
      __syncwarp();
      if (lane == 0) mbar_arrive(bars + BAR_FULL + 8 * s);
      if (Et <= 0) break;
    }
  } else {
    asm volatile("setmaxnreg.inc.sync.aligned.u32 %0;" ::"n"(REGS_EPI));
    const int g = warp >> 2;
    const int wq = warp & 3, q = lane & 3;
    const int r0 = 64 * g + 16 * wq + (lane >> 2);
    float* txs = reinterpret_cast<float*>(sm + OFF_TX);
    float2 run = make_float2(0.f, 0.f);
    float run3 = 0.f;
    float d[64];
#pragma unroll
    for (int i = 0; i < 64; ++i) d[i] = 0.f;
    mbar_wait(bars + BAR_W, 0);
    for (int t = 0;; ++t) {
      const int acc = t & (N_ACC - 1), s = t & (N_STAGE - 1);
      if (!COORD && g == 0 && t > 0) named_sync(BAR_TURN0, 32 * N_EPI_WARPS);
      mbar_wait(bars + BAR_TBL + 8 * acc, (t / N_ACC) & 1);
      const uint8_t* tb = sm + OFF_TBL + acc * TBL_BYTES;
      const int* hdr = reinterpret_cast<const int*>(tb + TBL_HDR);
      const int Et = hdr[0];
      if (Et <= 0) break;
      const uint32_t bhi = sbase + OFF_ST + s * STAGE_BYTES, blo = bhi + B_BYTES;
      if (!COORD) {
        if (g == 1) named_sync(BAR_TURN1, 32 * N_EPI_WARPS);
        mbar_wait(bars + BAR_FULL + 8 * s, (t / N_STAGE) & 1);
        fence_acc(d);
        wg_fence();
        mma_3xf16(d, sbase + OFF_WHI + g * 1024, sbase + OFF_WLO + g * 1024, W_LBO, bhi, blo, B_LBO, 2 * B_LBO, 8, false);
        wg_commit();
        named_arrive(g == 0 ? BAR_TURN1 : BAR_TURN0, 32 * N_EPI_WARPS);
        wg_wait_all();
        fence_acc(d);
      } else {
        mbar_wait(bars + BAR_FULL + 8 * s, (t / N_STAGE) & 1);
        gemm_3xf16(d, bhi + g * 1024, blo + g * 1024, B_LBO, sbase + OFF_WHI, sbase + OFF_WLO, W_LBO, 2 * W_LBO, 8, false);
      }
      __syncwarp();
      if (lane == 0) mbar_arrive(bars + BAR_EMPTY + 8 * s);

      const int nrt = hdr[1];
      const bool first_chunk = hdr[3] & 1, last_chunk = hdr[3] & 2;
      const size_t gb = (size_t)hdr[4] * N;
      const float2* emds = reinterpret_cast<const float2*>(tb + TBL_EM);
      const int* rownode = reinterpret_cast<const int*>(tb + TBL_ROWNODE);
      const int* rowstart = reinterpret_cast<const int*>(tb + TBL_ROWSTART);
      if (!COORD) {
        const float2 bias = make_float2(b2w5[r0].x * -1.4426950408889634f, b2w5[r0 + 8].x * -1.4426950408889634f);
        const float inv_norm = 1.0f / gm.normalization_factor;
        const int E0 = 32 * q;
        const bool has = E0 < Et;
        int cur = 0;
        if (has) { while (rowstart[cur + 1] <= E0) ++cur; }
        const int hrow = cur;
        uint32_t bmask = 0;
        int nr = cur + 1;
        if (has) { for (; nr <= nrt && rowstart[nr] < E0 + 32; ++nr) bmask |= 1u << (rowstart[nr] - E0); }
        const bool open_end = has && nr <= nrt && rowstart[nr] > E0 + 32;
        const bool cut = Et < E0 + 32;
        const uint32_t wmask = __reduce_or_sync(0xffffffffu, bmask);
        float2 hsum = make_float2(0.f, 0.f), sum = make_float2(0.f, 0.f);
        bool in_head = true;
#pragma unroll
        for (int tt = 0; tt < 32; ++tt) {
          if (wmask & (1u << tt)) {
            const bool here = (bmask >> tt) & 1u;
            if (here && !in_head) {
              float* dst = a.agg + (gb + rownode[cur]) * H;
              dst[r0] = sum.x * inv_norm; dst[r0 + 8] = sum.y * inv_norm;
            }
            hsum = here && in_head ? sum : hsum;
            sum = here ? make_float2(0.f, 0.f) : sum;
            in_head = in_head && !here;
            cur += here ? 1 : 0;
          }
          const float2 ed = emds[E0 + tt];
          const float2 u = ffma2(make_float2(d[(tt >> 1) * 4 + (tt & 1)], d[(tt >> 1) * 4 + 2 + (tt & 1)]),
                                 make_float2(ed.y, ed.y), bias);
          const float2 v = fmul2(usig2(u), make_float2(ed.x, ed.x));
          sum = fadd2(sum, v);
        }
        if (in_head) hsum = sum;
        const float2 lsum = sum;
        const bool cont_in = has && rowstart[hrow] < E0;
        float2 cin = (q == 0 && nrt == 1 && !first_chunk) ? run : make_float2(0.f, 0.f);
#pragma unroll
        for (int k = 0; k < 3; ++k) {
          const float2 cout = in_head ? fadd2(cin, hsum) : lsum;
          const float px = __shfl_up_sync(0xffffffffu, cout.x, 1, 4), py = __shfl_up_sync(0xffffffffu, cout.y, 1, 4);
          if (q == k + 1 && cont_in) cin = make_float2(px, py);
        }
        const float2 htot = fadd2(cin, hsum);
        if (nrt == 1) {
          const int src = (lane & ~3) | ((Et - 1) >> 5);
          run = make_float2(__shfl_sync(0xffffffffu, htot.x, src), __shfl_sync(0xffffffffu, htot.y, src));
        }
        if (has && last_chunk) {
          if (!in_head || !open_end) {
            float* dst = a.agg + (gb + rownode[hrow]) * H;
            dst[r0] = htot.x * inv_norm; dst[r0 + 8] = htot.y * inv_norm;
          }
          if (!in_head && !open_end && !cut) {
            float* dst = a.agg + (gb + rownode[cur]) * H;
            dst[r0] = lsum.x * inv_norm; dst[r0 + 8] = lsum.y * inv_norm;
          }
        }
        __syncwarp();
        if (lane == 0) mbar_arrive(bars + BAR_TEMPTY + 8 * acc);
      } else {
        const float2 eda = emds[min(r0, Et - 1)], edb = emds[min(r0 + 8, Et - 1)];
        float2 pa = make_float2(0.f, 0.f), pb = make_float2(0.f, 0.f);
#pragma unroll
        for (int j = 0; j < 16; ++j) {
          const float2 w0 = b2w5[8 * j + 2 * q], w1 = b2w5[8 * j + 2 * q + 1];
          const float2 va = ffma2(make_float2(d[4 * j], d[4 * j + 1]), make_float2(eda.y, eda.y), make_float2(w0.x, w1.x));
          const float2 vb = ffma2(make_float2(d[4 * j + 2], d[4 * j + 3]), make_float2(edb.y, edb.y), make_float2(w0.x, w1.x));
          pa = ffma2(silu2(va), make_float2(w0.y, w1.y), pa);
          pb = ffma2(silu2(vb), make_float2(w0.y, w1.y), pb);
        }
        float phia = pa.x + pa.y, phib = pb.x + pb.y;
        phia += __shfl_xor_sync(0xffffffffu, phia, 1); phib += __shfl_xor_sync(0xffffffffu, phib, 1);
        phia += __shfl_xor_sync(0xffffffffu, phia, 2); phib += __shfl_xor_sync(0xffffffffu, phib, 2);
        const float* cds = reinterpret_cast<const float*>(tb + TBL_CD);
        if (q == 0 && r0 < Et) {
          const float w = phia * eda.x;
          txs[r0 * 3 + 0] = cds[r0 * 3 + 0] * w; txs[r0 * 3 + 1] = cds[r0 * 3 + 1] * w; txs[r0 * 3 + 2] = cds[r0 * 3 + 2] * w;
        }
        if (q == 0 && r0 + 8 < Et) {
          const int e = r0 + 8;
          const float w = phib * edb.x;
          txs[e * 3 + 0] = cds[e * 3 + 0] * w; txs[e * 3 + 1] = cds[e * 3 + 1] * w; txs[e * 3 + 2] = cds[e * 3 + 2] * w;
        }
        named_sync(2, 32 * N_EPI_WARPS);
        if (tid < nrt * 3) {
          const int rr = tid / 3, dim = tid - rr * 3;
          float sacc = (nrt == 1 && !first_chunk) ? run3 : 0.f;
          const int col0 = rowstart[rr];
          const int ncc = rowstart[rr + 1] - col0;
          for (int jj = 0; jj < ncc; ++jj) sacc += txs[(col0 + jj) * 3 + dim];
          if (nrt == 1) run3 = sacc;
          if (last_chunk) {
            const int i = rownode[rr];
            const float lm = a.linker_mask ? a.linker_mask[gb + i] : 1.f;
            const float xv = a.x[(gb + i) * 3 + dim];
            const float xn = (xv + (sacc / gm.normalization_factor) * lm) * a.nm[gb + i];
            a.x_out[(gb + i) * 3 + dim] = xn;
            reinterpret_cast<float*>(a.x4_out + gb + i)[dim] = xn;
          }
        }
        named_sync(2, 32 * N_EPI_WARPS);
        if (lane == 0) mbar_arrive(bars + BAR_TEMPTY + 8 * acc);
      }
    }
  }
}

template <typename K>
inline bool opt_in_smem(K kern) {
  return cudaFuncSetAttribute(kern, cudaFuncAttributeMaxDynamicSharedMemorySize, SMEM_BYTES) == cudaSuccess;
}
inline dl_status configure() {
  const bool ok = opt_in_smem(k_edge_tc<true, false>) && opt_in_smem(k_edge_tc<true, true>) &&
                  opt_in_smem(k_edge_tc<false, false>) && opt_in_smem(k_edge_tc<false, true>);
  return ok ? DL_OK : DL_ERR_CUDA;
}

constexpr double NEG_LN2 = -0.6931471805599453094;
constexpr double NEG_LOG2E = -1.4426950408889634074;

inline size_t pack_w2(const std::vector<float>& W_in, std::vector<__half>& blob, float* descale) {
  std::vector<float> W(W_in.size());
  for (size_t i = 0; i < W.size(); ++i) W[i] = (float)((double)W_in[i] * NEG_LN2);
  while (blob.size() % 64) blob.push_back(__float2half(0.f));
  const size_t off = blob.size();
  blob.resize(off + 2 * (size_t)KC * H * 8);
  float mx = 0.f;
  for (float v : W) mx = std::max(mx, std::fabs(v));
  int ex = 0;
  if (mx > 0.f && std::isfinite(mx)) { std::frexp(mx, &ex); ex -= 1; }
  const int sh = std::min(std::max(13 - ex, -40), 40);
  const float scale = std::ldexp(1.0f, sh);
  *descale = std::ldexp(1.0f, -sh);
  for (int kc = 0; kc < KC; ++kc)
    for (int c = 0; c < H; ++c)
      for (int u = 0; u < 8; ++u) {
        const float v = W[(size_t)c * H + kc * 8 + u] * scale;
        const __half hi = __float2half_rn(v);
        const __half lo = __float2half_rn(v - __half2float(hi));
        blob[off + ((size_t)kc * H + c) * 8 + u] = hi;
        blob[off + (size_t)KC * H * 8 + ((size_t)kc * H + c) * 8 + u] = lo;
      }
  return off;
}

inline dl_status launch_edge_tc(const Geom& gm, const EdgeArgs& ea, bool coord, const void* w2_tc, int num_sms,
                                cudaStream_t st) {
  const __half* w = reinterpret_cast<const __half*>(w2_tc);
  if (ea.recs != nullptr) {
    if (coord) k_edge_tc<true, true><<<num_sms, EDGE_TC_THREADS, SMEM_BYTES, st>>>(gm, ea, w);
    else k_edge_tc<false, true><<<num_sms, EDGE_TC_THREADS, SMEM_BYTES, st>>>(gm, ea, w);
  } else if (coord) k_edge_tc<true, false><<<num_sms, EDGE_TC_THREADS, SMEM_BYTES, st>>>(gm, ea, w);
  else k_edge_tc<false, false><<<num_sms, EDGE_TC_THREADS, SMEM_BYTES, st>>>(gm, ea, w);
  return DL_OK;
}

constexpr int PN = 256;
constexpr int P_LBO = PN * 16 + 16;
constexpr int P_OFF_BHI = 2 * W_BYTES, P_OFF_BLO = P_OFF_BHI + KC * P_LBO;
constexpr int P_SMEM_BYTES = P_OFF_BLO + KC * P_LBO + 1024;
template <bool B_MN>
__global__ void __launch_bounds__(256, 1) k_wgmma_probe(const __half* __restrict__ A ,
                                                        const __half* __restrict__ Bm ,
                                                        float* __restrict__ D ) {
  extern __shared__ uint8_t smem_raw[];
  uint8_t* sm = smem_raw + ((1024u - (smem_u32(smem_raw) & 1023u)) & 1023u);
  const uint32_t sbase = smem_u32(sm);
  const int tid = threadIdx.x, lane = tid & 31, warp = tid >> 5;
  for (int idx = tid; idx < 2 * KC * H; idx += 256) {
    const int copy = idx / (KC * H), rem = idx % (KC * H), kcx = rem / H, row = rem % H;
    *reinterpret_cast<uint4*>(sm + (copy ? OFF_WLO : OFF_WHI) + kcx * W_LBO + row * 16) =
        *reinterpret_cast<const uint4*>(A + (size_t)idx * 8);
  }
  constexpr int MN_LBO = (PN / 8) * 128;
  for (int idx = tid; idx < 2 * KC * PN; idx += 256) {
    const int copy = idx / (KC * PN), rem = idx % (KC * PN), kcx = rem / PN, row = rem % PN;
    if (!B_MN) {
      *reinterpret_cast<uint4*>(sm + (copy ? P_OFF_BLO : P_OFF_BHI) + kcx * P_LBO + row * 16) =
          *reinterpret_cast<const uint4*>(Bm + (size_t)idx * 8);
    } else {
      for (int u = 0; u < 8; ++u)
        *reinterpret_cast<__half*>(sm + (copy ? P_OFF_BLO : P_OFF_BHI) + kcx * MN_LBO + (row >> 3) * 128 + u * 16 + (row & 7) * 2) =
            Bm[(size_t)idx * 8 + u];
    }
  }
  fence_proxy_async();
  __syncthreads();
  const int g = warp >> 2;
  const int r0 = 64 * g + 16 * (warp & 3) + (lane >> 2), q = lane & 3;
  float d[64];
  for (int nh = 0; nh < 2; ++nh) {
    const uint32_t bhi = sbase + P_OFF_BHI + nh * (B_MN ? 16 * 128 : 128 * 16), blo = bhi + (P_OFF_BLO - P_OFF_BHI);
    if (B_MN)
      gemm_3xf16<1>(d, sbase + OFF_WHI + g * 1024, sbase + OFF_WLO + g * 1024, W_LBO, bhi, blo, MN_LBO, 2 * MN_LBO, 8, false);
    else
      gemm_3xf16<0>(d, sbase + OFF_WHI + g * 1024, sbase + OFF_WLO + g * 1024, W_LBO, bhi, blo, P_LBO, 2 * P_LBO, 8, false);
#pragma unroll
    for (int j = 0; j < 16; ++j) {
      const int col = nh * 128 + 8 * j + 2 * q;
      D[(size_t)r0 * PN + col] = d[4 * j]; D[(size_t)r0 * PN + col + 1] = d[4 * j + 1];
      D[(size_t)(r0 + 8) * PN + col] = d[4 * j + 2]; D[(size_t)(r0 + 8) * PN + col + 1] = d[4 * j + 3];
    }
  }
}

inline dl_status selftest(int , float* max_abs_err, float* max_rel_err, bool b_mn_major = false) {
  std::vector<float> A((size_t)H * H), Bv((size_t)PN * H);
  uint32_t s = 12345u;
  auto rnd = [&]() { s = s * 1664525u + 1013904223u; return ((s >> 8) & 0xFFFF) / 65536.0f - 0.5f; };
  for (auto& v : A) v = rnd() * 0.2f;
  for (auto& v : Bv) v = rnd() * 3.0f;
  auto pack = [&](const std::vector<float>& M, int rows) {
    std::vector<__half> out(2 * (size_t)KC * rows * 8);
    for (int kc = 0; kc < KC; ++kc)
      for (int r = 0; r < rows; ++r)
        for (int u = 0; u < 8; ++u) {
          const float v = M[(size_t)r * H + kc * 8 + u];
          const __half hi = __float2half_rn(v);
          out[((size_t)kc * rows + r) * 8 + u] = hi;
          out[(size_t)KC * rows * 8 + ((size_t)kc * rows + r) * 8 + u] = __float2half_rn(v - __half2float(hi));
        }
    return out;
  };
  std::vector<__half> Ap = pack(A, H), Bp = pack(Bv, PN);
  __half *dA = nullptr, *dB = nullptr;
  float* dD = nullptr;
  if (cudaMalloc(&dA, Ap.size() * 2) != cudaSuccess || cudaMalloc(&dB, Bp.size() * 2) != cudaSuccess ||
      cudaMalloc(&dD, (size_t)H * PN * 4) != cudaSuccess)
    return DL_ERR_CUDA;
  cudaMemcpy(dA, Ap.data(), Ap.size() * 2, cudaMemcpyHostToDevice);
  cudaMemcpy(dB, Bp.data(), Bp.size() * 2, cudaMemcpyHostToDevice);
  cudaMemset(dD, 0, (size_t)H * PN * 4);
  if (b_mn_major) {
    cudaFuncSetAttribute(k_wgmma_probe<true>, cudaFuncAttributeMaxDynamicSharedMemorySize, P_SMEM_BYTES);
    k_wgmma_probe<true><<<1, 256, P_SMEM_BYTES>>>(dA, dB, dD);
  } else {
    cudaFuncSetAttribute(k_wgmma_probe<false>, cudaFuncAttributeMaxDynamicSharedMemorySize, P_SMEM_BYTES);
    k_wgmma_probe<false><<<1, 256, P_SMEM_BYTES>>>(dA, dB, dD);
  }
  cudaError_t err = cudaDeviceSynchronize();
  std::vector<float> D((size_t)H * PN);
  cudaMemcpy(D.data(), dD, D.size() * 4, cudaMemcpyDeviceToHost);
  cudaFree(dA); cudaFree(dB); cudaFree(dD);
  if (err != cudaSuccess) {
    fprintf(stderr, "[dl selftest] k_wgmma_probe failed: %s\n", cudaGetErrorString(err));
    return DL_ERR_CUDA;
  }
  double ma = 0, mr = 0, mref = 0;
  for (int m = 0; m < H; ++m)
    for (int n = 0; n < PN; ++n) {
      double ref = 0;
      for (int k = 0; k < H; ++k) ref += (double)A[(size_t)m * H + k] * (double)Bv[(size_t)n * H + k];
      ma = std::max(ma, std::fabs(ref - (double)D[(size_t)m * PN + n]));
      mref = std::max(mref, std::fabs(ref));
    }
  mr = ma / std::max(mref, 1e-30);
  if (max_abs_err) *max_abs_err = (float)ma;
  if (max_rel_err) *max_rel_err = (float)mr;
  fprintf(stderr, "[dl selftest] 3xFP16 wgmma 128x256x128 (B %s-major): max abs err %.3e (rel to max |ref| %.3e)\n",
          b_mn_major ? "MN" : "K", ma, mr);
  return DL_OK;
}

}
}
```

include/difflinker_b200.h:

```cpp
#ifndef DIFFLINKER_B200_H_
#define DIFFLINKER_B200_H_

#include <stdint.h>

#ifdef __cplusplus
extern "C" {
#endif

typedef struct dl_engine dl_engine;

typedef enum dl_status {
  DL_OK = 0,
  DL_NAN_DETECTED = 1,
  DL_ERR_INVALID = -1,
  DL_ERR_CUDA = -2,
  DL_ERR_WEIGHTS = -3,
  DL_ERR_UNSUPPORTED = -4
} dl_status;

enum { DL_GRAPH_FC = 0, DL_GRAPH_4A = 1, DL_GRAPH_FC_4A = 2, DL_GRAPH_FC_10A_4A = 3 };
enum { DL_EDGE_AUTO = 0, DL_EDGE_SIMT = 1, DL_EDGE_WGMMA = 2 };
enum { DL_SAMPLER_LINKER = 0, DL_SAMPLER_INPAINT = 1 };

typedef struct dl_config {
  int32_t n_dims;
  int32_t in_node_nf;
  int32_t context_node_nf;
  int32_t hidden_nf;
  int32_t n_layers;
  int32_t inv_sublayers;
  int32_t condition_time;
  int32_t centering;
  int32_t graph_type;
  int32_t device;
  int32_t edge_impl;
  float norm_constant;
  float normalization_factor;
} dl_config;

typedef struct dl_step_coef {
  float t;
  float a;
  float b;
  float c;
  int32_t frame;
  float qa;
  float qb;
  float pad;
} dl_step_coef;

const char* dl_version(void);
const char* dl_last_error(void);

dl_status dl_create(const dl_config* cfg, dl_engine** out);
dl_status dl_destroy(dl_engine* e);

dl_status dl_set_weight(dl_engine* e, const char* name, const float* data, int64_t numel);
dl_status dl_finalize_weights(dl_engine* e);
int64_t dl_expected_param_count(const dl_engine* e);

dl_status dl_dynamics_forward(dl_engine* e, int32_t B, int32_t N, const float* t, int32_t t_numel, const float* xh,
                              const int8_t* node_mask, const float* linker_mask, const int8_t* edge_mask,
                              const float* context, float* out, int32_t* nan_flags, void* stream);

dl_status dl_dynamics_forward_host(dl_engine* e, int32_t B, int32_t N, const float* t, int32_t t_numel,
                                   const float* xh, const int8_t* node_mask, const float* linker_mask,
                                   const int8_t* edge_mask, const float* context, float* out, int32_t* nan_flags);

dl_status dl_sample_chain(dl_engine* e, int32_t sampler, int32_t B, int32_t N, int32_t T, int32_t keep_frames,
                          const float* xh, const int8_t* node_mask, const float* fragment_mask,
                          const float* linker_mask, const int8_t* edge_mask, const float* context,
                          const float* noise, const dl_step_coef* coef, const float* norm, float* chain,
                          int32_t* nan_flags, void* stream);

dl_status dl_sample_chain_rng(dl_engine* e, int32_t sampler, int32_t B, int32_t N, int32_t T, int32_t keep_frames,
                              const float* xh, const int8_t* node_mask, const float* fragment_mask,
                              const float* linker_mask, const int8_t* edge_mask, const float* context, uint64_t seed,
                              uint64_t offset, uint64_t* offset_consumed, const dl_step_coef* coef, const float* norm,
                              float* chain, int32_t* nan_flags, void* stream);
dl_status dl_set_noise_slice(dl_engine* e, int32_t B_full, int32_t b0);
dl_status dl_noise_fill(dl_engine* e, int32_t n_draws, int32_t B, int32_t N, uint64_t seed, uint64_t offset, float* out,
                        uint64_t* offset_consumed, void* stream);

dl_status dl_sample_chain_host(dl_engine* e, int32_t sampler, int32_t B, int32_t N, int32_t T, int32_t keep_frames,
                               const float* xh, const int8_t* node_mask, const float* fragment_mask,
                               const float* linker_mask, const int8_t* edge_mask, const float* context,
                               const float* noise, const dl_step_coef* coef, const float* norm, float* chain,
                               int32_t* nan_flags);

int64_t dl_launch_count(const dl_engine* e);
float dl_last_elapsed_ms(dl_engine* e);
float dl_time_edge_kernel(dl_engine* e, int32_t reps);
dl_status dl_cut_graph_stats(dl_engine* e, int64_t* out);
dl_status dl_selftest_tc(dl_engine* e, float* max_abs_err, float* max_rel_err);
dl_status dl_selftest_tc_layout(dl_engine* e, int32_t b_mn_major, float* max_abs_err, float* max_rel_err);

dl_status dl_restore_frame(int32_t B, int32_t N, int32_t row_stride, float* xh, const float* positions,
                           const float* com_mask, const int8_t* node_mask, void* stream);
dl_status dl_restore_frame2(int32_t B, int32_t N, int32_t N_pos, int32_t row_stride, float* xh, const float* positions,
                            const float* com_mask, const int8_t* node_mask, void* stream);

int64_t dl_format_xyz(int32_t B, int32_t N, int32_t F, const float* positions, int32_t pos_row_stride,
                      const float* one_hot, int32_t oh_row_stride, const int8_t* node_mask,
                      const char* const* symbols, int32_t n_symbols, char* out, int64_t out_cap, int64_t* offsets);

dl_status dl_bond_orders(int32_t B, int32_t N, int32_t n_types, const float* x, int32_t x_row_stride,
                         const int32_t* atom_types, const int8_t* node_mask, const float* thr1, const float* thr2,
                         const float* thr3, int8_t* E, void* stream);

typedef struct dl_sizegnn dl_sizegnn;
typedef struct dl_sizegnn_config {
  int32_t in_node_nf;
  int32_t hidden_nf;
  int32_t out_node_nf;
  int32_t n_layers;
  int32_t device;
} dl_sizegnn_config;
dl_status dl_sizegnn_create(const dl_sizegnn_config* cfg, dl_sizegnn** out);
dl_status dl_sizegnn_destroy(dl_sizegnn* e);
dl_status dl_sizegnn_set_weight(dl_sizegnn* e, const char* name, const float* host_data, int64_t numel);
dl_status dl_sizegnn_finalize_weights(dl_sizegnn* e);
dl_status dl_sizegnn_forward(dl_sizegnn* e, int32_t B, int32_t N, const float* xh, const int8_t* fragment_mask,
                             const int8_t* edge_mask, float* out, void* stream);

#ifdef __cplusplus
}
#endif
#endif
```

Before: 166.1.

## Pack edge tiles as flat segments across rows with balanced per-CTA ranges

For the tensor-core non-coordinate edge path, the planner now picks rows per item to minimise tile padding. It also assigns items to CTAs with a min-max tile-count partition (cta_begin). A new SegIter walks each item as a flat edge range, so a tile can span row boundaries. The epilogue carries running sums across chunks for this, and the activation/gating pass is hoisted into a vectorised loop before the segmented sum. An optional compile-time profiling build is added. The intent is less padding waste and better load balance across SMs, at the cost of more complex row-crossing reduction logic and a serial single-thread planner loop.

```diff
diff --git a/difflinker_b200/_native.py b/difflinker_b200/_native.py
--- a/difflinker_b200/_native.py
+++ b/difflinker_b200/_native.py
@@ -50,6 +50,7 @@
     "dl_selftest_tc": (_I32, [_P, C.POINTER(_F), C.POINTER(_F)]),
     "dl_selftest_tc_layout": (_I32, [_P, _I32, C.POINTER(_F), C.POINTER(_F)]),
     "dl_cut_graph_stats": (_I32, [_P, C.POINTER(_I64)]),
+    "dl_edge_prof": (_I32, [_I32, C.POINTER(_I64)]),
     "dl_sizegnn_create": (_I32, [C.POINTER(DLSizeGNNConfig), C.POINTER(_P)]),
     "dl_sizegnn_destroy": (_I32, [_P]),
     "dl_sizegnn_set_weight": (_I32, [_P, C.c_char_p, _P, _I64]),
diff --git a/difflinker_b200/build.py b/difflinker_b200/build.py
--- a/difflinker_b200/build.py
+++ b/difflinker_b200/build.py
@@ -6,6 +6,7 @@
 PKG_DIR = os.path.dirname(os.path.abspath(__file__))
 CSRC = os.path.join(PKG_DIR, "csrc")
 LIB_PATH = os.path.join(PKG_DIR, "libdifflinker_b200.so")
+PROF_LIB_PATH = os.path.join(PKG_DIR, "libdifflinker_b200_prof.so")
 SOURCES = ["dl_engine.cu", "output_stage.cu"]
 HEADERS = ["common.cuh", "size_gnn.cuh", "kernels_simt.cuh", "kernels_tc.cuh", "kernels_node_tc.cuh", os.path.join("..", "..", "include", "difflinker_b200.h")]
 
@@ -17,10 +18,10 @@
     return None
 
 
-def is_stale() -> bool:
-    if not os.path.isfile(LIB_PATH):
+def is_stale(lib_path: str = LIB_PATH) -> bool:
+    if not os.path.isfile(lib_path):
         return True
-    t = os.path.getmtime(LIB_PATH)
+    t = os.path.getmtime(lib_path)
     for f in SOURCES + HEADERS:
         p = os.path.join(CSRC, f)
         if os.path.isfile(p) and os.path.getmtime(p) > t:
@@ -28,14 +29,16 @@
     return False
 
 
-def build_native(force: bool = False, verbose: bool = False) -> str:
-    if not force and not is_stale():
-        return LIB_PATH
+def build_native(force: bool = False, verbose: bool = False, prof: bool = False) -> str:
+    lib_path = PROF_LIB_PATH if prof else LIB_PATH
+    if not force and not is_stale(lib_path):
+        return lib_path
     nvcc = nvcc_path()
     if nvcc is None:
-        raise RuntimeError("nvcc not found: cannot build libdifflinker_b200.so")
+        raise RuntimeError(f"nvcc not found: cannot build {os.path.basename(lib_path)}")
     cmd = [nvcc, "-gencode", "arch=compute_90a,code=sm_90a", "-O3", "-lineinfo", "-std=c++17",
-           "-Xcompiler", "-fPIC", "-shared", "-o", LIB_PATH] + [os.path.join(CSRC, s) for s in SOURCES]
+           "-Xcompiler", "-fPIC", "-shared", "-o", lib_path] + (["-DDL_EDGE_PROF"] if prof else []) + \
+          [os.path.join(CSRC, s) for s in SOURCES]
     if verbose:
         cmd.insert(1, "-Xptxas=-v")
         print(" ".join(cmd), file=sys.stderr)
@@ -44,8 +47,8 @@
         raise RuntimeError(f"nvcc failed:\n{res.stdout}\n{res.stderr}")
     if verbose:
         print(res.stderr, file=sys.stderr)
-    return LIB_PATH
+    return lib_path
 
 
 if __name__ == "__main__":
-    print(build_native(force="--force" in sys.argv, verbose=True))
+    print(build_native(force="--force" in sys.argv, verbose=True, prof="--prof" in sys.argv))
diff --git a/difflinker_b200/csrc/common.cuh b/difflinker_b200/csrc/common.cuh
--- a/difflinker_b200/csrc/common.cuh
+++ b/difflinker_b200/csrc/common.cuh
@@ -121,6 +121,7 @@
   const int* nxr;
   const int4* items;
   const int* n_items;
+  const int* cta_begin;
   const int* xmols;
   const int* n_xmols;
   const int4* xitems;
diff --git a/difflinker_b200/csrc/dl_engine.cu b/difflinker_b200/csrc/dl_engine.cu
--- a/difflinker_b200/csrc/dl_engine.cu
+++ b/difflinker_b200/csrc/dl_engine.cu
@@ -50,6 +50,7 @@
   int4* items = nullptr;
   int4* xitems = nullptr;
   int* tile_ctr = nullptr;
+  int* cta_begin = nullptr;
   std::vector<void*> allocs;
 };
 
@@ -219,6 +220,7 @@
   WSA(agg, n * H); WSA(z, n * xd); WSA(eps, n * xd); WSA(cls, n); WSA(x04, n); WSA(xa4, n); WSA(xb4, n); WSA(ABgmax, n * 2); WSA(ABcmax, n * 2);
   WSA(rowidx, n); WSA(colidx, n); WSA(xrowidx, n); WSA(nr, B); WSA(nc, B); WSA(nxr, B); WSA(n_items, 1);
   WSA(xmols, B); WSA(n_xmols, 1); WSA(items, n); WSA(xitems, n); WSA(n_xitems, 1); WSA(tile_ctr, 64);
+  WSA(cta_begin, e->num_sms + 1);
   if (e->use_tc && e->cfg.graph_type != 0) { WSA(nbr, n * N); WSA(recs, n * CUT_REC); WSA(xrecs, n * CUT_REC); WSA(n_recs, 2); }
 #undef WSA
   ws.B = B; ws.N = N;
@@ -229,7 +231,7 @@
   Plan p;
   p.rowidx = ws.rowidx; p.colidx = ws.colidx; p.xrowidx = ws.xrowidx; p.nr = ws.nr; p.nc = ws.nc; p.nxr = ws.nxr;
   p.items = ws.items; p.n_items = ws.n_items; p.xmols = ws.xmols; p.n_xmols = ws.n_xmols;
-  p.xitems = ws.xitems; p.n_xitems = ws.n_xitems;
+  p.xitems = ws.xitems; p.n_xitems = ws.n_xitems; p.cta_begin = ws.cta_begin;
   return p;
 }
 
@@ -260,7 +262,8 @@
   const int tile_edges = e->use_tc ? tc::TN : ET;
   const int max_rows = e->use_tc ? tc::MAXR : MAXR;
   k_plan_items<<<1, 1, 0, st>>>(B, tile_edges, max_rows, 1, max_rows, ws.nr, ws.nc, ws.nxr, ws.items, ws.n_items, ws.xmols,
-                                ws.n_xmols, ws.xitems, ws.n_xitems);
+                                ws.n_xmols, ws.xitems, ws.n_xitems, e->use_tc ? e->num_sms : 0,
+                                e->use_tc ? ws.cta_begin : nullptr);
   LAUNCH_CHECK();
   e->launches += 2;
   return DL_OK;
@@ -964,6 +967,21 @@
   return DL_OK;
 }
 
+int32_t dl_edge_prof(int32_t n_cta, int64_t* out) {
+#ifdef DL_EDGE_PROF
+  const size_t n = (size_t)std::min<int32_t>(std::max<int32_t>(n_cta, 0), tc::PROF_MAX_CTAS) * tc::PROF_N;
+  if (cudaMemcpyFromSymbol(out, tc::g_edge_prof, n * sizeof(int64_t)) != cudaSuccess) {
+    set_err("dl_edge_prof: %s", cudaGetErrorString(cudaGetLastError()));
+    return DL_ERR_CUDA;
+  }
+  return tc::PROF_N;
+#else
+  (void)n_cta; (void)out;
+  set_err("dl_edge_prof: this library was built without -DDL_EDGE_PROF (python -m difflinker_b200.build --prof)");
+  return DL_ERR_UNSUPPORTED;
+#endif
+}
+
 float dl_time_edge_kernel(dl_engine* e, int32_t reps) {
   if (!e || !e->finalized || e->last_B == 0 || reps < 1) { set_err("dl_time_edge_kernel: no previous forward"); return -1.f; }
   if (cudaSetDevice(e->cfg.device) != cudaSuccess) return -1.f;
diff --git a/difflinker_b200/csrc/kernels_simt.cuh b/difflinker_b200/csrc/kernels_simt.cuh
--- a/difflinker_b200/csrc/kernels_simt.cuh
+++ b/difflinker_b200/csrc/kernels_simt.cuh
@@ -49,11 +49,24 @@
   }
 }
 
+__device__ int gcl_segment_rows(int nc, int tile_edges, int max_rows, int max_tiles) {
+  if (nc * max_rows <= tile_edges) return max_rows;
+  int best = 1;
+  long long best_pad = -1, best_edges = 1;
+  for (int R = 1; (R * nc + tile_edges - 1) / tile_edges <= max_tiles; ++R) {
+    const long long edges = (long long)R * nc;
+    const long long pad = (edges + tile_edges - 1) / tile_edges * tile_edges - edges;
+    if (best_pad < 0 || pad * best_edges < best_pad * edges) { best = R; best_pad = pad; best_edges = edges; }
+  }
+  return best;
+}
+constexpr int GCL_SEGMENT_MAX_TILES = 5;
+
 __global__ void k_plan_items(int B, int tile_edges, int max_rows, int col_pad, int max_rows_gcl, const int* __restrict__ nr,
                              const int* __restrict__ nc, const int* __restrict__ nxr, int4* __restrict__ items,
                              int* __restrict__ n_items, int* __restrict__ xmols, int* __restrict__ n_xmols,
                              int4* __restrict__ xitems, int* __restrict__ n_xitems, int n_cta = 0,
-                             int* __restrict__ cta_begin = nullptr, int* __restrict__ xcta_begin = nullptr) {
+                             int* __restrict__ cta_begin = nullptr) {
   if (threadIdx.x != 0 || blockIdx.x != 0) return;
   int cnt = 0, xc = 0, xi = 0;
   for (int b = 0; b < B; ++b) {
@@ -62,6 +75,7 @@
       const int cp = (c + col_pad - 1) / col_pad * col_pad;
       int per = cp >= tile_edges ? 1 : tile_edges / cp;
       if (per > max_rows_gcl) per = max_rows_gcl;
+      if (cta_begin != nullptr) per = gcl_segment_rows(c, tile_edges, max_rows_gcl, GCL_SEGMENT_MAX_TILES);
       for (int r0 = 0; r0 < r; r0 += per) items[cnt++] = make_int4(b, r0, min(per, r - r0), c);
     }
     if (nxr[b] > 0 && c > 0) {
@@ -82,22 +96,25 @@
   *n_xmols = xc;
   *n_xitems = xi;
   if (n_cta > 0 && cta_begin != nullptr) {
-    for (int pass = 0; pass < 2; ++pass) {
-      const int4* list = pass == 0 ? items : xitems;
-      const int total = pass == 0 ? cnt : xi;
-      int* out = pass == 0 ? cta_begin : xcta_begin;
-      if (out == nullptr) continue;
-      long long sum = 0;
-      for (int k = 0; k < total; ++k) sum += (long long)list[k].z * ((list[k].w + col_pad - 1) / col_pad * col_pad) + 32;
-      long long run = 0;
-      int c = 0;
-      out[0] = 0;
-      for (int k = 0; k < total; ++k) {
-        while (c + 1 < n_cta && run * n_cta >= (long long)(c + 1) * sum) out[++c] = k;
-        run += (long long)list[k].z * ((list[k].w + col_pad - 1) / col_pad * col_pad) + 32;
-      }
-      while (c < n_cta) out[++c] = total;
-    }
+    auto tiles = [&](int k) { return (items[k].z * items[k].w + tile_edges - 1) / tile_edges; };
+    int total = 0, largest = 0;
+    for (int k = 0; k < cnt; ++k) { total += tiles(k); largest = max(largest, tiles(k)); }
+    int cap = max((total + n_cta - 1) / n_cta, largest);
+    for (;; ++cap) {
+      int ctas = 1, load = 0;
+      for (int k = 0; k < cnt; ++k) {
+        if (load + tiles(k) > cap) { ++ctas; load = 0; }
+        load += tiles(k);
+      }
+      if (ctas <= n_cta) break;
+    }
+    int c = 0, load = 0;
+    cta_begin[0] = 0;
+    for (int k = 0; k < cnt; ++k) {
+      if (load + tiles(k) > cap) { cta_begin[++c] = k; load = 0; }
+      load += tiles(k);
+    }
+    while (c < n_cta) cta_begin[++c] = cnt;
   }
 }
 
diff --git a/difflinker_b200/csrc/kernels_tc.cuh b/difflinker_b200/csrc/kernels_tc.cuh
--- a/difflinker_b200/csrc/kernels_tc.cuh
+++ b/difflinker_b200/csrc/kernels_tc.cuh
@@ -192,6 +192,37 @@
   lo = *reinterpret_cast<uint32_t*>(&l);
 }
 __device__ __forceinline__ int gcl_row_of_edge(int e) { return 8 * ((e & 31) >> 1) + 2 * (e >> 5) + (e & 1); }
+enum EdgeProfSlot {
+  PROF_TILES, PROF_CYCLES,
+  PROF_TBL_TOTAL, PROF_TBL_TEMPTY,
+  PROF_PROD_TOTAL, PROF_PROD_TBL, PROF_PROD_EMPTY,
+  PROF_MMA_TOTAL, PROF_MMA_TURN, PROF_MMA_TBL, PROF_MMA_FULL, PROF_MMA_WGMMA, PROF_MMA_W,
+  PROF_MMA_N = PROF_MMA_W - PROF_MMA_TOTAL + 1,
+  PROF_N = PROF_MMA_TOTAL + 2 * PROF_MMA_N
+};
+constexpr int PROF_MAX_CTAS = 1024;
+#ifdef DL_EDGE_PROF
+__device__ long long g_edge_prof[PROF_MAX_CTAS * PROF_N];
+#define EDGE_PROF_WAIT(slot, stmt)                             \
+  do {                                                         \
+    const long long t0_ = clock64();                           \
+    stmt;                                                      \
+    if (prof_rec) s_prof[slot] += clock64() - t0_;             \
+  } while (0)
+#define EDGE_PROF_BEGIN() const long long prof_t0_ = clock64()
+#define EDGE_PROF_END(total, first, last)                                                          \
+  do {                                                                                             \
+    if (prof_rec) {                                                                                \
+      s_prof[total] = clock64() - prof_t0_;                                                        \
+      for (int k_ = (first); k_ < (last); ++k_) g_edge_prof[blockIdx.x * PROF_N + k_] = s_prof[k_]; \
+    }                                                                                              \
+  } while (0)
+#else
+#define EDGE_PROF_WAIT(slot, stmt) stmt
+#define EDGE_PROF_BEGIN() ((void)0)
+#define EDGE_PROF_END(total, first, last) ((void)0)
+#endif
+
 struct Tile {
   int b, nc, slot0, nrt, c0, ncc;
   bool first_chunk, last_chunk;
@@ -229,11 +260,47 @@
       if (per > MAXR) per = MAXR;
       if (rt >= r_count || nc <= 0) { wi += 1; rt = 0; c0 = 0; continue; }
       t.b = b; t.nc = nc; t.slot0 = r_begin + rt; t.nrt = min(per, r_count - rt);
-      t.c0 = c0; t.ncc = min(TN, nc - c0);
+      t.c0 = c0; t.ncc = min(TN, nc - c0); t.Et = t.nrt * t.ncc;
       t.first_chunk = c0 == 0; t.last_chunk = c0 + TN >= nc;
       t.rows = rowlist + (size_t)b * N;
       c0 += TN;
       if (c0 >= nc) { c0 = 0; rt += per; }
+      return true;
+    }
+    return false;
+  }
+};
+
+struct SegIter {
+  const int4* list;
+  const int* rowlist;
+  int N, wi_end, wi, g0, cache_base, lane;
+  int4 cache;
+  __device__ SegIter(const Plan& p, int N_) : N(N_), g0(0), cache_base(-(1 << 30)), lane(threadIdx.x & 31) {
+    list = p.items;
+    rowlist = p.rowidx;
+    wi = p.cta_begin[blockIdx.x];
+    wi_end = p.cta_begin[blockIdx.x + 1];
+    cache = make_int4(0, 0, 0, 0);
+  }
+  __device__ bool next(Tile& t) {
+    while (wi < wi_end) {
+      if (wi - cache_base >= 32) {
+        cache_base = wi;
+        cache = list[min(wi + lane, wi_end - 1)];
+      }
+      const int src = wi - cache_base;
+      const int b = __shfl_sync(0xffffffffu, cache.x, src), r_begin = __shfl_sync(0xffffffffu, cache.y, src);
+      const int r_count = __shfl_sync(0xffffffffu, cache.z, src), nc = __shfl_sync(0xffffffffu, cache.w, src);
+      const int E = r_count * nc;
+      if (g0 >= E) { wi += 1; g0 = 0; continue; }
+      t.b = b; t.nc = nc; t.ncc = nc;
+      t.Et = min(TN, E - g0);
+      const int rf = g0 / nc, rl = (g0 + t.Et - 1) / nc;
+      t.slot0 = r_begin + rf; t.nrt = rl - rf + 1; t.c0 = g0 - rf * nc;
+      t.first_chunk = t.c0 == 0; t.last_chunk = (g0 + t.Et) % nc == 0;
+      t.rows = rowlist + (size_t)b * N;
+      g0 += TN;
       return true;
     }
     return false;
@@ -276,9 +343,12 @@
 };
 
 template <bool COORD, bool SPARSE>
-__device__ __forceinline__ typename std::conditional<SPARSE, RecIter, TileIter<COORD>>::type make_iter(const EdgeArgs& a, int N) {
+using IterOf = typename std::conditional<SPARSE, RecIter, typename std::conditional<COORD, TileIter<true>, SegIter>::type>::type;
+template <bool COORD, bool SPARSE>
+__device__ __forceinline__ IterOf<COORD, SPARSE> make_iter(const EdgeArgs& a, int N) {
   if constexpr (SPARSE) return RecIter(a.recs, a.n_recs);
-  else return TileIter<COORD>(a.plan, N);
+  else if constexpr (COORD) return TileIter<true>(a.plan, N);
+  else return SegIter(a.plan, N);
 }
 
 template <bool COORD, bool SPARSE = false>
@@ -291,6 +361,11 @@
 
   const uint32_t bars = sbase + OFF_BAR;
   float2* b2w5 = reinterpret_cast<float2*>(sm + OFF_B2W5);
+#ifdef DL_EDGE_PROF
+  __shared__ long long s_prof[PROF_N];
+  const bool prof_rec = lane == 0 && (warp == W_TBL || warp == W_PROD || warp == 0 || warp == 4);
+  if (tid < PROF_N) s_prof[tid] = 0;
+#endif
 
   if (tid == 0) {
     mbar_init(bars + BAR_W, 1);
@@ -308,17 +383,19 @@
     asm volatile("setmaxnreg.dec.sync.aligned.u32 %0;" ::"n"(REGS_CTRL));
   if (warp >= W_TBL && warp < W_TBL + N_TBL_WARPS) {
     const int tw = warp - W_TBL;
-    typename std::conditional<SPARSE, RecIter, TileIter<COORD>>::type iter = make_iter<COORD, SPARSE>(a, N);
+    EDGE_PROF_BEGIN();
+    IterOf<COORD, SPARSE> iter = make_iter<COORD, SPARSE>(a, N);
     Tile cur;
     for (int t = 0;; ++t) {
       const int acc = t & (N_ACC - 1);
       const bool more = iter.next(cur);
       if (t % N_TBL_WARPS != tw) { if (!more) break; continue; }
-      if (t >= N_ACC) mbar_wait_relaxed(bars + BAR_TEMPTY + 8 * acc, ((t - N_ACC) / N_ACC) & 1);
+      if (t >= N_ACC)
+        EDGE_PROF_WAIT(PROF_TBL_TEMPTY, mbar_wait_relaxed(bars + BAR_TEMPTY + 8 * acc, ((t - N_ACC) / N_ACC) & 1));
       uint8_t* tb = sm + OFF_TBL + acc * TBL_BYTES;
       int* hdr = reinterpret_cast<int*>(tb + TBL_HDR);
       if (more) {
-        const int Et = SPARSE ? cur.Et : cur.nrt * cur.ncc;
+        const int Et = cur.Et;
         const size_t gb = (size_t)cur.b * N;
         if (lane == 0) {
           hdr[0] = Et; hdr[1] = cur.nrt; hdr[2] = cur.ncc;
@@ -334,7 +411,7 @@
         } else {
           if (lane < cur.nrt) {
             reinterpret_cast<int*>(tb + TBL_ROWNODE)[lane] = cur.rows[cur.slot0 + lane];
-            reinterpret_cast<int*>(tb + TBL_ROWSTART)[lane] = lane * cur.ncc;
+            reinterpret_cast<int*>(tb + TBL_ROWSTART)[lane] = lane == 0 ? 0 : lane * cur.nc - cur.c0;
           }
           if (lane == 0) reinterpret_cast<int*>(tb + TBL_ROWSTART)[cur.nrt] = Et;
         }
@@ -353,9 +430,9 @@
             j = raw & 0x7fffffff;
             ew_list = raw < 0 ? 0.f : 1.f;
           } else {
-            const int rr = ev / cur.ncc, jj = ev - rr * cur.ncc;
+            const int g = cur.c0 + ev, rr = g / cur.nc, jj = g - rr * cur.nc;
             i = cur.rows[cur.slot0 + rr];
-            j = a.plan.colidx[gb + cur.c0 + jj];
+            j = a.plan.colidx[gb + jj];
           }
           const float4 xi = a.x4[gb + i], xj = a.x4[gb + j], yi = a.x04[gb + i], yj = a.x04[gb + j];
           const float dx = xi.x - xj.x, dy = xi.y - xj.y, dz = xi.z - xj.z;
@@ -396,6 +473,7 @@
       if (lane == 0) mbar_arrive(bars + BAR_TBL + 8 * acc);
       if (!more) break;
     }
+    EDGE_PROF_END(PROF_TBL_TOTAL, PROF_TBL_TOTAL, PROF_PROD_TOTAL);
   } else if (warp == W_LOAD) {
     if (lane == 0) {
       mbar_expect_tx(bars + BAR_W, 2 * W_BYTES);
@@ -411,12 +489,14 @@
       wdr[q] = make_float2(__ldg(a.wd + kc * 8 + 2 * q), __ldg(a.wd + kc * 8 + 2 * q + 1));
       w0r[q] = make_float2(__ldg(a.w0 + kc * 8 + 2 * q), __ldg(a.w0 + kc * 8 + 2 * q + 1));
     }
+    EDGE_PROF_BEGIN();
     for (int t = 0;; ++t) {
       const int acc = t & (N_ACC - 1), s = t & (N_STAGE - 1);
-      mbar_wait(bars + BAR_TBL + 8 * acc, (t / N_ACC) & 1);
+      EDGE_PROF_WAIT(PROF_PROD_TBL, mbar_wait(bars + BAR_TBL + 8 * acc, (t / N_ACC) & 1));
       const uint8_t* tb = sm + OFF_TBL + acc * TBL_BYTES;
       const int Et = reinterpret_cast<const int*>(tb + TBL_HDR)[0];
-      if (t >= N_STAGE) mbar_wait(bars + BAR_EMPTY + 8 * s, ((t - N_STAGE) / N_STAGE) & 1);
+      if (t >= N_STAGE)
+        EDGE_PROF_WAIT(PROF_PROD_EMPTY, mbar_wait(bars + BAR_EMPTY + 8 * s, ((t - N_STAGE) / N_STAGE) & 1));
       if (Et > 0) {
         const int* rowoff = reinterpret_cast<const int*>(tb + TBL_ROWOFF);
         const int* coloff = reinterpret_cast<const int*>(tb + TBL_COLOFF);
@@ -427,55 +507,48 @@
         uint8_t* blo = bhi + B_BYTES;
         const bool rescale = reinterpret_cast<const int*>(tb + TBL_HDR)[5] != 0;
         constexpr int ITEMS = TN / (2 * N_PROD_WARPS);
-        float4 pa0, pa1, pb[2][2];
+        constexpr int PF = 2;
+        float4 pa[PF][2], pb[PF][2];
         const int e_base = ITEMS * (2 * pw + esub);
-        int ro_cur = rowoff[e_base];
-        {
-          const float* ap = a.AB + ro_cur + kc * 8;
-          pa0 = __ldg(reinterpret_cast<const float4*>(ap)); pa1 = __ldg(reinterpret_cast<const float4*>(ap + 4));
-        }
-#pragma unroll
-        for (int pf = 0; pf < 2; ++pf) {
+#pragma unroll
+        for (int pf = 0; pf < PF; ++pf) {
+          const float* ap = a.AB + rowoff[e_base + pf] + kc * 8;
           const float* bp = a.AB + coloff[e_base + pf] + kc * 8;
+          pa[pf][0] = __ldg(reinterpret_cast<const float4*>(ap)); pa[pf][1] = __ldg(reinterpret_cast<const float4*>(ap + 4));
           pb[pf][0] = __ldg(reinterpret_cast<const float4*>(bp)); pb[pf][1] = __ldg(reinterpret_cast<const float4*>(bp + 4));
         }
 #pragma unroll
         for (int it = 0; it < ITEMS; ++it) {
           const int e = e_base + it;
-          const int slot = it & 1;
-          const float4 b0 = pb[slot][0], b1 = pb[slot][1];
-          if (it + 2 < ITEMS) {
-            const float* bp = a.AB + coloff[e + 2] + kc * 8;
+          const int slot = it % PF;
+          const float4 a0 = pa[slot][0], a1 = pa[slot][1], b0 = pb[slot][0], b1 = pb[slot][1];
+          if (it + PF < ITEMS) {
+            const float* ap = a.AB + rowoff[e + PF] + kc * 8;
+            const float* bp = a.AB + coloff[e + PF] + kc * 8;
+            pa[slot][0] = __ldg(reinterpret_cast<const float4*>(ap)); pa[slot][1] = __ldg(reinterpret_cast<const float4*>(ap + 4));
             pb[slot][0] = __ldg(reinterpret_cast<const float4*>(bp)); pb[slot][1] = __ldg(reinterpret_cast<const float4*>(bp + 4));
           }
-          const int ro = rowoff[e];
-          if (ro != ro_cur) {
-            ro_cur = ro;
-            const float* ap = a.AB + ro + kc * 8;
-            pa0 = __ldg(reinterpret_cast<const float4*>(ap)); pa1 = __ldg(reinterpret_cast<const float4*>(ap + 4));
-          }
-          const float4 a0 = pa0, a1 = pa1;
-          if (e < Et) {
-            const float d = dv[e], d0 = d0v[e];
-            const float2 dd = make_float2(d, d), dd0 = make_float2(d0, d0);
-            const float2 av[4] = {make_float2(a0.x, a0.y), make_float2(a0.z, a0.w), make_float2(a1.x, a1.y), make_float2(a1.z, a1.w)};
-            const float2 bv[4] = {make_float2(b0.x, b0.y), make_float2(b0.z, b0.w), make_float2(b1.x, b1.y), make_float2(b1.z, b1.w)};
-            float2 sv[4];
-#pragma unroll
-            for (int q = 0; q < 4; ++q)
-              sv[q] = usig2(ffma2(dd0, w0r[q], ffma2(dd, wdr[q], fadd2(av[q], bv[q]))));
-            if (rescale) {
-              const float sc = scv[e];
-#pragma unroll
-              for (int q = 0; q < 4; ++q) sv[q] = fmul2(sv[q], make_float2(sc, sc));
-            }
-            uint4 hi, lo;
-            split2v(sv[0], hi.x, lo.x); split2v(sv[1], hi.y, lo.y);
-            split2v(sv[2], hi.z, lo.z); split2v(sv[3], hi.w, lo.w);
-            const int row = COORD ? e : gcl_row_of_edge(e);
-            *reinterpret_cast<uint4*>(bhi + row * 16) = hi;
-            *reinterpret_cast<uint4*>(blo + row * 16) = lo;
-          }
+          const float d = dv[e], d0 = d0v[e];
+          const float2 dd = make_float2(d, d), dd0 = make_float2(d0, d0);
+          const float2 av[4] = {make_float2(a0.x, a0.y), make_float2(a0.z, a0.w), make_float2(a1.x, a1.y), make_float2(a1.z, a1.w)};
+          const float2 bv[4] = {make_float2(b0.x, b0.y), make_float2(b0.z, b0.w), make_float2(b1.x, b1.y), make_float2(b1.z, b1.w)};
+          float2 uv[4], sv[4];
+#pragma unroll
+          for (int q = 0; q < 4; ++q)
+            uv[q] = ffma2(dd0, w0r[q], ffma2(dd, wdr[q], fadd2(av[q], bv[q])));
+          usig4(uv[0], uv[1], sv[0], sv[1]);
+          usig4(uv[2], uv[3], sv[2], sv[3]);
+          if (rescale) {
+            const float sc = scv[e];
+#pragma unroll
+            for (int q = 0; q < 4; ++q) sv[q] = fmul2(sv[q], make_float2(sc, sc));
+          }
+          uint4 hi, lo;
+          split2v(sv[0], hi.x, lo.x); split2v(sv[1], hi.y, lo.y);
+          split2v(sv[2], hi.z, lo.z); split2v(sv[3], hi.w, lo.w);
+          const int row = COORD ? e : gcl_row_of_edge(e);
+          *reinterpret_cast<uint4*>(bhi + row * 16) = hi;
+          *reinterpret_cast<uint4*>(blo + row * 16) = lo;
         }
         fence_proxy_async();
       }
@@ -483,6 +556,7 @@
       if (lane == 0) mbar_arrive(bars + BAR_FULL + 8 * s);
       if (Et <= 0) break;
     }
+    EDGE_PROF_END(PROF_PROD_TOTAL, PROF_PROD_TOTAL, PROF_MMA_TOTAL);
   } else {
     asm volatile("setmaxnreg.inc.sync.aligned.u32 %0;" ::"n"(REGS_EPI));
     const int g = warp >> 2;
@@ -494,25 +568,28 @@
     float d[64];
 #pragma unroll
     for (int i = 0; i < 64; ++i) d[i] = 0.f;
-    mbar_wait(bars + BAR_W, 0);
-    for (int t = 0;; ++t) {
+    EDGE_PROF_BEGIN();
+    const int pm = PROF_MMA_N * g;
+    EDGE_PROF_WAIT(pm + PROF_MMA_W, mbar_wait(bars + BAR_W, 0));
+    int t = 0;
+    for (;; ++t) {
       const int acc = t & (N_ACC - 1), s = t & (N_STAGE - 1);
-      if (!COORD && g == 0 && t > 0) named_sync(BAR_TURN0, 32 * N_EPI_WARPS);
-      mbar_wait(bars + BAR_TBL + 8 * acc, (t / N_ACC) & 1);
+      if (!COORD && g == 0 && t > 0) EDGE_PROF_WAIT(pm + PROF_MMA_TURN, named_sync(BAR_TURN0, 32 * N_EPI_WARPS));
+      EDGE_PROF_WAIT(pm + PROF_MMA_TBL, mbar_wait(bars + BAR_TBL + 8 * acc, (t / N_ACC) & 1));
       const uint8_t* tb = sm + OFF_TBL + acc * TBL_BYTES;
       const int* hdr = reinterpret_cast<const int*>(tb + TBL_HDR);
       const int Et = hdr[0];
       if (Et <= 0) break;
       const uint32_t bhi = sbase + OFF_ST + s * STAGE_BYTES, blo = bhi + B_BYTES;
       if (!COORD) {
-        if (g == 1) named_sync(BAR_TURN1, 32 * N_EPI_WARPS);
-        mbar_wait(bars + BAR_FULL + 8 * s, (t / N_STAGE) & 1);
+        if (g == 1) EDGE_PROF_WAIT(pm + PROF_MMA_TURN, named_sync(BAR_TURN1, 32 * N_EPI_WARPS));
+        EDGE_PROF_WAIT(pm + PROF_MMA_FULL, mbar_wait(bars + BAR_FULL + 8 * s, (t / N_STAGE) & 1));
         fence_acc(d);
         wg_fence();
         mma_3xf16(d, sbase + OFF_WHI + g * 1024, sbase + OFF_WLO + g * 1024, W_LBO, bhi, blo, B_LBO, 2 * B_LBO, 8, false);
         wg_commit();
         named_arrive(g == 0 ? BAR_TURN1 : BAR_TURN0, 32 * N_EPI_WARPS);
-        wg_wait_all();
+        EDGE_PROF_WAIT(pm + PROF_MMA_WGMMA, wg_wait_all());
         fence_acc(d);
       } else {
         mbar_wait(bars + BAR_FULL + 8 * s, (t / N_STAGE) & 1);
@@ -538,11 +615,21 @@
         uint32_t bmask = 0;
         int nr = cur + 1;
         if (has) { for (; nr <= nrt && rowstart[nr] < E0 + 32; ++nr) bmask |= 1u << (rowstart[nr] - E0); }
-        const bool open_end = has && nr <= nrt && rowstart[nr] > E0 + 32;
+        const bool open_end = has && ((nr <= nrt && rowstart[nr] > E0 + 32) || (!last_chunk && Et <= E0 + 32));
         const bool cut = Et < E0 + 32;
         const uint32_t wmask = __reduce_or_sync(0xffffffffu, bmask);
         float2 hsum = make_float2(0.f, 0.f), sum = make_float2(0.f, 0.f);
         bool in_head = true;
+#pragma unroll
+        for (int tp = 0; tp < 32; tp += 2) {
+          const float4 ed = *reinterpret_cast<const float4*>(emds + E0 + tp);
+          const float2 u0 = ffma2(make_float2(d[2 * tp], d[2 * tp + 2]), make_float2(ed.y, ed.y), bias);
+          const float2 u1 = ffma2(make_float2(d[2 * tp + 1], d[2 * tp + 3]), make_float2(ed.w, ed.w), bias);
+          float2 s0, s1;
+          usig4(u0, u1, s0, s1);
+          const float2 v0 = fmul2(s0, make_float2(ed.x, ed.x)), v1 = fmul2(s1, make_float2(ed.z, ed.z));
+          d[2 * tp] = v0.x; d[2 * tp + 2] = v0.y; d[2 * tp + 1] = v1.x; d[2 * tp + 3] = v1.y;
+        }
 #pragma unroll
         for (int tt = 0; tt < 32; ++tt) {
           if (wmask & (1u << tt)) {
@@ -556,16 +643,12 @@
             in_head = in_head && !here;
             cur += here ? 1 : 0;
           }
-          const float2 ed = emds[E0 + tt];
-          const float2 u = ffma2(make_float2(d[(tt >> 1) * 4 + (tt & 1)], d[(tt >> 1) * 4 + 2 + (tt & 1)]),
-                                 make_float2(ed.y, ed.y), bias);
-          const float2 v = fmul2(usig2(u), make_float2(ed.x, ed.x));
-          sum = fadd2(sum, v);
+          sum = fadd2(sum, make_float2(d[(tt >> 1) * 4 + (tt & 1)], d[(tt >> 1) * 4 + 2 + (tt & 1)]));
         }
         if (in_head) hsum = sum;
         const float2 lsum = sum;
         const bool cont_in = has && rowstart[hrow] < E0;
-        float2 cin = (q == 0 && nrt == 1 && !first_chunk) ? run : make_float2(0.f, 0.f);
+        float2 cin = (q == 0 && !first_chunk) ? run : make_float2(0.f, 0.f);
 #pragma unroll
         for (int k = 0; k < 3; ++k) {
           const float2 cout = in_head ? fadd2(cin, hsum) : lsum;
@@ -573,11 +656,12 @@
           if (q == k + 1 && cont_in) cin = make_float2(px, py);
         }
         const float2 htot = fadd2(cin, hsum);
-        if (nrt == 1) {
+        if (!last_chunk) {
           const int src = (lane & ~3) | ((Et - 1) >> 5);
-          run = make_float2(__shfl_sync(0xffffffffu, htot.x, src), __shfl_sync(0xffffffffu, htot.y, src));
-        }
-        if (has && last_chunk) {
+          const float2 tail = in_head ? htot : lsum;
+          run = make_float2(__shfl_sync(0xffffffffu, tail.x, src), __shfl_sync(0xffffffffu, tail.y, src));
+        }
+        if (has) {
           if (!in_head || !open_end) {
             float* dst = a.agg + (gb + rownode[hrow]) * H;
             dst[r0] = htot.x * inv_norm; dst[r0 + 8] = htot.y * inv_norm;
@@ -634,6 +718,13 @@
         if (lane == 0) mbar_arrive(bars + BAR_TEMPTY + 8 * acc);
       }
     }
+#ifdef DL_EDGE_PROF
+    if (prof_rec && g == 0) {
+      g_edge_prof[blockIdx.x * PROF_N + PROF_TILES] = t;
+      g_edge_prof[blockIdx.x * PROF_N + PROF_CYCLES] = clock64() - prof_t0_;
+    }
+#endif
+    EDGE_PROF_END(pm + PROF_MMA_TOTAL, pm + PROF_MMA_TOTAL, pm + PROF_MMA_TOTAL + PROF_MMA_N);
   }
 }
 
diff --git a/include/difflinker_b200.h b/include/difflinker_b200.h
--- a/include/difflinker_b200.h
+++ b/include/difflinker_b200.h
@@ -92,6 +92,7 @@
 float dl_last_elapsed_ms(dl_engine* e);
 float dl_time_edge_kernel(dl_engine* e, int32_t reps);
 dl_status dl_cut_graph_stats(dl_engine* e, int64_t* out);
+int32_t dl_edge_prof(int32_t n_cta, int64_t* out);
 dl_status dl_selftest_tc(dl_engine* e, float* max_abs_err, float* max_rel_err);
 dl_status dl_selftest_tc_layout(dl_engine* e, int32_t b_mn_major, float* max_abs_err, float* max_rel_err);
 
diff --git a/profiles/edge_roles.py b/profiles/edge_roles.py
--- /dev/null
+++ b/profiles/edge_roles.py
@@ -0,0 +1,57 @@
+import ctypes as C
+import os
+import sys
+
+sys.path.insert(0, os.path.dirname(os.path.dirname(os.path.abspath(__file__))))
+import torch
+
+from difflinker_b200 import _native, build
+
+_native.LIB_PATH = build.build_native(prof=True)
+from difflinker_b200 import DDPM, synthetic
+from difflinker_b200.batching import collate
+from difflinker_b200.ddpm import sampler_inputs
+
+ROLES = [("table warps", 2, {"TEMPTY": 3}),
+         ("producers", 4, {"TBL": 5, "EMPTY": 6}),
+         ("MMA WG 0", 7, {"TURN": 8, "TBL": 9, "FULL": 10, "wgmma": 11, "W": 12}),
+         ("MMA WG 1", 13, {"TURN": 14, "TBL": 15, "FULL": 16, "wgmma": 17, "W": 18})]
+
+wl = sys.argv[1] if len(sys.argv) > 1 else "cfg2_zinc"
+spec = synthetic.SPECS[wl]
+hp = synthetic.model_hparams(spec)
+dev = torch.device("cuda", 0)
+torch.manual_seed(0)
+ddpm = DDPM(**hp)
+synthetic.init_reference_like_weights(ddpm, coord_gain=100.0 if spec.N <= 64 else 1.0)
+ddpm = ddpm.to(dev)
+data = {k: (v.to(dev) if torch.is_tensor(v) else v) for k, v in collate(synthetic.make_items(spec)).items()}
+kw = sampler_inputs(ddpm, data)
+z = torch.cat([kw['x'], kw['h'] / 4], dim=2)
+z = z * kw['fragment_mask'] + torch.randn_like(z) * kw['linker_mask']
+t = torch.full((spec.B, 1), 0.5, device=dev)
+dyn = ddpm.edm.dynamics
+dyn(t, z, kw['node_mask'], kw['linker_mask'], kw['edge_mask'], kw['context'])
+torch.cuda.synchronize()
+lib = _native.load_library()
+assert os.path.basename(lib._name) == os.path.basename(build.PROF_LIB_PATH), lib._name
+eng = dyn.engine(0)
+lib.dl_time_edge_kernel(eng, 1)
+n_cta = torch.cuda.get_device_properties(0).multi_processor_count
+buf = (C.c_int64 * (1024 * 32))()
+n_slot = _native.check(lib.dl_edge_prof(n_cta, buf), "dl_edge_prof")
+rows = [[buf[c * n_slot + k] for k in range(n_slot)] for c in range(n_cta)]
+busy = [r for r in rows if r[0] > 0]
+tiles = sum(r[0] for r in busy)
+slow = max(busy, key=lambda r: r[1])
+print(f"{wl}: {len(busy)} of {n_cta} CTAs with tiles, {tiles} tiles, {max(r[0] for r in busy)} on the busiest CTA; "
+      f"cycles per tile (MMA WG 0 span): all CTAs {sum(r[1] for r in busy) / tiles:.0f}, slowest CTA {slow[1] / slow[0]:.0f} "
+      f"({slow[0]} tiles, {slow[1]} cycles)")
+print(f"{'role':<12} {'cyc/tile':>9} {'work':>7}  waits per tile (all CTAs)                       | slowest CTA: cyc/tile work")
+for name, tot, waits in ROLES:
+    total = sum(r[tot] for r in busy) / tiles
+    w = {k: sum(r[s] for r in busy) / tiles for k, s in waits.items()}
+    s_total = slow[tot] / slow[0]
+    s_work = (slow[tot] - sum(slow[s] for s in waits.values())) / slow[0]
+    ws = "  ".join(f"{k} {v:.0f}" for k, v in w.items())
+    print(f"{name:<12} {total:>9.0f} {total - sum(w.values()):>7.0f}  {ws:<48}| {s_total:.0f} {s_work:.0f}")
```

Result: no change. 167.3, median of 6 (+0.7%).
